# google/supersonic

Measured on AMD Instinct MI355X. Metric: rows/sec filter->project->aggregate, 100M x 8 INT64/DOUBLE, higher is better.
Workload: dtype int64/f64; 1 GPU; Q-FPA-wide: SUM(a+b),COUNT(*),SUM(c),MIN(d),MAX(d0),SUM(d1),SUM(d2*d3) WHERE a>499 over a device-resident 100000000-row x 8-col block per GPU; rows_per_gpu=100000000, parallelism=single GPU, tile_rows=512, grid=768, lds_bytes=35568, specialized_stages=1

## Files before the change

supersonic_amd/csrc/launch.h:

```cpp
#ifndef SSGPU_LAUNCH_H_
#define SSGPU_LAUNCH_H_

#ifndef __HIPCC_RTC__
#include <hip/hip_runtime_api.h>
#include <stdint.h>
#endif
#include "vm.h"

enum SlotKind {
  SLOT_SUM_INT = 0, SLOT_SUM_DD = 1, SLOT_MIN_U64 = 2, SLOT_MAX_U64 = 3, SLOT_MIN_F64 = 4,
  SLOT_MAX_F64 = 5, SLOT_FIRST = 6, SLOT_LAST = 7, SLOT_COUNT = 8
};
enum EmitKind {
  EMIT_U64 = 0, EMIT_I64KEY = 1, EMIT_U32 = 2, EMIT_I32KEY = 3, EMIT_F64 = 4, EMIT_F32 = 5,
  EMIT_DD_F64 = 6, EMIT_DD_F32 = 7, EMIT_U8 = 8,
  EMIT_DDRES_F64 = 9,
  EMIT_CNT_U64 = 20, EMIT_CNT_U32 = 21,
  EMIT_FKEY_F64 = 100, EMIT_FKEY_F32 = 101
};
#define SSGPU_STATE_ARRAYS 8

struct EmitDesc { void* data; uint8_t* is_null; int slot; int out_kind; };

struct GroupKeyOut { void* data; uint8_t* is_null; uint32_t shift, bits, nullbit, width; };
// ... 27 lines not shown
#define SSGPU_PART_MAX_WORDS 20
struct PartAggParams {
  const unsigned long long* recs;
  const unsigned int* counts;
  unsigned int n_segs, seg_cap, rec_words, n_parts;
  unsigned int local_capacity;
  unsigned int n_gaggs;
  unsigned int n_aggs, any_cnt;
  unsigned int slab_segs;
  VmGroupTable T;
  unsigned long long desc[VM_MAX_AGG_SLOTS];
  unsigned int* nan_flag;
  unsigned int hot_only, hot_base;
  DenseKeyMap dense;
};
hipError_t ssgpu_launch_part_agg(const PartAggParams& P, unsigned int lds_bytes, hipStream_t stream);
#if defined(__HIPCC__) || defined(__HIPCC_RTC__)
__device__ __forceinline__ bool ssgpu_dense_index(const DenseKeyMap& D, unsigned long long key, unsigned int* idx) {
  unsigned int i = 0; bool in = true;
  for (unsigned int k = 0; k < D.n_keys; ++k) {
    const DenseKeyMap::Key K = D.keys[k];
    const unsigned long long mask = K.bits >= 64u ? ~0ull : ((1ull << K.bits) - 1ull);
    unsigned long long off = ((key >> K.shift) - K.lo) & mask;
    const bool nullable = K.nullbit != 0xFFu;
    const bool is_null = nullable && ((key >> K.nullbit) & 1ull);
    const unsigned int values = nullable ? K.span - 1u : K.span;
    if (is_null) off = K.span - 1u;
    else if (off >= values) { in = false; off = 0; }
    i += (unsigned int)off * K.stride;
  }
  *idx = i;
  return in;
}
__device__ __forceinline__ unsigned long long ssgpu_dense_key_of(const DenseKeyMap& D, unsigned int idx) {
  unsigned long long key = 0ull;
  for (unsigned int k = 0; k < D.n_keys; ++k) {
    const DenseKeyMap::Key K = D.keys[k];
    const unsigned long long mask = K.bits >= 64u ? ~0ull : ((1ull << K.bits) - 1ull);
    const unsigned int off = (idx / K.stride) % K.span;
    if (K.nullbit != 0xFFu && off == K.span - 1u) key |= 1ull << K.nullbit;
    else key |= ((K.lo + off) & mask) << K.shift;
  }
  return key;
}
__device__ __forceinline__ unsigned int ssgpu_dense_entry(const DenseKeyMap& D, unsigned int idx, unsigned int* part) {
  if (D.n_parts == 1u) { *part = 0u; return idx; }
  unsigned int q = __umulhi(idx, D.parts_inv);
  if (q * D.n_parts > idx) --q;
  *part = idx - q * D.n_parts;
  return q;
}
#endif

#define SSGPU_PSCAT_THREADS 1024
#define SSGPU_PSCAT_XCDS 8
#define SSGPU_PSCAT_MAX_KEYS 8
#define SSGPU_PSCAT_MAX_FIELDS 24
#define SSGPU_PSCAT_MAX_PREDS 4
#define SSGPU_HOT_MAX 32
#define SSGPU_HOT_SLOTS 64
struct PlainScatterParams {
  unsigned long long n_rows;
  unsigned int n_parts, seg_cap, rec_words, rec_inv;
  unsigned int n_keys, n_fields, n_preds;
  struct Key { const void* data; const unsigned char* nulls; unsigned int width, shift, bits, nullbit; } keys[SSGPU_PSCAT_MAX_KEYS];
  struct Field { const void* src; unsigned int width, off; } fields[SSGPU_PSCAT_MAX_FIELDS];
  struct Pred { const void* data; const unsigned char* nulls; unsigned int kind, cmp, col_on_left, pad; unsigned long long bits; } preds[SSGPU_PSCAT_MAX_PREDS];
  unsigned long long* recs;
  unsigned int* counts;
  unsigned int* overflow;
  unsigned int n_hot, hot_pad;
  unsigned long long hot_keys[SSGPU_HOT_MAX];
  DenseKeyMap dense;
};
hipError_t ssgpu_launch_key_domain(const PlainScatterParams& S, const unsigned int* is_signed, unsigned long long* out, int grid, hipStream_t stream);
#define SSGPU_DENSE_HEADER 64
struct DenseFoldParams {
  const void* chunks; unsigned int n_chunks, n_gaggs, any_cnt, slots;
  unsigned long long chunk_bytes;
  unsigned long long* keys; unsigned long long* acc; unsigned int* cnt;
  const unsigned int* merge_op;
  unsigned int* flags_out;
  unsigned int* clear[2]; unsigned int n_clear[2];
};
hipError_t ssgpu_launch_dense_fold(const DenseFoldParams& P, hipStream_t stream);
hipError_t ssgpu_launch_dense_headers(void* chunks, unsigned int n_chunks, unsigned long long chunk_bytes, const unsigned int* overflow4, const unsigned int* error_flag, hipStream_t stream,
                                      unsigned int forced_flags = 0);
hipError_t ssgpu_launch_hot_keys(const PlainScatterParams& S, unsigned long long n_sample, unsigned int min_count, unsigned long long* out, hipStream_t stream);
struct PscatGeom { unsigned int threads, rows, wgs_per_cu, lds, pipe; };
PscatGeom ssgpu_part_scatter_plain_geom(unsigned int n_parts, unsigned int rec_words, int threads, int rows, int wgs_per_cu);
hipError_t ssgpu_launch_part_scatter_plain(const PlainScatterParams& P, const PscatGeom& g, int grid, hipStream_t stream);
struct FoldTailColumn {
  const void* src; const unsigned char* src_nulls; void* dst; unsigned char* dst_nulls; unsigned int op, kind;
  const unsigned long long* by; const unsigned char* by_nulls;
};
hipError_t ssgpu_launch_fold_tail(const FoldTailColumn* cols_dev, unsigned int n_cols, unsigned long long n_in, unsigned long long limit, hipStream_t stream);
unsigned int ssgpu_part_scatter_plain_lds(unsigned int n_parts, unsigned int rec_words, int rows_per_thread, int threads = SSGPU_PSCAT_THREADS);
hipError_t ssgpu_part_agg_set_max_lds(int bytes);
hipError_t ssgpu_launch_group_resident(const PartAggParams& A, const PlainScatterParams& S, unsigned int lds_bytes, int grid, hipStream_t stream);

struct JoinBuildParams {
  const void* key_data[8];
  const unsigned char* key_nulls[8];
  unsigned int width[8], shift[8], bits[8];
  unsigned int n_keys;
  unsigned int capacity_mask;
  unsigned long long n_rows;
  unsigned long long* keys;
  unsigned int* rows;
  unsigned int* special;
  unsigned int* flags;
  unsigned int* counts;
  unsigned int* slot_of_row;
  unsigned int word[8];
  unsigned long long* keys_hi;
};
hipError_t ssgpu_launch_join_expand(const unsigned int* offsets, const unsigned int* run_start, const unsigned int* rows_sorted,
                                    unsigned long long n_lhs, unsigned long long n_out, unsigned int* lhs_idx, unsigned int* rhs_row, hipStream_t stream);
hipError_t ssgpu_launch_join_build(const JoinBuildParams& P, hipStream_t stream);
hipError_t ssgpu_launch_fill_u32(unsigned int* p, unsigned int v, size_t n, hipStream_t stream);
struct GroupInitParams {
  unsigned long long* keys; unsigned long long n_keys;
  unsigned long long* acc; const unsigned long long* pattern; unsigned int ng; unsigned long long n_acc;
  unsigned int* cnt; unsigned long long n_cnt;
  unsigned int* z[4]; unsigned long long nz[4];
  unsigned int n_rep, pad; unsigned long long rep_stride;
};
hipError_t ssgpu_launch_group_init(const GroupInitParams& P, hipStream_t stream);

hipError_t ssgpu_launch_pipeline(const VmParams& P, int K, int grid, hipStream_t stream);
#ifndef __HIPCC_RTC__
#include <string>
void* ssgpu_rtc_specialize(int device, const VmInstr* prog, int n_instr, int K, bool math, const uint32_t* staged_width, const uint32_t* staged_lds_off,
                           int n_staged, uint32_t static_lds, std::string* why);
hipError_t ssgpu_launch_pipeline_rtc(void* handle, const VmParams& P, int grid, bool static_lds, hipStream_t stream);
void* ssgpu_rtc_specialize_part_agg(int device, const unsigned long long* desc, int n_aggs, unsigned int rec_words, unsigned int n_gaggs, bool any_cnt,
                                    unsigned int lds_bytes, std::string* why, const PlainScatterParams* source = nullptr,
                                    bool dense = false,
                                    bool prefetch = false);
hipError_t ssgpu_launch_group_resident_rtc(void* handle, const PartAggParams& A, const PlainScatterParams& S, int grid, hipStream_t stream);
hipError_t ssgpu_launch_part_agg_rtc(void* handle, const PartAggParams& P, hipStream_t stream);
void* ssgpu_rtc_specialize_pscat(int device, const PlainScatterParams& S, const PscatGeom& g, std::string* why);
hipError_t ssgpu_launch_part_scatter_plain_rtc(void* handle, const PlainScatterParams& P, const PscatGeom& g, int grid, hipStream_t stream);
void* ssgpu_rtc_function(void* handle);
void ssgpu_rtc_release(void* handle);
void ssgpu_rtc_cached_only(bool on);
void ssgpu_rtc_mode(int mode);
int ssgpu_rtc_current_mode();
bool ssgpu_rtc_pending();
void ssgpu_rtc_trim(int keep);
void ssgpu_rtc_stats(long long* modules, long long* code_bytes, long long* compilations, long long* disk_hits);
#endif
hipError_t ssgpu_pipeline_set_max_lds(int bytes);
hipError_t ssgpu_launch_finish_slots(const VmAccRec* partials, int n_slots, int n_parts, const int* slot_kind,
                                     VmAccRec* out, uint64_t* state , hipStream_t stream,
                                     const EmitDesc* descs = nullptr, int n_out = 0 );
hipError_t ssgpu_launch_slots_to_state(const VmAccRec* recs, int n_slots, const int* slot_kind, uint64_t* state,
                                       hipStream_t stream);
hipError_t ssgpu_launch_fold_state(const uint64_t* images, int n_images, uint64_t* state, int n_slots, const int* slot_kind, hipStream_t stream);
hipError_t ssgpu_launch_fold_emit(const uint64_t* images, int n_images, uint64_t* state, int n_slots, const int* slot_kind, VmAccRec* recs,
                                  const EmitDesc* descs, int n_out, hipStream_t stream);
hipError_t ssgpu_launch_state_to_slots(const uint64_t* state, int n_slots, const int* slot_kind, VmAccRec* recs,
                                       hipStream_t stream);
hipError_t ssgpu_launch_emit_scalar(const VmAccRec* recs, const EmitDesc* descs, int n_out, hipStream_t stream);
hipError_t ssgpu_launch_scan_counts(const uint32_t* in, uint32_t* out, int n, uint64_t* total, hipStream_t stream);
hipError_t ssgpu_launch_group_count(const GroupExtractParams& P, uint32_t* tile_counts, hipStream_t stream);
hipError_t ssgpu_launch_group_extract_lb(const GroupExtractParams& P, unsigned long long* status, uint64_t epoch, unsigned int* ctrl, unsigned int* error_flag, hipStream_t stream);
hipError_t ssgpu_launch_group_extract(const GroupExtractParams& P, hipStream_t stream);
hipError_t ssgpu_launch_fill_u64(uint64_t* p, uint64_t v, size_t n, hipStream_t stream);
hipError_t ssgpu_launch_fill_pattern_u64(uint64_t* p, const uint64_t* pattern, uint32_t plen, size_t n,
                                         hipStream_t stream);

hipError_t ssgpu_launch_sort_iota(uint32_t* idx, uint64_t n, hipStream_t s);
hipError_t ssgpu_launch_sort_load_keys(uint64_t* keys, const uint32_t* idx, const void* col, const uint8_t* nulls, uint32_t width,
                                       int kind, int descending, int null_pass, uint64_t n, unsigned long long* bits, hipStream_t s);
uint32_t ssgpu_sort_tiles(uint64_t n);
hipError_t ssgpu_launch_sort_hist(const uint64_t* keys, uint32_t shift, uint64_t n, uint32_t* hist, hipStream_t s);
hipError_t ssgpu_launch_sort_scatter(const uint64_t* keys_in, const uint32_t* idx_in, uint64_t* keys_out, uint32_t* idx_out,
                                     uint32_t shift, uint64_t n, const uint32_t* offsets, hipStream_t s);
hipError_t ssgpu_launch_sort_load_keys_hist(uint64_t* keys, const uint32_t* idx, const void* col, const uint8_t* nulls, uint32_t width, int kind,
                                            int descending, int null_pass, uint64_t n, unsigned long long* bits, uint32_t* hist8, uint32_t* base8, hipStream_t s,
                                            uint64_t* compact_out = nullptr);
hipError_t ssgpu_launch_sort_onesweep(const uint64_t* keys_in, const uint32_t* idx_in, uint64_t* keys_out, uint32_t* idx_out, uint32_t shift, uint64_t n,
                                      const uint32_t* digit_base, unsigned long long* status, uint32_t* ticket, uint64_t epoch, uint32_t* stuck, hipStream_t s);
hipError_t ssgpu_launch_sort_fix_ties(uint64_t* keys, uint32_t* idx, uint64_t n, uint32_t hi_shift, uint32_t* too_long, hipStream_t s);
struct SortRecField { const void* src; void* dst; unsigned int off, width; };
#define SSGPU_SORT_MAX_FIELDS 96
struct SortRecParams { void* recs; unsigned long long n; unsigned int stride, n_fields; SortRecField fields[SSGPU_SORT_MAX_FIELDS]; };
hipError_t ssgpu_launch_sort_pack(const SortRecParams& P, hipStream_t s);
hipError_t ssgpu_launch_sort_gather_rec(const SortRecParams& P, const uint32_t* idx, uint32_t idx_stride, hipStream_t s);
hipError_t ssgpu_launch_sort_fix_ties_compact(uint64_t* kc, const uint64_t* keys, uint64_t n, uint32_t* too_long, hipStream_t s);
hipError_t ssgpu_launch_sort_extract_idx(uint32_t* idx, const uint64_t* kc, uint64_t n, hipStream_t s);
struct UnpackPiece { unsigned long long src_off; void* dst; unsigned long long bytes; };
hipError_t ssgpu_launch_unpack(const char* slab, const UnpackPiece* pieces, unsigned int n_pieces, hipStream_t s);
uint64_t ssgpu_str_scan_partials(uint64_t n);
hipError_t ssgpu_launch_str_scan(uint64_t* data, uint64_t n, uint64_t* partials, hipStream_t s);
hipError_t ssgpu_launch_str_hash(const uint8_t* bytes, const uint64_t* offs, const uint8_t* nulls, uint64_t n, uint64_t* hashes, hipStream_t s);
hipError_t ssgpu_launch_str_insert(const uint8_t* bytes, const uint64_t* offs, const uint8_t* nulls, const uint64_t* hashes, uint64_t n,
                                   uint64_t* table, uint64_t cap, uint32_t* row_slot, uint32_t* error, hipStream_t s);
hipError_t ssgpu_launch_str_compact(const uint64_t* table, uint64_t cap, const uint8_t* bytes, const uint64_t* offs, uint32_t* count,
                                    uint32_t* d_slot, uint64_t* d_off, uint64_t* d_len, uint64_t* d_key, uint32_t* d_idx, hipStream_t s);
hipError_t ssgpu_launch_str_sort(uint64_t* d_key, uint32_t* d_idx, uint64_t d, uint64_t p, const uint8_t* bytes, const uint64_t* d_off,
                                 const uint64_t* d_len, hipStream_t s);
hipError_t ssgpu_launch_str_rank(const uint32_t* d_idx, const uint32_t* d_slot, const uint64_t* d_len, uint64_t d, int32_t* slot_rank,
                                 uint64_t* out_len, hipStream_t s);
hipError_t ssgpu_launch_str_codes(const uint32_t* row_slot, const uint8_t* nulls, const int32_t* slot_rank, uint64_t n, int32_t* codes, hipStream_t s);
hipError_t ssgpu_launch_str_gather(const uint8_t* bytes, const uint64_t* d_off, const uint32_t* d_idx, const uint64_t* out_off, uint64_t d,
                                   uint8_t* out, hipStream_t s);
hipError_t ssgpu_launch_str_recode(const int32_t* src, const uint8_t* nulls, const int32_t* remap, int32_t n_remap, uint64_t n, int32_t* dst,
                                   hipStream_t s);
hipError_t ssgpu_launch_sort_unkey(void* out, const uint64_t* keys, uint32_t width, int kind, int descending, uint64_t n, hipStream_t s);
hipError_t ssgpu_launch_sort_gather(void* out, uint8_t* out_nulls, const void* col, const uint8_t* nulls, uint32_t width,
                                    const uint32_t* idx, uint64_t n, hipStream_t s);
hipError_t ssgpu_launch_cluster_count(const void* const* data, const uint8_t* const* nulls, const uint32_t* width, uint32_t nkeys,
                                      uint64_t n, uint32_t* tile_counts, hipStream_t s);
hipError_t ssgpu_launch_cluster_flags(const void* const* data, const uint8_t* const* nulls, const uint32_t* width, uint32_t nkeys,
                                      uint64_t n, uint8_t* flag, hipStream_t s);
hipError_t ssgpu_launch_cluster_assign(const void* const* data, const uint8_t* const* nulls, const uint32_t* width, uint32_t nkeys,
                                       void* const* out_data, uint8_t* const* out_nulls, uint64_t n, const uint32_t* tile_offsets,
                                       uint32_t* seg_id, hipStream_t s);
hipError_t ssgpu_launch_gather_rowid(void* dst, const uint8_t* dst_null, const void* src, uint32_t width, int src_kind, int dst_kind, const uint64_t* rowids,
                                     uint64_t rowid_mask , int64_t row_id_base, const uint64_t* n_rows_dev, uint64_t n_rows_max, hipStream_t stream);
hipError_t ssgpu_launch_seq_sum(const void* src, const uint8_t* src_nulls, int src_kind, const uint32_t* seg_id, uint64_t n,
                                void* dst, uint8_t* dst_nulls, int dst_kind, hipStream_t s, uint64_t first = 0, uint64_t* state = nullptr, int resume = 0);
hipError_t ssgpu_launch_seg_first(const uint32_t* seg_id, const uint64_t* rowid, uint64_t n, uint32_t* first, hipStream_t s);
hipError_t ssgpu_launch_rank_scatter(const uint32_t* sorted, uint64_t n_seg, uint32_t* rank, hipStream_t s);
hipError_t ssgpu_launch_rank_rows(const uint32_t* seg_id, const uint32_t* rank, uint64_t n, uint32_t limit, uint32_t* out_rank, uint8_t* out_own, hipStream_t s);
hipError_t ssgpu_launch_dense_extract(const uint64_t* acc, const uint32_t* cnt, uint32_t n_gaggs, uint64_t n_rows,
                                      const GroupAggOut* outs, uint32_t n_out, hipStream_t s);

struct ImagePiece { const void* src; unsigned long long image_off; unsigned long long unpacked_off; unsigned int width; unsigned int pad; };
#define SSGPU_IMAGE_MAX_PIECES 92
#define SSGPU_IMAGE_HEADER 64
struct ImagePackParams {
  void* image;
  const unsigned long long* rows_dev;
  unsigned long long rows_host, capacity;
  unsigned int n_pieces, n_flags;
  const unsigned int* error_flags[8];
  const unsigned int* retry_flags[4];
  unsigned int n_retry, pad2;
  ImagePiece pieces[SSGPU_IMAGE_MAX_PIECES];
};
struct ImageUnpackParams {
  const void* images; void* unpacked;
  unsigned long long image_bytes, capacity, valid_off, trailer_off;
  unsigned int n_pieces, n_images;
  ImagePiece pieces[SSGPU_IMAGE_MAX_PIECES];
};
hipError_t ssgpu_launch_pack_image(const ImagePackParams& P, hipStream_t s);
struct ImageRoutePieces { unsigned int n_keys, n_dest; unsigned long long image_bytes; unsigned int* counters; unsigned int key_piece[16]; int key_null_piece[16]; };
hipError_t ssgpu_launch_route_images(const ImagePackParams& P, const ImageRoutePieces& R, hipStream_t s);
hipError_t ssgpu_launch_unpack_images(const ImageUnpackParams& P, hipStream_t s);

#endif
```

supersonic_amd/csrc/pipeline_kernels.hip:

```cpp
#ifndef __HIPCC_RTC__
#include <hip/hip_runtime.h>
#include <stdint.h>
#endif
#include "vm.h"
#include "launch.h"
#ifdef SSGPU_RTC_NINSTR
#include "rtc_prog.h"
#endif

typedef unsigned long long u64;
typedef long long i64;
typedef unsigned int u32;
typedef int i32;
typedef unsigned char u8;

#ifdef SSGPU_PC_PROFILE
#define PC_PROF(...) __VA_ARGS__
#else
#define PC_PROF(...)
#endif
struct LdsBase {
  __device__ __forceinline__ char* operator+(u32 off) const {
    return (char*)(__attribute__((address_space(3))) char*)off;
  }
// ... 344 lines not shown
        int src = __ffsll((long long)owner) - 1;                               \
        u64 tval = readlane64(bval, src);                                      \
        if (lane == 0) {                                                       \
          VmAccRec* A = acc_rec(P, I.dst, wave);                               \
          u64 x = A->cnt ? A->v1 : (u64)(IDENT), y = trow;                     \
          if (BETTER) { A->v1 = trow; A->v0 = tval; }                          \
          A->cnt += cnt;                                                       \
        }                                                                      \
      }                                                                        \
    }                                                                          \
  } break;

#define AGG_FUSED_I64(OPNAME, EXPR)                                            \
  case VM_##OPNAME: { CASE_FENCE;                                              \
    if (I.dst < VM_FAST_SLOTS) {                                               \
      u64 acc = F0[I.dst]; u32 ac = FC[I.dst];                                 \
      _Pragma("unroll") FOR_PAIRS {                                            \
        auto va = fetch2<u64>(I.a, I.a_mask, p);                               \
        auto vd = fetch2<u64>(I.d, I.b_mask, p);                               \
        Valid2 m = valid_pair_(p, tile_valid, I.b, I.c);                       \
        { u64 a = va.x, b = vd.x; acc += m.x ? (EXPR) : 0ull; }                \
        { u64 a = va.y, b = vd.y; acc += m.y ? (EXPR) : 0ull; }                \
        ac += (u32)m.x + (u32)m.y;                                             \
      }                                                                        \
      F0[I.dst] = acc; FC[I.dst] = ac;                                         \
    }                                                                          \
  } break;
#define AGG_FUSED_F64(OPNAME, EXPR)                                            \
  case VM_##OPNAME: { CASE_FENCE;                                              \
    if (I.dst < VM_FAST_SLOTS) {                                               \
      DD local; local.hi = u2d(F0[I.dst]); local.lo = u2d(F1[I.dst]); u32 ac = FC[I.dst]; \
      _Pragma("unroll") FOR_PAIRS {                                            \
        auto va = fetch2<double>(I.a, I.a_mask, p);                            \
        auto vd = fetch2<double>(I.d, I.b_mask, p);                            \
        Valid2 m = valid_pair_(p, tile_valid, I.b, I.c);                       \
        { double a = va.x, b = vd.x; if (m.x) local = dd_add_d(local, (EXPR)); } \
        { double a = va.y, b = vd.y; if (m.y) local = dd_add_d(local, (EXPR)); } \
        ac += (u32)m.x + (u32)m.y;                                             \
      }                                                                        \
      F0[I.dst] = d2u(local.hi); F1[I.dst] = d2u(local.lo); FC[I.dst] = ac;    \
    }                                                                          \
  } break;

#define STORE_OP(OPNAME, T)                                                    \
  case VM_##OPNAME: { CASE_FENCE;                                              \
    T* out = reinterpret_cast<T*>(P.outputs[I.dst].dst);                       \
    _Pragma("unroll") FOR_PAIRS {                                              \
      i64 r0 = tile_base + 2 * (i64)p;                                         \
      auto vv = fetch2<T>(I.a, I.a_mask, p);                             \
      if (r0 + 1 < vm_n_rows) {                                                \
        *reinterpret_cast<typename Vec2<T>::type*>(out + r0) = vv;             \
      } else if (r0 < vm_n_rows) {                                             \
        out[r0] = vv.x;                                                        \
      }                                                                        \
    }                                                                          \
  } break;

#define STOREC_OP(OPNAME, T)                                                   \
  case VM_##OPNAME: { CASE_FENCE;                                              \
    T* out = reinterpret_cast<T*>(P.outputs[I.dst].dst);                       \
    _Pragma("unroll") FOR_PAIRS {                                              \
      Valid2 m = valid_pair_(p, tile_valid, VM_NONE, I.c);          \
      auto vv = fetch2<T>(I.a, I.a_mask, p);                             \
      auto rk = lds_load2<u32>(I.b, p);                                        \
      if (m.x) out[rk.x] = vv.x;                                               \
      if (m.y) out[rk.y] = vv.y;                                               \
    }                                                                          \
  } break;

#define KEY_APPEND_OP(OPNAME, T, UT)                                           \
  case VM_##OPNAME: { CASE_FENCE;                                              \
    const u32 shift = (u32)(I.imm & 0xFF), bits = (u32)((I.imm >> 8) & 0xFF);  \
    const u32 nullbit = (u32)((I.imm >> 16) & 0xFF);                           \
    const u64 vmask = bits >= 64 ? ~0ull : ((1ull << bits) - 1ull);            \
    _Pragma("unroll") FOR_PAIRS {                                              \
      auto kk = lds_load2<u64>(I.dst, p);                                      \
      auto vv = lds_load2<T>(I.a, p);                                          \
      u64 a0 = ((u64)(UT)vv.x) & vmask, a1 = ((u64)(UT)vv.y) & vmask;          \
      if (I.b != VM_NONE) {                                                    \
        auto z = lds_load2<u8>(I.b, p);                                        \
        if (z.x) a0 = 1ull << (nullbit - shift);                               \
        if (z.y) a1 = 1ull << (nullbit - shift);                               \
      }                                                                        \
      lds_store2<u64>(I.dst, p, kk.x | (a0 << shift), kk.y | (a1 << shift));   \
    }                                                                          \
  } break;

#define GAGG_PROLOGUE(LOADT)                                                   \
      Valid2 m = valid_pair_(p, tile_valid, I.b, VM_NONE);          \
      auto sl = lds_load2<u32>(I.c, p);                                        \
      m.x = m.x && sl.x != 0xFFFFFFFFu; m.y = m.y && sl.y != 0xFFFFFFFFu;      \
      auto vv = lds_load2<LOADT>(I.a, p);

#define GAGG_APPLY(LOADT, SL, E, ATOM)                                         \
      if ((SL) & VM_SLOT_LOCAL) {                                              \
        const u32 li = ((SL) & ~VM_SLOT_LOCAL) * P.group.local_stride + s;     \
        u64* A = reinterpret_cast<u64*>(smem + P.group.local_acc_off) + li; LOADT e = (E); ATOM; \
        if (has_cnt) atomicAdd(reinterpret_cast<u32*>(smem + P.group.local_cnt_off) + li, 1u); \
      } else {                                                                 \
        u64* A = &P.group.acc[(u64)(SL) * ng + s]; LOADT e = (E); ATOM;        \
        if (has_cnt) atomicAdd(&P.group.cnt[(u64)(SL) * ng + s], 1u);          \
      }

#define GAGG_ATOMIC(OPNAME, LOADT, ATOM)                                       \
  case VM_##OPNAME: { CASE_FENCE;                                              \
    const u32 ng = (u32)(I.imm >> 32) & 0x7FFFFFFFu, s = (u32)I.imm;           \
    const bool has_cnt = (I.imm >> 63) != 0;                                   \
    _Pragma("unroll") FOR_PAIRS {                                              \
      GAGG_PROLOGUE(LOADT)                                                     \
      if (m.x) { GAGG_APPLY(LOADT, sl.x, vv.x, ATOM) }                         \
      if (m.y) { GAGG_APPLY(LOADT, sl.y, vv.y, ATOM) }                         \
    }                                                                          \
  } break;

__device__ __noinline__ u32 lookback_rows_before(unsigned long long* status, int tile, u32 run, u64 tag, unsigned int* ctrl, unsigned int* error_flag, int lane) {
  unsigned long long* const mine = status + tile;
  if (lane == 0) __hip_atomic_store(mine, (1ull << 62) | tag | (u64)run, __ATOMIC_RELAXED, __HIP_MEMORY_SCOPE_AGENT);
  u32 excl = 0, spins = 0;
  for (int j0 = tile - 1; j0 >= 0;) {
    const int j = j0 - lane;
    u64 v = (2ull << 62) | tag;
    if (j >= 0) v = __hip_atomic_load(status + j, __ATOMIC_RELAXED, __HIP_MEMORY_SCOPE_AGENT);
    const bool ready = (v >> 62) != 0 && (v & (0x3FFFFFFFull << 32)) == tag;
    const u64 pending = __ballot(!ready), prefixes = __ballot(ready && (v >> 62) == 2);
    const u32 stop = prefixes ? (u32)__builtin_ctzll(prefixes) : 63u;
    const u64 need = stop >= 63u ? ~0ull : ((2ull << stop) - 1ull);
    if (pending & need) {
      __builtin_amdgcn_s_sleep(2);
      if (++spins > (1u << 22)) { if (lane == 0) { atomicExch(ctrl + 3, 1u); atomicExch(error_flag, 3u); } break; }
      continue;
    }
    u32 part = (u32)lane <= stop ? (u32)v : 0u;
    for (int o = 32; o > 0; o >>= 1) part += (u32)__shfl_xor((int)part, o);
    excl += part;
    if (prefixes) break;
    j0 -= 64;
  }
  if (lane == 0) __hip_atomic_store(mine, (2ull << 62) | tag | (u64)(excl + run), __ATOMIC_RELAXED, __HIP_MEMORY_SCOPE_AGENT);
  return excl;
}

__device__ __forceinline__ double vm_math1(u32 fn, double a) {
  switch (fn) {
    case VM_MATH_EXP: return exp(a);     case VM_MATH_LN: return log(a);       case VM_MATH_LOG10: return log10(a);
    case VM_MATH_LOG2: return log2(a);   case VM_MATH_SIN: return sin(a);      case VM_MATH_COS: return cos(a);
    case VM_MATH_TAN: return tan(a);     case VM_MATH_ASIN: return asin(a);    case VM_MATH_ACOS: return acos(a);
    case VM_MATH_ATAN: return atan(a);   case VM_MATH_SINH: return sinh(a);    case VM_MATH_COSH: return cosh(a);
    case VM_MATH_TANH: return tanh(a);   case VM_MATH_ASINH: return asinh(a);  case VM_MATH_ACOSH: return acosh(a);
    default: return atanh(a);
  }
}

#ifndef SSGPU_RTC_PART
template <int K, bool MATH>
__global__ __launch_bounds__(VM_WG_THREADS, VM_WAVES_PER_EU) void ssgpu_pipeline_kernel(const VmParams P) {
#ifdef SSGPU_RTC_STATIC_LDS
  __shared__ __attribute__((aligned(16))) char rtc_static_lds[SSGPU_RTC_STATIC_LDS];
  asm volatile("" ::"v"((u32)(size_t)(__attribute__((address_space(3))) char*)rtc_static_lds));
#endif
  const int t = threadIdx.x;
  const int lane = t & 63;
  const int wave = t >> 6;
  const int tile_rows = VM_TILE_UNIT * K;
  i64 vm_n_rows = P.n_rows; int vm_n_tiles = P.n_tiles;
  if (P.n_rows_dev) {
    const u64 have = *P.n_rows_dev;
    vm_n_rows = have < (u64)P.n_rows ? (i64)have : P.n_rows;
    vm_n_tiles = (int)((vm_n_rows + tile_rows - 1) / tile_rows);
  }
  const int vm_first_tile = ((P.flags & VM_FLAG_XCD_CHUNKS) && (gridDim.x & 7u) == 0u) ? (int)((blockIdx.x & 7u) * (gridDim.x >> 3) + (blockIdx.x >> 3)) : (int)blockIdx.x;
  const int n_my_tiles = vm_n_tiles > vm_first_tile ? (vm_n_tiles - vm_first_tile + (int)gridDim.x - 1) / (int)gridDim.x : 0;
  const int n_units = STAGED_COUNT(P) * K;

  for (u32 o = (u32)t * 8u; o < (u32)P.n_slots * VM_ACC_STRIDE; o += VM_COMPUTE_THREADS * 8u)
    *reinterpret_cast<u64*>(smem + P.acc_lds_off + o) = 0ull;
  typedef u64 u64xS __attribute__((ext_vector_type(VM_FAST_SLOTS)));
  typedef u32 u32xS __attribute__((ext_vector_type(VM_FAST_SLOTS)));
  u64xS F0, F1; u32xS FC;
#pragma unroll
  for (int s = 0; s < VM_FAST_SLOTS; ++s) { F0[s] = P.slot_init0[s]; F1[s] = P.slot_init1[s]; FC[s] = 0; }
  bool vm_nan_seen = false;
  for (u32 o = (u32)t * 8u; o < 2u * (u32)tile_rows; o += VM_COMPUTE_THREADS * 8u)
    *reinterpret_cast<u64*>(smem + P.const_lds_off + o) = o < (u32)tile_rows ? 0x0101010101010101ull : 0ull;

  typedef u32 u32x8 __attribute__((ext_vector_type(8)));
  typedef const __attribute__((address_space(4))) u32x8* ProgPtr;
  const ProgPtr prog0 = (ProgPtr)(P.prog);

  for (int pc = t; pc < P.n_instr; pc += VM_COMPUTE_THREADS) {
    const VmInstr J = P.prog[pc];
    const u32 w = J.imm_width;
    if (w) {
      u64 lo = J.imm;
      if (w == 4) lo = (lo & 0xFFFFFFFFull) * 0x100000001ull;
      else if (w == 1) lo = (lo & 0xFFull) * 0x0101010101010101ull;
      u64* e = reinterpret_cast<u64*>(smem + P.imm_pool_lds_off + (u32)pc * 16u);
      e[0] = lo; e[1] = lo;
    }
  }

  if (P.group.local_capacity) {
    const VmGroupTable& G = P.group;
    for (u32 e = (u32)t; e < G.local_capacity; e += VM_COMPUTE_THREADS)
      reinterpret_cast<u64*>(smem + G.local_keys_off)[e] = VM_KEY_EMPTY;
    for (u32 i = (u32)t; i < G.local_capacity * G.local_stride; i += VM_COMPUTE_THREADS) {
      reinterpret_cast<u64*>(smem + G.local_acc_off)[i] = G.acc_init[(i % G.local_stride) % G.n_gaggs];
      if (G.local_cnt_off != VM_NONE) reinterpret_cast<u32*>(smem + G.local_cnt_off)[i] = 0u;
    }
    if (t < 2) reinterpret_cast<u32*>(smem + P.scratch_lds_off + 128u)[t] = 0u;
  }
  if (P.part_n) {
    u32* h = reinterpret_cast<u32*>(smem + P.part_lds_off);
    for (u32 i = (u32)t; i < P.part_n; i += VM_COMPUTE_THREADS) h[i] = 0u;
  }
  PC_PROF(if (P.debug_pc) for (int i = t; i <= P.n_instr; i += VM_COMPUTE_THREADS) reinterpret_cast<u64*>(smem + P.debug_pc_lds_off)[i] = 0ull;)
  __syncthreads();

  u32x4 pf[VM_PF_UNITS];
#pragma unroll
  for (int u = 0; u < VM_PF_UNITS; ++u) pf[u] = u32x4{0u, 0u, 0u, 0u};
  const int n_pf = n_units < VM_PF_UNITS ? n_units : VM_PF_UNITS;
  {
    const i64 tb = (i64)vm_first_tile * tile_rows;
    if (n_my_tiles > 0 && tb + tile_rows <= vm_n_rows) {
#pragma unroll
      for (int u = 0; u < VM_PF_UNITS; ++u)
        if (u < n_pf) load_unit<K>(P, u, tb, t, pf[u]);
    }
  }

  u64 dbg_wait = 0;
  const u64 dbg_t0 = P.debug ? __builtin_amdgcn_s_memtime() : 0;
  const ProgPtr prog = prog0;
  for (int it = 0; it < n_my_tiles; ++it) {
    const int tile = vm_first_tile + it * (int)gridDim.x;
    const i64 tile_base = (i64)tile * tile_rows;
    const u32 tile_valid = (u32)((vm_n_rows - tile_base) < (i64)tile_rows ? (vm_n_rows - tile_base) : (i64)tile_rows);
    const u64 tw0 = (P.debug || P.debug_pc) ? __builtin_amdgcn_s_memtime() : 0;
    __builtin_amdgcn_s_setprio(VM_STAGE_PRIO);
    if (tile_valid == (u32)tile_rows) {
      int tc = t;
      asm volatile("" : "+v"(tc));
#pragma unroll
      for (int u = 0; u < VM_PF_UNITS; ++u)
        if (u < n_pf) commit_unit<K>(P, u, pf[u], tc);
      if (P.debug) dbg_wait += __builtin_amdgcn_s_memtime() - tw0;
      if (n_units > VM_PF_UNITS) stage_units_direct<K>(P, VM_PF_UNITS, n_units, tile_base, tile_valid, t);
    } else {
      stage_units_direct<K>(P, 0, n_units, tile_base, tile_valid, t);
    }
    {
      const i64 tb = tile_base + (i64)gridDim.x * tile_rows;
      if (it + 1 < n_my_tiles && tb + tile_rows <= vm_n_rows) {
        int tl = t;
        asm volatile("" : "+v"(tl));
#pragma unroll
        for (int u = 0; u < VM_PF_UNITS; ++u)
          if (u < n_pf) load_unit<K>(P, u, tb, tl, pf[u]);
      }
    }

    __builtin_amdgcn_s_setprio(0);
#ifdef SSGPU_RTC_NINSTR
#define VM_PC_LOOP _Pragma("unroll") for (int pc = 0; pc < SSGPU_RTC_NINSTR; ++pc)
#define VM_FETCH_NEXT(pc) u32x8{kRtcProg[pc][0], kRtcProg[pc][1], kRtcProg[pc][2], kRtcProg[pc][3], kRtcProg[pc][4], kRtcProg[pc][5], kRtcProg[pc][6], kRtcProg[pc][7]}
    (void)prog;
    u32x8 raw_next = VM_FETCH_NEXT(0);
#else
#define VM_PC_LOOP for (int pc = 0; pc < P.n_instr; ++pc)
#define VM_FETCH_NEXT(pc) prog[pc]
    u32x8 raw_next = prog[0];
#endif
    PC_PROF(u64 dbg_pc_last = 0;
    if (P.debug_pc) { dbg_pc_last = __builtin_amdgcn_s_memtime(); if (t == 0) reinterpret_cast<u64*>(smem + P.debug_pc_lds_off)[P.n_instr] += dbg_pc_last - tw0; })
#ifdef SSGPU_RTC_NINSTR
#include "rtc_steps.h"
#else
    VM_PC_LOOP {
#include "vm_body.inc"
    }
#endif
    PC_PROF(if (P.debug_pc && P.n_instr > 0 && t == 0) reinterpret_cast<u64*>(smem + P.debug_pc_lds_off)[P.n_instr - 1] += __builtin_amdgcn_s_memtime() - dbg_pc_last;)
  }

  if (vm_nan_seen && P.error_flag) atomicOr(P.error_flag, SSGPU_FLAG_NAN_IN_MINMAX);
  if (P.part_n && P.tile_counts) {
    __syncthreads();
    const u32* h = reinterpret_cast<const u32*>(smem + P.part_lds_off);
    for (u32 i = (u32)t; i < P.part_n; i += VM_COMPUTE_THREADS) P.tile_counts[(u64)i * gridDim.x + blockIdx.x] = h[i] < P.part_seg_cap ? h[i] : P.part_seg_cap;
  }
  if (P.group.local_capacity) {
    const VmGroupTable& G = P.group;
    __syncthreads();
    const u32 ng = G.n_gaggs;
    u32 occupied = 0;
    for (u32 e = (u32)t; e < G.local_capacity; e += VM_COMPUTE_THREADS) {
      const u64 key = reinterpret_cast<const u64*>(smem + G.local_keys_off)[e];
      if (key == VM_KEY_EMPTY) continue;
      ++occupied;
      const u32 gs = group_insert(G, key);
      if (gs == 0xFFFFFFFFu) continue;
      for (u32 s = 0; s < ng; ++s) {
        const u64 v = reinterpret_cast<const u64*>(smem + G.local_acc_off)[e * G.local_stride + s];
        u64* A = &G.acc[(u64)gs * ng + s];
        const u32 op = G.merge_op[s];
        if (op == VM_MERGE_ADD_U64) { if (v) atomicAdd(A, v); }
        else if (op == VM_MERGE_MIN_U64) atomicMin(A, v);
        else if (op == VM_MERGE_MAX_U64) atomicMax(A, v);
        else if (op == VM_MERGE_ADD_F64_HI) dd_atomic_add(reinterpret_cast<double*>(A), u2d(v));
        else unsafeAtomicAdd(reinterpret_cast<double*>(A), u2d(v));
        if (G.local_cnt_off != VM_NONE) {
          const u32 c = reinterpret_cast<const u32*>(smem + G.local_cnt_off)[e * G.local_stride + s];
          if (c) atomicAdd(&G.cnt[(u64)gs * ng + s], c);
        }
      }
    }
    u32* st = reinterpret_cast<u32*>(smem + P.scratch_lds_off + 128u);
    if (occupied) atomicAdd(&st[1], occupied);
    __syncthreads();
    if (t == 0) { if (st[0]) atomicAdd(&G.stats[0], st[0]); atomicMax(&G.stats[1], st[1]); }
  }

  PC_PROF(if (P.debug_pc && t == 0) for (int i = 0; i <= P.n_instr; ++i) atomicAdd(&P.debug_pc[i], reinterpret_cast<const u64*>(smem + P.debug_pc_lds_off)[i]);)
  if (P.debug && t == 0) {
    P.debug[blockIdx.x * 4 + 0] = __builtin_amdgcn_s_memtime() - dbg_t0;
    P.debug[blockIdx.x * 4 + 1] = dbg_wait;
    P.debug[blockIdx.x * 4 + 2] = (u64)n_my_tiles;
  }
#pragma unroll
  for (int s = 0; s < VM_FAST_SLOTS; ++s) {
    if (s < P.n_slots) {
      const int kind = P.slot_kind[s];
      const u64 cnt = wave_reduce_u64((u64)FC[s], [](u64 x, u64 y) { return x + y; });
      u64 v0 = 0, v1 = 0;
      switch (kind) {
        case SLOT_COUNT: v0 = cnt; break;
        case SLOT_SUM_INT: v0 = wave_reduce_u64(F0[s], [](u64 x, u64 y) { return x + y; }); break;
        case SLOT_MIN_U64: v0 = wave_reduce_u64(F0[s], [](u64 x, u64 y) { return x < y ? x : y; }); break;
        case SLOT_MAX_U64: v0 = wave_reduce_u64(F0[s], [](u64 x, u64 y) { return x > y ? x : y; }); break;
        case SLOT_MIN_F64: v0 = wave_reduce_u64(F0[s], [](u64 x, u64 y) { return u2d(y) < u2d(x) ? y : x; }); break;
        case SLOT_MAX_F64: v0 = wave_reduce_u64(F0[s], [](u64 x, u64 y) { return u2d(x) < u2d(y) ? y : x; }); break;
        case SLOT_SUM_DD: {
          DD d; d.hi = u2d(F0[s]); d.lo = u2d(F1[s]);
          d = wave_reduce_dd(d); v0 = d2u(d.hi); v1 = d2u(d.lo);
        } break;
        case SLOT_FIRST: case SLOT_LAST: {
          const bool first = kind == SLOT_FIRST;
          const u64 trow = first ? wave_reduce_u64(F1[s], [](u64 x, u64 y) { return x < y ? x : y; })
                                 : wave_reduce_u64(FC[s] ? F1[s] : 0ull, [](u64 x, u64 y) { return x > y ? x : y; });
          const u64 owner = __ballot(FC[s] != 0 && F1[s] == trow);
          const int src = owner ? __ffsll((long long)owner) - 1 : 0;
          v0 = readlane64(F0[s], src); v1 = trow;
        } break;
        default: break;
      }
      if (lane == 0) { VmAccRec* A = acc_rec(P, (u32)s, wave); A->v0 = v0; A->v1 = v1; A->cnt = cnt; A->pad = 0; }
    }
  }

  __syncthreads();
  for (int s = t; s < P.n_slots; s += VM_COMPUTE_THREADS)
    for (int w = 0; w < VM_WAVES; ++w)
      P.wg_partials[((size_t)blockIdx.x * P.n_slots + s) * VM_WAVES + w] = *acc_rec(P, (u32)s, w);
}
#endif

#ifndef __HIPCC_RTC__

__device__ __forceinline__ void combine_rec(int kind, VmAccRec& acc, const VmAccRec& r) {
  if (r.cnt == 0) return;
  switch (kind) {
    case SLOT_COUNT:
    case SLOT_SUM_INT: acc.v0 += r.v0; break;
    case SLOT_SUM_DD: {
      DD a; a.hi = u2d(acc.v0); a.lo = u2d(acc.v1);
      DD b; b.hi = u2d(r.v0); b.lo = u2d(r.v1);
      a = dd_add(a, b); acc.v0 = d2u(a.hi); acc.v1 = d2u(a.lo);
    } break;
    case SLOT_MIN_U64: acc.v0 = acc.cnt ? (r.v0 < acc.v0 ? r.v0 : acc.v0) : r.v0; break;
    case SLOT_MAX_U64: acc.v0 = acc.cnt ? (r.v0 > acc.v0 ? r.v0 : acc.v0) : r.v0; break;
    case SLOT_MIN_F64: acc.v0 = acc.cnt ? (u2d(r.v0) < u2d(acc.v0) ? r.v0 : acc.v0) : r.v0; break;
    case SLOT_MAX_F64: acc.v0 = acc.cnt ? (u2d(acc.v0) < u2d(r.v0) ? r.v0 : acc.v0) : r.v0; break;
    case SLOT_FIRST: if (!acc.cnt || r.v1 < acc.v1) { acc.v0 = r.v0; acc.v1 = r.v1; } break;
    case SLOT_LAST: if (!acc.cnt || r.v1 >= acc.v1) { acc.v0 = r.v0; acc.v1 = r.v1; } break;
  }
  acc.cnt += r.cnt;
}

__device__ __forceinline__ void slot_to_state(const VmAccRec r, int kind, int s, int n_slots, u64* __restrict__ state) {
  u64* sum_i = state; u64* cnt = state + n_slots; u64* hi = state + 2 * n_slots; u64* lo = state + 3 * n_slots;
  u64* mn = state + 4 * n_slots; u64* mx = state + 5 * n_slots;
  u64* mnf = state + 6 * n_slots; u64* mxf = state + 7 * n_slots;
  const bool fl = kind == SLOT_FIRST || kind == SLOT_LAST;
  sum_i[s] = (kind == SLOT_SUM_INT || kind == SLOT_COUNT || fl) ? r.v0 : 0;
  cnt[s] = r.cnt;
  hi[s] = kind == SLOT_SUM_DD ? r.v0 : d2u(0.0);
  lo[s] = kind == SLOT_SUM_DD ? r.v1 : d2u(0.0);
  mn[s] = (kind == SLOT_MIN_U64 && r.cnt) ? (r.v0 ^ 0x8000000000000000ull) : (kind == SLOT_FIRST && r.cnt) ? (r.v1 ^ 0x8000000000000000ull) : 0x7FFFFFFFFFFFFFFFull;
  mx[s] = (kind == SLOT_MAX_U64 && r.cnt) ? (r.v0 ^ 0x8000000000000000ull) : (kind == SLOT_LAST && r.cnt) ? (r.v1 ^ 0x8000000000000000ull) : 0x8000000000000000ull;
  mnf[s] = (kind == SLOT_MIN_F64 && r.cnt) ? r.v0 : d2u(__builtin_inf());
  mxf[s] = (kind == SLOT_MAX_F64 && r.cnt) ? r.v0 : d2u(-__builtin_inf());
}
__device__ __forceinline__ VmAccRec state_to_slot(const u64* __restrict__ state, int kind, int s, int n_slots) {
  VmAccRec r; r.v0 = 0; r.v1 = 0; r.pad = 0;
  r.cnt = state[n_slots + s];
  switch (kind) {
    case SLOT_COUNT: case SLOT_SUM_INT: r.v0 = state[s]; break;
    case SLOT_SUM_DD: {
      DD a; a.hi = u2d(state[2 * n_slots + s]); a.lo = 0.0;
      a = dd_add_d(a, u2d(state[3 * n_slots + s]));
      r.v0 = d2u(a.hi); r.v1 = d2u(a.lo);
    } break;
    case SLOT_MIN_U64: r.v0 = state[4 * n_slots + s] ^ 0x8000000000000000ull; break;
    case SLOT_MAX_U64: r.v0 = state[5 * n_slots + s] ^ 0x8000000000000000ull; break;
    case SLOT_MIN_F64: r.v0 = state[6 * n_slots + s]; break;
    case SLOT_MAX_F64: r.v0 = state[7 * n_slots + s]; break;
    case SLOT_FIRST: r.v0 = state[s]; r.v1 = state[4 * n_slots + s] ^ 0x8000000000000000ull; break;
    case SLOT_LAST: r.v0 = state[s]; r.v1 = state[5 * n_slots + s] ^ 0x8000000000000000ull; break;
    default: break;
  }
  return r;
}

__device__ __forceinline__ void emit_scalar_one(const EmitDesc d, const VmAccRec r);
__global__ __launch_bounds__(256) void ssgpu_finish_slots_kernel(const VmAccRec* __restrict__ partials, int n_slots,
                                                                 int n_parts, const int* __restrict__ slot_kind,
                                                                 VmAccRec* __restrict__ out, u64* __restrict__ state,
                                                                 const EmitDesc* __restrict__ descs, int n_out) {
  __shared__ VmAccRec tree[256];
  const int s = blockIdx.x, t = threadIdx.x;
  const int kind = slot_kind[s];
  VmAccRec acc; acc.v0 = 0; acc.v1 = 0; acc.cnt = 0; acc.pad = 0;
  if (kind == SLOT_SUM_DD) { acc.v0 = d2u(-0.0); acc.v1 = d2u(0.0); }
  for (int i = t; i < n_parts; i += 256) {
    const VmAccRec r = partials[((size_t)(i / VM_WAVES) * n_slots + s) * VM_WAVES + (i % VM_WAVES)];
    combine_rec(kind, acc, r);
  }
  tree[t] = acc;
  __syncthreads();
  for (int stride = 128; stride > 0; stride >>= 1) {
    if (t < stride) { VmAccRec a = tree[t]; combine_rec(kind, a, tree[t + stride]); tree[t] = a; }
    __syncthreads();
  }
  if (t == 0) { out[s] = tree[0]; if (state) slot_to_state(tree[0], kind, s, n_slots, state); }
  if (descs)
    for (int i = t; i < n_out; i += 256) { const EmitDesc d = descs[i]; if (d.slot == s) emit_scalar_one(d, tree[0]); }
}

__global__ void ssgpu_slots_to_state_kernel(const VmAccRec* __restrict__ recs, int n_slots,
                                            const int* __restrict__ slot_kind, u64* __restrict__ state) {
  int s = blockIdx.x * blockDim.x + threadIdx.x;
  if (s >= n_slots) return;
  slot_to_state(recs[s], slot_kind[s], s, n_slots, state);
}
__global__ void ssgpu_state_to_slots_kernel(const u64* __restrict__ state, int n_slots,
                                            const int* __restrict__ slot_kind, VmAccRec* __restrict__ recs) {
  int s = blockIdx.x * blockDim.x + threadIdx.x;
  if (s >= n_slots) return;
  recs[s] = state_to_slot(state, slot_kind[s], s, n_slots);
}


__device__ __forceinline__ void emit_value(void* dst, size_t idx, int out_kind, u64 v0, u64 v1) {
  switch (out_kind) {
    case EMIT_U64: reinterpret_cast<u64*>(dst)[idx] = v0; break;
    case EMIT_I64KEY: reinterpret_cast<i64*>(dst)[idx] = unkey_i64(v0); break;
    case EMIT_U32: reinterpret_cast<u32*>(dst)[idx] = (u32)v0; break;
    case EMIT_I32KEY: reinterpret_cast<i32*>(dst)[idx] = (i32)unkey_i64(v0); break;
    case EMIT_F64: reinterpret_cast<double*>(dst)[idx] = u2d(v0); break;
    case EMIT_F32: reinterpret_cast<float*>(dst)[idx] = (float)u2d(v0); break;
    case EMIT_DD_F64: { double hi = u2d(v0), lo = u2d(v1);
      reinterpret_cast<double*>(dst)[idx] = (lo == 0.0) ? hi : hi + lo; } break;
    case EMIT_DDRES_F64: { const double hi = u2d(v0), lo = u2d(v1), sm = hi + lo, bp = sm - hi;
      reinterpret_cast<double*>(dst)[idx] = (lo == 0.0) ? 0.0 : (hi - (sm - bp)) + (lo - bp); } break;
    case EMIT_DD_F32: { double hi = u2d(v0), lo = u2d(v1);
      reinterpret_cast<float*>(dst)[idx] = (float)((lo == 0.0) ? hi : hi + lo); } break;
    case EMIT_U8: reinterpret_cast<u8*>(dst)[idx] = (u8)(v0 != 0); break;
    default: break;
  }
}


__device__ __forceinline__ void emit_scalar_one(const EmitDesc d, const VmAccRec r) {
  if (d.out_kind == EMIT_CNT_U64 || d.out_kind == EMIT_CNT_U32)
    emit_value(d.data, 0, d.out_kind == EMIT_CNT_U64 ? EMIT_U64 : EMIT_U32, r.cnt, 0);
  else
    emit_value(d.data, 0, d.out_kind, r.v0, r.v1);
  if (d.is_null) d.is_null[0] = r.cnt == 0;
}
__global__ void ssgpu_emit_scalar_kernel(const VmAccRec* __restrict__ recs, const EmitDesc* __restrict__ descs,
                                         int n_out) {
  int i = blockIdx.x * blockDim.x + threadIdx.x;
  if (i >= n_out) return;
  const EmitDesc d = descs[i];
  emit_scalar_one(d, recs[d.slot]);
}

__global__ __launch_bounds__(1024) void ssgpu_scan_counts_kernel(const u32* __restrict__ in, u32* __restrict__ out,
                                                                  int n, u64* __restrict__ total) {
  __shared__ u64 wave_sums[16];
  __shared__ u64 carry_s;
  const int t = threadIdx.x, lane = t & 63, wave = t >> 6;
  if (t == 0) carry_s = 0;
  __syncthreads();
  for (int base = 0; base < n; base += 1024 * 8) {
    u32 v[8]; u64 sum = 0;
    int i0 = base + t * 8;
#pragma unroll
    for (int j = 0; j < 8; ++j) { v[j] = (i0 + j < n) ? in[i0 + j] : 0u; sum += v[j]; }
    u64 inc = sum;
#pragma unroll
    for (int d = 1; d < 64; d <<= 1) { u64 o = __shfl_up(inc, d); if (lane >= d) inc += o; }
    if (lane == 63) wave_sums[wave] = inc;
    __syncthreads();
    u64 wpre = 0;
    for (int w = 0; w < wave; ++w) wpre += wave_sums[w];
    u64 run = carry_s + wpre + (inc - sum);
#pragma unroll
    for (int j = 0; j < 8; ++j) { if (i0 + j < n) out[i0 + j] = (u32)run; run += v[j]; }
    __syncthreads();
    if (t == 1023) carry_s = run;
    __syncthreads();
  }
  if (t == 0) *total = carry_s;
}

__device__ __forceinline__ bool group_slot_occupied(const GroupExtractParams& P, u32 slot) {
  if (slot > P.capacity + P.extra_slots) return false;
  return P.keys[slot] != VM_KEY_EMPTY;
}

__global__ __launch_bounds__(256) void ssgpu_group_count_kernel(const GroupExtractParams P, u32* __restrict__ tile_counts) {
  __shared__ u32 wsum[4];
  const int t = threadIdx.x, lane = t & 63, wave = t >> 6;
  u32 s0 = blockIdx.x * 512u + t * 2u;
  bool o0 = group_slot_occupied(P, s0);
  bool o1 = group_slot_occupied(P, s0 + 1);
  u32 c = (u32)__popcll(__ballot(o0)) + (u32)__popcll(__ballot(o1));
  if (lane == 0) wsum[wave] = c;
  __syncthreads();
  if (t == 0) tile_counts[blockIdx.x] = wsum[0] + wsum[1] + wsum[2] + wsum[3];
}

__device__ __forceinline__ void group_extract_slot(const GroupExtractParams& P, u32 slot, u32 row);
__global__ __launch_bounds__(256) void ssgpu_group_extract_lb_kernel(const GroupExtractParams P, unsigned long long* __restrict__ status, u64 tag,
                                                                     unsigned int* __restrict__ ctrl, unsigned int* __restrict__ error_flag) {
  __shared__ u32 wsum[4];
  __shared__ u32 s_tile, s_base;
  const int t = threadIdx.x, lane = t & 63, wave = t >> 6;
  if (t == 0) s_tile = atomicAdd(ctrl + 2, 1u);
  __syncthreads();
  const u32 tile = s_tile;
  const u32 s0 = tile * 512u + (u32)t * 2u;
  const bool o0 = group_slot_occupied(P, s0), o1 = group_slot_occupied(P, s0 + 1);
  const u64 b0 = __ballot(o0), b1 = __ballot(o1);
  if (lane == 0) wsum[wave] = (u32)__popcll(b0) + (u32)__popcll(b1);
  __syncthreads();
  if (wave == 0) {
    const u32 run = wsum[0] + wsum[1] + wsum[2] + wsum[3];
    const u32 excl = lookback_rows_before(status, (int)tile, run, tag, ctrl, error_flag, lane);
    if (lane == 0) {
      s_base = excl;
      if (tile == gridDim.x - 1u) *reinterpret_cast<u64*>(ctrl) = (u64)excl + run;
    }
  }
  __syncthreads();
  u32 base = s_base;
  for (int w = 0; w < wave; ++w) base += wsum[w];
  const u64 lt = (1ull << lane) - 1ull;
  const u32 r0 = base + (u32)__popcll(b0 & lt) + (u32)__popcll(b1 & lt);
  if (o0) group_extract_slot(P, s0, r0);
  if (o1) group_extract_slot(P, s0 + 1, r0 + (o0 ? 1u : 0u));
}

__global__ __launch_bounds__(256) void ssgpu_group_extract_kernel(const GroupExtractParams P) {
  __shared__ u32 wsum[4];
  const int t = threadIdx.x, lane = t & 63, wave = t >> 6;
  u32 s0 = blockIdx.x * 512u + t * 2u;
  bool o0 = group_slot_occupied(P, s0);
  bool o1 = group_slot_occupied(P, s0 + 1);
  u64 b0 = __ballot(o0), b1 = __ballot(o1);
  if (lane == 0) wsum[wave] = (u32)__popcll(b0) + (u32)__popcll(b1);
  __syncthreads();
  u32 base = P.tile_offsets[blockIdx.x];
  for (int w = 0; w < wave; ++w) base += wsum[w];
  const u64 lt = (1ull << lane) - 1ull;
  u32 r0 = base + (u32)__popcll(b0 & lt) + (u32)__popcll(b1 & lt);
  if (o0) group_extract_slot(P, s0, r0);
  if (o1) group_extract_slot(P, s0 + 1, r0 + (o0 ? 1u : 0u));
}
__device__ __forceinline__ void group_extract_slot(const GroupExtractParams& P, u32 slot, u32 row) {
  {
    const u64 key = slot == P.capacity ? VM_KEY_EMPTY : P.keys[slot];
    for (u32 q = 0; q < P.n_keys; ++q) {
      const GroupKeyOut ko = P.keys_out[q];
      u64 field = key >> ko.shift;
      bool isnull = ko.nullbit != 0xFF && ((key >> ko.nullbit) & 1ull);
      u64 vmask = ko.bits >= 64 ? ~0ull : ((1ull << ko.bits) - 1ull);
      u64 v = isnull ? 0ull : (field & vmask);
      if (ko.width == 8) reinterpret_cast<u64*>(ko.data)[row] = v;
      else if (ko.width == 4) reinterpret_cast<u32*>(ko.data)[row] = (u32)v;
      else reinterpret_cast<u8*>(ko.data)[row] = (u8)v;
      if (ko.is_null) ko.is_null[row] = isnull;
    }
    for (u32 q = 0; q < P.n_aggs_out; ++q) {
      const GroupAggOut ao = P.aggs_out[q];
      u64 v0 = P.acc[(u64)slot * P.n_gaggs + ao.s];
      u32 c = ao.has_cnt ? P.cnt[(u64)slot * P.n_gaggs + ao.s] : 1u;
      if (ao.out_kind == EMIT_FKEY_F64) {
        v0 = (v0 & 0x8000000000000000ull) ? (v0 & 0x7FFFFFFFFFFFFFFFull) : ~v0;
        emit_value(ao.data, row, EMIT_F64, v0, 0);
      } else if (ao.out_kind == EMIT_FKEY_F32) {
        v0 = (v0 & 0x8000000000000000ull) ? (v0 & 0x7FFFFFFFFFFFFFFFull) : ~v0;
        emit_value(ao.data, row, EMIT_F32, v0, 0);
      } else {
        emit_value(ao.data, row, ao.out_kind, v0, (ao.out_kind == EMIT_DD_F64 || ao.out_kind == EMIT_DDRES_F64) ? P.acc[(u64)slot * P.n_gaggs + ao.s + 1] : 0ull);
      }
      if (ao.is_null) ao.is_null[row] = c == 0;
    }
  }
}

#endif

#if !defined(__HIPCC_RTC__) || defined(SSGPU_RTC_PART)
#ifdef SSGPU_RTC_PART
#include "rtc_part.h"
#define PART_NG(P) kPartNg
#define PART_W(P) kPartW
#define PART_ANY_CNT(P) (kPartAnyCnt != 0u)
#define PART_NAGGS(P) kPartNAggs
#define PART_AGG_LOOP _Pragma("unroll") for (u32 s = 0; s < kPartNAggs; ++s)
#define PART_DESC(s) kPartDesc[s]
#define PART_DENSE(P) (kPartDense != 0u)
#else
#define PART_NG(P) (P).n_gaggs
#define PART_W(P) (P).rec_words
#define PART_ANY_CNT(P) ((P).any_cnt != 0u)
#define PART_NAGGS(P) (P).n_aggs
#define PART_AGG_LOOP for (u32 s = 0; s < n_aggs; ++s)
#define PART_DESC(s) readlane64(mydesc, (int)(s))
#define PART_DENSE(P) ((P).dense.on != 0u)
// ... 635 lines not shown
  size_t stride = (size_t)gridDim.x * blockDim.x;
  for (; i < n; i += stride) p[i] = v;
}

__global__ void ssgpu_fill_u64_kernel(u64* __restrict__ p, u64 v, size_t n) {
  size_t i = (size_t)blockIdx.x * blockDim.x + threadIdx.x;
  size_t stride = (size_t)gridDim.x * blockDim.x;
  for (; i < n; i += stride) p[i] = v;
}
__global__ __launch_bounds__(256) void ssgpu_group_init_kernel(const GroupInitParams P) {
  const u64 first = (u64)blockIdx.x * 256 + threadIdx.x, stride = (u64)gridDim.x * 256;
  for (u32 r = 0; r <= P.n_rep; ++r) {
    u64* const keys = reinterpret_cast<u64*>(reinterpret_cast<char*>(P.keys) + (u64)r * P.rep_stride);
    u64* const acc = reinterpret_cast<u64*>(reinterpret_cast<char*>(P.acc) + (u64)r * P.rep_stride);
    u32* const cnt = reinterpret_cast<u32*>(reinterpret_cast<char*>(P.cnt) + (u64)r * P.rep_stride);
    for (u64 i = first; i < P.n_keys; i += stride) keys[i] = VM_KEY_EMPTY;
    for (u64 i = first; i < P.n_acc; i += stride) acc[i] = P.pattern[i % P.ng];
    for (u64 i = first; i < P.n_cnt; i += stride) cnt[i] = 0u;
  }
  for (int q = 0; q < 4; ++q) for (u64 i = first; i < P.nz[q]; i += stride) P.z[q][i] = 0u;
}
__global__ void ssgpu_fill_pattern_u64_kernel(u64* __restrict__ p, const u64* __restrict__ pattern, u32 plen, size_t n) {
  size_t i = (size_t)blockIdx.x * blockDim.x + threadIdx.x;
  size_t stride = (size_t)gridDim.x * blockDim.x;
  for (; i < n; i += stride) p[i] = pattern[i % plen];
}

hipError_t ssgpu_launch_pipeline(const VmParams& P, int K, int grid, hipStream_t stream) {
  dim3 g(grid), b(VM_WG_THREADS);
  size_t lds = P.lds_bytes;
  if (P.uses_math) {
    switch (K) {
      case 1: hipLaunchKernelGGL((ssgpu_pipeline_kernel<1, true>), g, b, lds, stream, P); break;
      case 2: hipLaunchKernelGGL((ssgpu_pipeline_kernel<2, true>), g, b, lds, stream, P); break;
      case 4: hipLaunchKernelGGL((ssgpu_pipeline_kernel<4, true>), g, b, lds, stream, P); break;
      default: return hipErrorInvalidValue;
    }
    return hipGetLastError();
  }
  switch (K) {
    case 1: hipLaunchKernelGGL((ssgpu_pipeline_kernel<1, false>), g, b, lds, stream, P); break;
    case 2: hipLaunchKernelGGL((ssgpu_pipeline_kernel<2, false>), g, b, lds, stream, P); break;
    case 4: hipLaunchKernelGGL((ssgpu_pipeline_kernel<4, false>), g, b, lds, stream, P); break;
    default: return hipErrorInvalidValue;
  }
  return hipGetLastError();
}
__global__ __launch_bounds__(256) void ssgpu_join_expand_kernel(const u32* __restrict__ offsets, const u32* __restrict__ run_start,
                                                                const u32* __restrict__ rows_sorted, u64 n_lhs, u64 n_out,
                                                                u32* __restrict__ lhs_idx, u32* __restrict__ rhs_row) {
  const u64 o = (u64)blockIdx.x * 256 + threadIdx.x;
  if (o >= n_out) return;
  u64 lo = 0, hi = n_lhs - 1;
  while (lo < hi) {
    const u64 mid = (lo + hi + 1) >> 1;
    if ((u64)offsets[mid] <= o) lo = mid; else hi = mid - 1;
  }
  const u32 s = run_start[lo];
  lhs_idx[o] = (u32)lo;
  rhs_row[o] = s == VM_NONE ? VM_NONE : rows_sorted[(u64)s + (o - (u64)offsets[lo])];
}
hipError_t ssgpu_launch_join_expand(const unsigned int* offsets, const unsigned int* run_start, const unsigned int* rows_sorted,
                                    unsigned long long n_lhs, unsigned long long n_out, unsigned int* lhs_idx, unsigned int* rhs_row, hipStream_t stream) {
  if (n_out) hipLaunchKernelGGL(ssgpu_join_expand_kernel, dim3((unsigned)((n_out + 255) / 256)), dim3(256), 0, stream,
                                offsets, run_start, rows_sorted, (u64)n_lhs, (u64)n_out, lhs_idx, rhs_row);
  return hipGetLastError();
}
hipError_t ssgpu_launch_join_build(const JoinBuildParams& P, hipStream_t stream) {
  if (P.n_rows) hipLaunchKernelGGL(ssgpu_join_build_kernel, dim3((unsigned)((P.n_rows + 255) / 256)), dim3(256), 0, stream, P);
  return hipGetLastError();
}
__global__ __launch_bounds__(256) void ssgpu_gather_rowid_kernel(void* __restrict__ dst, const u8* __restrict__ dst_null, const void* __restrict__ src,
                                                                 u32 width, int src_kind, int dst_kind, const u64* __restrict__ rowids, u64 rowid_mask, i64 row_id_base,
                                                                 const u64* __restrict__ n_rows_dev, u64 n_rows_max) {
  const u64 i = (u64)blockIdx.x * 256 + threadIdx.x;
  const u64 n = n_rows_dev ? *n_rows_dev : n_rows_max;
  if (i >= n || i >= n_rows_max) return;
  const bool isnull = dst_null && dst_null[i];
  const u64 r = isnull ? 0ull : (u64)((i64)(rowids[i] & rowid_mask) - row_id_base);
  if (src_kind == dst_kind) {
    if (width == 8) reinterpret_cast<u64*>(dst)[i] = isnull ? 0ull : reinterpret_cast<const u64*>(src)[r];
    else if (width == 4) reinterpret_cast<u32*>(dst)[i] = isnull ? 0u : reinterpret_cast<const u32*>(src)[r];
    else reinterpret_cast<u8*>(dst)[i] = isnull ? (u8)0 : reinterpret_cast<const u8*>(src)[r];
    return;
  }
  i64 vi = 0; u64 vu = 0; double vf = 0.0; int fam = 0;
  if (!isnull) switch (src_kind) {
    case 0: vi = reinterpret_cast<const i32*>(src)[r]; fam = 0; break;
    case 1: vu = reinterpret_cast<const u32*>(src)[r]; fam = 1; break;
    case 2: vi = reinterpret_cast<const i64*>(src)[r]; fam = 0; break;
    case 3: vu = reinterpret_cast<const u64*>(src)[r]; fam = 1; break;
    case 4: vf = (double)reinterpret_cast<const float*>(src)[r]; fam = 2; break;
    case 5: vf = reinterpret_cast<const double*>(src)[r]; fam = 2; break;
    default: vu = reinterpret_cast<const u8*>(src)[r]; fam = 1; break;
  }
  if (dst_kind == 4 || dst_kind == 5) {
    const double d = fam == 2 ? vf : (fam == 1 ? (double)vu : (double)vi);
    if (dst_kind == 5) reinterpret_cast<double*>(dst)[i] = d;
    else reinterpret_cast<float*>(dst)[i] = fam == 2 ? (float)vf : (fam == 1 ? (float)vu : (float)vi);
    return;
  }
  u64 bits;
  if (fam == 2) {
    const double tr = trunc(vf);
    bits = (tr >= -9223372036854775808.0 && tr < 9223372036854775808.0) ? (u64)(i64)tr : 0x8000000000000000ull;
  } else bits = fam == 1 ? vu : (u64)vi;
  if (dst_kind == 2 || dst_kind == 3) reinterpret_cast<u64*>(dst)[i] = bits;
  else if (dst_kind == 0 || dst_kind == 1) reinterpret_cast<u32*>(dst)[i] = (u32)bits;
  else reinterpret_cast<u8*>(dst)[i] = (u8)bits;
}
hipError_t ssgpu_launch_gather_rowid(void* dst, const uint8_t* dst_null, const void* src, uint32_t width, int src_kind, int dst_kind, const uint64_t* rowids, uint64_t rowid_mask,
                                     int64_t row_id_base, const uint64_t* n_rows_dev, uint64_t n_rows_max, hipStream_t stream) {
  if (n_rows_max) hipLaunchKernelGGL(ssgpu_gather_rowid_kernel, dim3((unsigned)((n_rows_max + 255) / 256)), dim3(256), 0, stream,
                                     dst, dst_null, src, width, src_kind, dst_kind, (const u64*)rowids, (u64)rowid_mask, (i64)row_id_base, (const u64*)n_rows_dev, (u64)n_rows_max);
  return hipGetLastError();
}
hipError_t ssgpu_launch_fill_u32(unsigned int* p, unsigned int v, size_t n, hipStream_t stream) {
  if (n) hipLaunchKernelGGL(ssgpu_fill_u32_kernel, dim3((unsigned)std::min<size_t>((n + 255) / 256, 4096)), dim3(256), 0, stream, p, v, n);
  return hipGetLastError();
}
hipError_t ssgpu_launch_part_agg(const PartAggParams& P, unsigned int lds_bytes, hipStream_t stream) {
  if (P.rec_words <= 8) hipLaunchKernelGGL(ssgpu_part_agg_kernel<8>, dim3(P.n_parts), dim3(SSGPU_PART_THREADS), lds_bytes, stream, P);
  else if (P.rec_words <= 16) hipLaunchKernelGGL(ssgpu_part_agg_kernel<16>, dim3(P.n_parts), dim3(SSGPU_PART_THREADS), lds_bytes, stream, P);
  else if (P.rec_words <= SSGPU_PART_MAX_WORDS) hipLaunchKernelGGL(ssgpu_part_agg_kernel<SSGPU_PART_MAX_WORDS>, dim3(P.n_parts), dim3(SSGPU_PART_THREADS), lds_bytes, stream, P);
  else return hipErrorInvalidValue;
  return hipGetLastError();
}
hipError_t ssgpu_launch_group_resident(const PartAggParams& P, const PlainScatterParams& S, unsigned int lds_bytes, int grid, hipStream_t stream) {
  if (P.rec_words <= 8) hipLaunchKernelGGL(ssgpu_group_resident_kernel<8>, dim3(grid), dim3(SSGPU_PART_THREADS), lds_bytes, stream, P, S);
  else hipLaunchKernelGGL(ssgpu_group_resident_kernel<16>, dim3(grid), dim3(SSGPU_PART_THREADS), lds_bytes, stream, P, S);
  return hipGetLastError();
}
hipError_t ssgpu_part_agg_set_max_lds(int bytes) {
  hipError_t e = hipFuncSetAttribute(reinterpret_cast<const void*>(ssgpu_part_agg_kernel<8>), hipFuncAttributeMaxDynamicSharedMemorySize, bytes);
  if (e != hipSuccess) return e;
  e = hipFuncSetAttribute(reinterpret_cast<const void*>(ssgpu_group_resident_kernel<8>), hipFuncAttributeMaxDynamicSharedMemorySize, bytes);
  if (e != hipSuccess) return e;
  e = hipFuncSetAttribute(reinterpret_cast<const void*>(ssgpu_group_resident_kernel<16>), hipFuncAttributeMaxDynamicSharedMemorySize, bytes);
  if (e != hipSuccess) return e;
  e = hipFuncSetAttribute(reinterpret_cast<const void*>(ssgpu_part_agg_kernel<SSGPU_PART_MAX_WORDS>), hipFuncAttributeMaxDynamicSharedMemorySize, bytes);
  if (e != hipSuccess) return e;
  return hipFuncSetAttribute(reinterpret_cast<const void*>(ssgpu_part_agg_kernel<16>), hipFuncAttributeMaxDynamicSharedMemorySize, bytes);
}
hipError_t ssgpu_pipeline_set_max_lds(int bytes) {
  hipError_t e;
  e = hipFuncSetAttribute(reinterpret_cast<const void*>(ssgpu_pipeline_kernel<1, false>), hipFuncAttributeMaxDynamicSharedMemorySize, bytes); if (e != hipSuccess) return e;
  e = hipFuncSetAttribute(reinterpret_cast<const void*>(ssgpu_pipeline_kernel<2, false>), hipFuncAttributeMaxDynamicSharedMemorySize, bytes); if (e != hipSuccess) return e;
  e = hipFuncSetAttribute(reinterpret_cast<const void*>(ssgpu_pipeline_kernel<4, false>), hipFuncAttributeMaxDynamicSharedMemorySize, bytes); if (e != hipSuccess) return e;
  e = hipFuncSetAttribute(reinterpret_cast<const void*>(ssgpu_pipeline_kernel<1, true>), hipFuncAttributeMaxDynamicSharedMemorySize, bytes); if (e != hipSuccess) return e;
  e = hipFuncSetAttribute(reinterpret_cast<const void*>(ssgpu_pipeline_kernel<2, true>), hipFuncAttributeMaxDynamicSharedMemorySize, bytes); if (e != hipSuccess) return e;
  e = hipFuncSetAttribute(reinterpret_cast<const void*>(ssgpu_pipeline_kernel<4, true>), hipFuncAttributeMaxDynamicSharedMemorySize, bytes);
  return e;
}
hipError_t ssgpu_launch_finish_slots(const VmAccRec* partials, int n_slots, int n_parts, const int* slot_kind,
                                     VmAccRec* out, uint64_t* state, hipStream_t stream, const EmitDesc* descs, int n_out) {
  hipLaunchKernelGGL(ssgpu_finish_slots_kernel, dim3(n_slots), dim3(256), 0, stream, partials, n_slots, n_parts, slot_kind, out, (u64*)state, descs, n_out);
  return hipGetLastError();
}
hipError_t ssgpu_launch_slots_to_state(const VmAccRec* recs, int n_slots, const int* slot_kind, uint64_t* state, hipStream_t stream) {
  int blocks = (n_slots + 63) / 64;
  hipLaunchKernelGGL(ssgpu_slots_to_state_kernel, dim3(blocks), dim3(64), 0, stream, recs, n_slots, slot_kind, (u64*)state);
  return hipGetLastError();
}
__device__ __forceinline__ void fold_state_slot(const u64* __restrict__ images, int n_images, u64* __restrict__ state, int n_slots, int kind, int s);
__global__ __launch_bounds__(64) void ssgpu_fold_state_kernel(const u64* __restrict__ images, int n_images, u64* __restrict__ state,
                                                              int n_slots, const int* __restrict__ slot_kind) {
  const int s = blockIdx.x * 64 + threadIdx.x;
  if (s >= n_slots) return;
  fold_state_slot(images, n_images, state, n_slots, slot_kind[s], s);
}
__device__ __forceinline__ void fold_state_slot(const u64* __restrict__ images, int n_images, u64* __restrict__ state, int n_slots, int kind, int s) {
  const size_t total = (size_t)SSGPU_STATE_ARRAYS * n_slots;
  u64 a[SSGPU_STATE_ARRAYS];
  for (int k = 0; k < SSGPU_STATE_ARRAYS; ++k) a[k] = images[(size_t)k * n_slots + s];
  for (int r = 1; r < n_images; ++r) {
    u64 v[SSGPU_STATE_ARRAYS];
    for (int k = 0; k < SSGPU_STATE_ARRAYS; ++k) v[k] = images[(size_t)r * total + (size_t)k * n_slots + s];
    if (kind == SLOT_FIRST) { if ((i64)v[4] < (i64)a[4]) a[0] = v[0]; }
    else if (kind == SLOT_LAST) { if ((i64)v[5] > (i64)a[5]) a[0] = v[0]; }
    else a[0] += v[0];
    a[1] += v[1];
    a[2] = d2u(u2d(a[2]) + u2d(v[2]));
    a[3] = d2u(u2d(a[3]) + u2d(v[3]));
    a[4] = (i64)v[4] < (i64)a[4] ? v[4] : a[4];
    a[5] = (i64)v[5] > (i64)a[5] ? v[5] : a[5];
    a[6] = u2d(v[6]) < u2d(a[6]) ? v[6] : a[6];
    a[7] = u2d(v[7]) > u2d(a[7]) ? v[7] : a[7];
  }
  for (int k = 0; k < SSGPU_STATE_ARRAYS; ++k) state[(size_t)k * n_slots + s] = a[k];
}
__global__ __launch_bounds__(256) void ssgpu_fold_emit_kernel(const u64* __restrict__ images, int n_images, u64* __restrict__ state, int n_slots,
                                                              const int* __restrict__ slot_kind, VmAccRec* __restrict__ recs,
                                                              const EmitDesc* __restrict__ descs, int n_out) {
  for (int s = threadIdx.x; s < n_slots; s += 256) {
    fold_state_slot(images, n_images, state, n_slots, slot_kind[s], s);
    recs[s] = state_to_slot(state, slot_kind[s], s, n_slots);
  }
  __threadfence_block();
  __syncthreads();
  for (int i = threadIdx.x; i < n_out; i += 256) { const EmitDesc d = descs[i]; emit_scalar_one(d, recs[d.slot]); }
}
hipError_t ssgpu_launch_fold_emit(const uint64_t* images, int n_images, uint64_t* state, int n_slots, const int* slot_kind, VmAccRec* recs,
                                  const EmitDesc* descs, int n_out, hipStream_t stream) {
  hipLaunchKernelGGL(ssgpu_fold_emit_kernel, dim3(1), dim3(256), 0, stream, (const u64*)images, n_images, (u64*)state, n_slots, slot_kind, recs, descs, n_out);
  return hipGetLastError();
}
hipError_t ssgpu_launch_fold_state(const uint64_t* images, int n_images, uint64_t* state, int n_slots, const int* slot_kind, hipStream_t stream) {
  if (n_slots > 0) hipLaunchKernelGGL(ssgpu_fold_state_kernel, dim3((n_slots + 63) / 64), dim3(64), 0, stream, (const u64*)images, n_images, (u64*)state, n_slots, slot_kind);
  return hipGetLastError();
}
hipError_t ssgpu_launch_state_to_slots(const uint64_t* state, int n_slots, const int* slot_kind, VmAccRec* recs, hipStream_t stream) {
  int blocks = (n_slots + 63) / 64;
  hipLaunchKernelGGL(ssgpu_state_to_slots_kernel, dim3(blocks), dim3(64), 0, stream, (const u64*)state, n_slots, slot_kind, recs);
  return hipGetLastError();
}
hipError_t ssgpu_launch_emit_scalar(const VmAccRec* recs, const EmitDesc* descs, int n_out, hipStream_t stream) {
  int blocks = (n_out + 63) / 64;
  hipLaunchKernelGGL(ssgpu_emit_scalar_kernel, dim3(blocks), dim3(64), 0, stream, recs, descs, n_out);
  return hipGetLastError();
}
__global__ __launch_bounds__(1024) void ssgpu_scan_chunk_totals_kernel(const u32* __restrict__ in, int n, u32* __restrict__ totals) {
  __shared__ u64 wave_sums[16];
  const int t = threadIdx.x, lane = t & 63, wave = t >> 6;
  const int i0 = blockIdx.x * 8192 + t * 8;
  u64 sum = 0;
#pragma unroll
  for (int j = 0; j < 8; ++j) sum += (i0 + j < n) ? in[i0 + j] : 0u;
#pragma unroll
  for (int d = 32; d > 0; d >>= 1) sum += __shfl_xor(sum, d);
  if (lane == 0) wave_sums[wave] = sum;
  __syncthreads();
  if (t == 0) { u64 s = 0; for (int w = 0; w < 16; ++w) s += wave_sums[w]; totals[blockIdx.x] = (u32)s; }
}
__global__ __launch_bounds__(1024) void ssgpu_scan_chunks_kernel(const u32* __restrict__ in, u32* __restrict__ out, int n,
                                                                  const u32* __restrict__ chunk_base) {
  __shared__ u64 wave_sums[16];
  const int t = threadIdx.x, lane = t & 63, wave = t >> 6;
  const int i0 = blockIdx.x * 8192 + t * 8;
  u32 v[8]; u64 sum = 0;
#pragma unroll
  for (int j = 0; j < 8; ++j) { v[j] = (i0 + j < n) ? in[i0 + j] : 0u; sum += v[j]; }
  u64 inc = sum;
#pragma unroll
  for (int d = 1; d < 64; d <<= 1) { u64 o = __shfl_up(inc, d); if (lane >= d) inc += o; }
  if (lane == 63) wave_sums[wave] = inc;
  __syncthreads();
  u64 run = chunk_base[blockIdx.x] + (inc - sum);
  for (int w = 0; w < wave; ++w) run += wave_sums[w];
#pragma unroll
  for (int j = 0; j < 8; ++j) { if (i0 + j < n) out[i0 + j] = (u32)run; run += v[j]; }
}

hipError_t ssgpu_launch_scan_counts(const uint32_t* in, uint32_t* out, int n, uint64_t* total, hipStream_t stream) {
  if (n <= 65536) {
    hipLaunchKernelGGL(ssgpu_scan_counts_kernel, dim3(1), dim3(1024), 0, stream, in, out, n, (u64*)total);
    return hipGetLastError();
  }
  static thread_local u32* d_totals = nullptr; static thread_local u32* d_bases = nullptr; static thread_local int cap = 0;
  const int chunks = (n + 8191) / 8192;
  if (chunks > cap) {
    if (d_totals) { (void)hipFree(d_totals); (void)hipFree(d_bases); }
    hipError_t e = hipMalloc((void**)&d_totals, (size_t)chunks * 4); if (e != hipSuccess) return e;
    e = hipMalloc((void**)&d_bases, (size_t)chunks * 4); if (e != hipSuccess) return e;
    cap = chunks;
  }
  hipLaunchKernelGGL(ssgpu_scan_chunk_totals_kernel, dim3(chunks), dim3(1024), 0, stream, in, n, d_totals);
  hipLaunchKernelGGL(ssgpu_scan_counts_kernel, dim3(1), dim3(1024), 0, stream, d_totals, d_bases, chunks, (u64*)total);
  hipLaunchKernelGGL(ssgpu_scan_chunks_kernel, dim3(chunks), dim3(1024), 0, stream, in, out, n, d_bases);
  return hipGetLastError();
}
hipError_t ssgpu_launch_group_count(const GroupExtractParams& P, uint32_t* tile_counts, hipStream_t stream) {
  int blocks = (int)(((size_t)P.capacity + 1 + 511) / 512);
  hipLaunchKernelGGL(ssgpu_group_count_kernel, dim3(blocks), dim3(256), 0, stream, P, tile_counts);
  return hipGetLastError();
}
hipError_t ssgpu_launch_group_extract_lb(const GroupExtractParams& P, unsigned long long* status, uint64_t epoch, unsigned int* ctrl, unsigned int* error_flag, hipStream_t stream) {
  int blocks = (int)(((size_t)P.capacity + 1 + P.extra_slots + 511) / 512);
  hipLaunchKernelGGL(ssgpu_group_extract_lb_kernel, dim3(blocks), dim3(256), 0, stream, P, status, (u64)((epoch & 0x3FFFFFFFull) << 32), ctrl, error_flag);
  return hipGetLastError();
}
hipError_t ssgpu_launch_group_extract(const GroupExtractParams& P, hipStream_t stream) {
  int blocks = (int)(((size_t)P.capacity + 1 + 511) / 512);
  hipLaunchKernelGGL(ssgpu_group_extract_kernel, dim3(blocks), dim3(256), 0, stream, P);
  return hipGetLastError();
}
hipError_t ssgpu_launch_fill_u64(uint64_t* p, uint64_t v, size_t n, hipStream_t stream) {
  int blocks = (int)((n + 255) / 256); if (blocks > 4096) blocks = 4096; if (blocks < 1) blocks = 1;
  hipLaunchKernelGGL(ssgpu_fill_u64_kernel, dim3(blocks), dim3(256), 0, stream, (u64*)p, (u64)v, n);
  return hipGetLastError();
}
hipError_t ssgpu_launch_group_init(const GroupInitParams& P, hipStream_t stream) {
  const uint64_t n = std::max<uint64_t>(std::max<uint64_t>(P.n_keys, P.n_acc), std::max<uint64_t>(P.n_cnt, std::max<uint64_t>(std::max<uint64_t>(P.nz[0], P.nz[3]), std::max<uint64_t>(P.nz[1], P.nz[2]))));
  int blocks = (int)std::min<uint64_t>((n + 255) / 256, 4096); if (blocks < 1) blocks = 1;
  hipLaunchKernelGGL(ssgpu_group_init_kernel, dim3(blocks), dim3(256), 0, stream, P);
  return hipGetLastError();
}
hipError_t ssgpu_launch_fill_pattern_u64(uint64_t* p, const uint64_t* pattern, uint32_t plen, size_t n, hipStream_t stream) {
  int blocks = (int)((n + 255) / 256); if (blocks > 4096) blocks = 4096; if (blocks < 1) blocks = 1;
  hipLaunchKernelGGL(ssgpu_fill_pattern_u64_kernel, dim3(blocks), dim3(256), 0, stream, (u64*)p, (const u64*)pattern, plen, n);
  return hipGetLastError();
}
#endif
```

supersonic_amd/csrc/runtime.cpp:

```cpp
#include <hip/hip_runtime_api.h>

#include <atomic>
#include <map>
#include <mutex>
#include <stdio.h>
#include <string.h>
#include <algorithm>
#include <cmath>
#include <string>
#include <unistd.h>
#include <thread>
#include <unordered_set>
#include <vector>
#include <deque>
#include <functional>

#include "engine.h"

using namespace ssgpu;

#define HIP_TRY(ctx, expr)                                                          \
  do {                                                                               \
    hipError_t _e = (expr);                                                          \
    if (_e != hipSuccess) {                                                          \
      (ctx)->err = _e == hipErrorOutOfMemory ? std::string("Memory exceeded: ") + #expr : std::string(#expr) + ": " + hipGetErrorString(_e); \
      return _e == hipErrorOutOfMemory ? SSGPU_ERROR_MEMORY_EXCEEDED : SSGPU_ERROR_HIP; \
    }                                                                                \
  } while (0)

static bool trace_on() { static const bool on = getenv("SSGPU_TRACE") != nullptr; return on; }
struct ssgpu_ctx {
  std::atomic<int> refs{1};
  int device = -1;
  hipStream_t stream = nullptr, copy_stream = nullptr;
  std::atomic<bool> copy_pending{false};
  hipEvent_t copy_ev = nullptr;
  bool own_stream = false;
  int cu_count = 0;
  std::string err;
  LowerOptions opt;
  int64_t grid_limit = 0;
  int64_t out_arena = 1;
  int64_t tile_map = 1;
  int64_t wgs_per_cu = 3;
  int64_t group_capacity = 1 << 18;
  int64_t group_local = 1;
  int64_t group_partition = 1;
  int64_t part_n = 0;
  int64_t part_wgs_per_cu = 0;
  int64_t part_lds_target = 0;
  int64_t sort_records = 1;
  int64_t sort_hybrid = 1;
  int64_t group_slab = 1;
  int64_t group_scout = 1;
  int64_t group_scout_rows = 8 << 20;
  int64_t group_resident = 1;
  int64_t group_dense = 1;
  int64_t dense_parts = 0;
  int64_t dense_min_rows = 1 << 16;
  int64_t async_handoff = 1;
  int64_t lazy_feedback = 0;
  int64_t part_prefetch = 1;
  int64_t fuse_emit = 1;
  int64_t pscat_pipe = 1;
  int64_t pscat_threads = 0, pscat_rows = 0, pscat_wgs = 0;
  int64_t part_plain = 1;
  int64_t sort_compact = 1;
  int64_t sort_hi_digits = 4;
  int64_t part_agg_lds = 0;
  int64_t profile = 1;
  int64_t profile_total = 1;
  int64_t debug_timing = 0;
  int64_t specialize = 3;
  int64_t specialize_min_rows = 1 << 22;
};

struct MemQuota { int64_t limit = -1; int64_t used = 0; };
static thread_local MemQuota* g_quota = nullptr;
struct QuotaScope { MemQuota* saved; explicit QuotaScope(MemQuota* q) : saved(g_quota) { g_quota = q; } ~QuotaScope() { g_quota = saved; } };

static std::atomic<long long> g_dev_bytes{0}, g_pinned_bytes{0}, g_live_plans{0}, g_live_blocks{0}, g_events{0};

struct DevPool {
  std::mutex m;
  std::multimap<size_t, std::pair<void*, int>> blocks;
  size_t bytes = 0;
  size_t limit() { static const size_t v = [] { const char* e = getenv("SSGPU_POOL_MB"); return (size_t)(e ? atoll(e) : 4096) << 20; }(); return v; }
  bool park(void* p, size_t cap) {
    if (limit() == 0) return false;
    hipPointerAttribute_t attr;
    if (hipPointerGetAttributes(&attr, p) != hipSuccess) { (void)hipGetLastError(); return false; }
    const int dev = attr.device;
    std::lock_guard<std::mutex> lock(m);
    if (bytes + cap > limit() || blocks.size() >= 4096) return false;
    blocks.emplace(cap, std::make_pair(p, dev)); bytes += cap;
    return true;
  }
  void* take(size_t want, size_t* cap) {
    int dev = 0;
    if (limit() == 0 || hipGetDevice(&dev) != hipSuccess) return nullptr;
    const size_t most = want <= 4096 ? 4096 : want * 2;
    std::lock_guard<std::mutex> lock(m);
    for (auto it = blocks.lower_bound(want); it != blocks.end() && it->first <= most; ++it)
      if (it->second.second == dev) { void* p = it->second.first; *cap = it->first; bytes -= it->first; blocks.erase(it); return p; }
    return nullptr;
  }
  size_t trim(int dev);
  size_t parked(int dev) {
    std::lock_guard<std::mutex> lock(m);
    size_t n = 0;
    for (auto& b : blocks) if (dev < 0 || b.second.second == dev) n += b.first;
    return n;
  }
};
static DevPool g_pool;
size_t DevPool::trim(int dev) {
  std::vector<std::pair<void*, size_t>> out;
  {
    std::lock_guard<std::mutex> lock(m);
    for (auto it = blocks.begin(); it != blocks.end();)
      if (dev < 0 || it->second.second == dev) { out.emplace_back(it->second.first, it->first); bytes -= it->first; it = blocks.erase(it); } else ++it;
  }
  size_t freed = 0;
  for (auto& b : out) { (void)hipFree(b.first); g_dev_bytes.fetch_sub((long long)b.second); freed += b.second; }
  return freed;
}
static std::atomic<int> g_device_contexts{0};
static thread_local bool tls_park_released = false;

struct DevBuf {
  void* p = nullptr;
  size_t cap = 0;
  bool view = false;
  MemQuota* q = nullptr;
  ~DevBuf() { release(); }
  void release() {
    if (p && !view) {
      if (q) q->used -= (int64_t)cap;
      if (!(tls_park_released && g_pool.park(p, cap))) { (void)hipFree(p); g_dev_bytes.fetch_sub((long long)cap); }
    }
    p = nullptr; cap = 0; q = nullptr; view = false;
  }
  void set_view(void* ptr, size_t bytes) { release(); p = ptr; cap = bytes; view = true; }
  hipError_t ensure(size_t bytes) {
    if (bytes <= cap && p) return hipSuccess;
    if (view) return hipErrorInvalidValue;
    size_t want = std::max<size_t>(bytes, 256);
    MemQuota* Q = g_quota;
    if (Q && Q->limit >= 0 && Q->used - (q == Q ? (int64_t)cap : 0) + (int64_t)want > Q->limit) return hipErrorOutOfMemory;
    static const bool trace = getenv("SSGPU_TRACE") != nullptr;
    if (trace && want >= (64u << 20)) fprintf(stderr, "[ssgpu trace] device buffer %zu -> %zu MiB\n", cap >> 20, want >> 20);
    release();
    size_t pooled_cap = 0;
    if (void* pooled = (Q && Q->limit >= 0) ? nullptr : g_pool.take(want, &pooled_cap)) { p = pooled; cap = pooled_cap; q = Q; if (q) q->used += (int64_t)cap; return hipSuccess; }
    hipError_t e = hipMalloc(&p, want);
    if (e == hipErrorOutOfMemory) {
      (void)hipGetLastError();
      int dev = -1;
      if (hipGetDevice(&dev) == hipSuccess && g_pool.trim(dev) > 0) e = hipMalloc(&p, want);
    }
    if (e == hipSuccess) { cap = want; q = Q; g_dev_bytes.fetch_add((long long)want); if (q) q->used += (int64_t)want; } else p = nullptr;
    return e;
  }
  template <typename T> T* as() const { return reinterpret_cast<T*>(p); }
};

struct PinnedBuf {
  void* p = nullptr;
  size_t cap = 0;
  ~PinnedBuf() { drop(); }
  void drop() { if (p) { (void)hipHostFree(p); g_pinned_bytes.fetch_sub((long long)cap); } p = nullptr; cap = 0; }
  hipError_t ensure(size_t bytes) {
    if (bytes <= cap && p) return hipSuccess;
    drop();
    size_t want = std::max<size_t>(bytes, 256);
    hipError_t e = hipHostMalloc(&p, want, hipHostMallocDefault);
    if (e == hipSuccess) { cap = want; g_pinned_bytes.fetch_add((long long)want); } else p = nullptr;
    return e;
  }
};

struct OutCol { DevBuf data, nulls; bool nullable = false; uint32_t width = 8; };

struct StageExec {
  DevBuf prog_main, prog_count;
  struct RtcSlot {
    void* h = nullptr; bool tried = false; uint32_t static_lds = 0, tag = 0;
    int missed_mode = -1;
    bool stronger_mode_now() const { if (h || missed_mode < 0) return false; const int m = ssgpu_rtc_current_mode(); return missed_mode == 1 && m != 1; }
    bool pending = false; std::chrono::steady_clock::time_point next_poll{};
    void drop() { if (h) ssgpu_rtc_release(h); h = nullptr; tried = false; static_lds = 0; tag = 0; pending = false; missed_mode = -1; }
    bool ask_again() {
      if (!pending) return false;
      const auto now = std::chrono::steady_clock::now();
      if (now < next_poll) return false;
      next_poll = now + std::chrono::milliseconds(20);
      return true;
    }
    void asked() { pending = !h && ssgpu_rtc_pending(); missed_mode = h ? -1 : ssgpu_rtc_current_mode(); if (pending) next_poll = std::chrono::steady_clock::now() + std::chrono::milliseconds(20); }
  };
  RtcSlot rtc_main;
  std::vector<VmInstr> host_prog_main;
  std::string rtc_why;
  ProgramLayout lay{};
  ProgramLayout lay_count{};
  int n_instr_main = 0, n_instr_count = 0;
  int grid = 0;
  DevBuf wg_partials, slot_recs, slot_kind, emit_descs, state;
  DevBuf tile_counts, tile_offsets, total;
  DevBuf xstatus; uint64_t x_epoch = 0;
  DevBuf gkeys, gacc, gcnt, goverflow, gpattern, gmergeop;
  int group_wgs = 3;
  bool group_local = true;
  int group_sub = 1;
  bool group_partitioned = false;
  uint32_t part_n = 256;
  bool part_n_chosen = false;
  bool part_slab_failed = false;
  bool scouted = false;
  int64_t scout_full_rows = 0;
  bool part_slab = false;
  double part_groups_est = 0;
  uint32_t part_seg_growth = 1;
  bool part_failed = false;
  DevBuf prog_pscatter, part_hist, part_recs;
  ProgramLayout lay_pscatter{};
  int n_instr_pscatter = 0;
  RtcSlot rtc_pscatter; std::vector<VmInstr> host_prog_pscatter;
  RtcSlot rtc_plain;
  RtcSlot rtc_part;
  RtcSlot rtc_resident;
  RtcSlot rtc_hot;
  uint32_t hot_n = 0; uint64_t hot_keys[SSGPU_HOT_MAX] = {0};
  int64_t hot_sampled_run = -1;
  DevBuf hot_out;
  struct DenseState {
    bool on = false, failed = false, checked = false, fixed = false, resident = false;
    uint32_t n_keys = 0, n_chunks = 1;
    uint64_t lo[8] = {0}, hi[8] = {0};
    uint32_t span[8] = {0}, stride[8] = {0};
    uint64_t slots = 0;
    uint32_t np = 0, cap = 0;
    uint64_t chunk_bytes = 0;
    int64_t widened = 0;
  } dense;
  DevBuf dense_dom, dense_flags;
  void* dense_table = nullptr;
  std::vector<DevBuf> rowid_tmp;
  std::vector<DevBuf> jkeys, jkeys_hi, jrows, jmisc;
  std::vector<DevBuf> jcounts, jstarts, jslot_of_row, jrows_sorted;
  DevBuf jx_offsets, jx_lhs_idx, jx_rhs_row;
  std::vector<VmJoin> vm_joins;
  uint32_t capacity = 0;
  DevBuf error_flag;
  DevBuf debug, debug_pc, total2;
  DevBuf skeys_a, skeys_b, skeys_c, sidx_a, sidx_b, shist, soffs, seg_id, sstatus, sticket, srecs, dflag;
  DevBuf rank_first, rank_of_seg, rank_row, rank_own;
  DevBuf seg_counts, seg_offsets, seg_total;
  DevBuf route_scratch;
  uint64_t sort_epoch = 0;
  bool emit_ready = false;
  bool emitted_with_finish = false;
  bool pattern_ready = false;
  DevBuf out_arena;
  std::vector<OutCol> out;
  int64_t out_rows = -1;
  const void* out_rows_dev = nullptr;
  int64_t out_capacity = 0;
  int last_group_shape = 0;
  int last_reruns = 0;
  int last_sort_passes = 0, last_sort_mode = 0;
  bool last_plain_scatter = false;
  PinnedBuf fb_host;
  int fb_pending = 0;
  hipEvent_t fb_event = nullptr;
  int steady = 0;
  uint32_t steady_bypass = 0;
};

struct ssgpu_result {
  ssgpu_plan* plan = nullptr;
  std::vector<PinnedBuf> host_data, host_nulls;
  std::vector<bool> fetched;
  std::vector<ssgpu_dict*> concat_dicts;
  ~ssgpu_result() { for (ssgpu_dict* d : concat_dicts) if (d) ssgpu_dict_destroy(d); }
};

struct ssgpu_plan {
  ssgpu_ctx* ctx = nullptr;
  MemQuota quota;
  int64_t expr_row_capacity = INT64_MAX;
  PlanDesc desc;
  std::vector<Stage> stages;
  std::vector<StageExec> exec;
  Schema result_schema;
  std::vector<std::string> attr_names;
  std::vector<ssgpu_column> aux_cols;
  int64_t aux_rows = -1;
  std::string describe, describe_full;
  std::atomic<int> interrupted{0};
  int64_t n_runs = 0;
  bool specialize = false;
  bool cached_only = false;
  bool best_effort = false; int64_t be_cut = -1, be_capacity = 0, be_window = 0, be_base = 0, be_window_fail = 0;
  uint32_t group_capacity_hint = 0;
  bool lazy_feedback = false;
  bool background = false;
  int64_t background_min_rows = 0;
  hipEvent_t ev_begin = nullptr, ev_end = nullptr, ev_dom0 = nullptr, ev_dom1 = nullptr;
  static const int kEventRing = 256;
  hipEvent_t ring0[kEventRing] = {nullptr}, ring1[kEventRing] = {nullptr};
  uint64_t profiled_runs = 0;
  bool events_valid = false;
  ssgpu_counters counters{};
  std::vector<VmInstr> host_prog_scratch;
  bool partial_pending = false;
  int64_t last_rows = 0;
  bool deferred = false;
  bool nan_seen = false;
  const ssgpu_dict* dict = nullptr;
  std::vector<ssgpu_column> last_cols; int64_t last_base = 0; bool last_partial = false;
  std::vector<DevBuf> host_stage_data[2], host_stage_nulls[2];
  DevBuf host_states;
  struct HostStream {
    bool open = false; int rc = SSGPU_OK;
    int64_t chunk_rows = 0, fill = 0, pushed = 0, chunks = 0; int cur = 0;
    int kind = 1;
    std::vector<PinnedBuf> pin_data[2], pin_nulls[2];
    hipEvent_t uploaded[2] = {nullptr, nullptr}, consumed[2] = {nullptr, nullptr};
    bool in_flight[2] = {false, false};
    void drop_events() {
      for (int b = 0; b < 2; ++b) {
        if (uploaded[b]) (void)hipEventDestroy(uploaded[b]);
        if (consumed[b]) (void)hipEventDestroy(consumed[b]);
        uploaded[b] = consumed[b] = nullptr; in_flight[b] = false;
      }
    }
  } host_stream;
  struct StreamJob {
    int kind = 0;
    ssgpu_plan* head = nullptr; ssgpu_plan* tail = nullptr;
    std::vector<DevBuf> acc_data, acc_nulls;
    int64_t acc_rows = 0, acc_cap = 0;
    int64_t rows_hint = 0;
  };
  StreamJob* stream_job = nullptr;
  ssgpu_plan* skip_plan = nullptr;
  int64_t run_row_end = 0;
  bool keep_error_flags = false;
  ssgpu_result result;
};

struct ssgpu_block {
  ssgpu_ctx* ctx = nullptr;
  Schema schema;
  int64_t capacity = 0, rows = 0;
  DevBuf arena;
  std::vector<DevBuf> data, nulls;
  ssgpu_dict* dict = nullptr;
};
static const size_t kBlockColumnSkew = 512, kBlockArenaMin = 32u << 20;

static int fail(ssgpu_ctx* ctx, const Status& s) { if (ctx) ctx->err = s.msg; return s.code; }
static const Stage::ConcatCol* concat_of(const ssgpu_plan* p, int32_t col) {
  if (p->stages.empty()) return nullptr;
  for (auto& cc : p->stages.back().concat) if (cc.out_col == col) return &cc;
  return nullptr;
}

extern "C" {

int ssgpu_abi_version(void) { return SSGPU_ABI_VERSION; }

int ssgpu_ctx_create(int device_id, ssgpu_ctx** out) {
  if (!out) return SSGPU_ERROR_INVALID_ARGUMENT_VALUE;
  ssgpu_ctx* c = new ssgpu_ctx;
  c->device = device_id;
  if (device_id >= 0) {
    int n = 0;
    hipError_t e = hipGetDeviceCount(&n);
    if (e != hipSuccess || device_id >= n) { delete c; return SSGPU_ERROR_NO_DEVICE; }
    if (hipSetDevice(device_id) != hipSuccess) { delete c; return SSGPU_ERROR_NO_DEVICE; }
    hipDeviceProp_t prop;
    if (hipGetDeviceProperties(&prop, device_id) != hipSuccess) { delete c; return SSGPU_ERROR_NO_DEVICE; }
    c->cu_count = prop.multiProcessorCount;
    if (hipStreamCreateWithFlags(&c->stream, hipStreamNonBlocking) != hipSuccess ||
        hipStreamCreateWithFlags(&c->copy_stream, hipStreamNonBlocking) != hipSuccess) { delete c; return SSGPU_ERROR_HIP; }
    c->own_stream = true;
    g_device_contexts.fetch_add(1);
    (void)ssgpu_pipeline_set_max_lds(160 * 1024);
    (void)ssgpu_part_agg_set_max_lds(160 * 1024);
  }
  if (const char* e = getenv("SSGPU_SPECIALIZE")) c->specialize = atoi(e);
  if (const char* e = getenv("SSGPU_GROUP_DENSE")) c->group_dense = atoi(e);
  *out = c;
  return SSGPU_OK;
}

static void ctx_release(ssgpu_ctx* c) {
  if (c->refs.fetch_sub(1) != 1) return;
  if (c->device >= 0) {
    if (c->own_stream && c->stream) (void)hipStreamDestroy(c->stream);
    if (c->copy_stream) (void)hipStreamDestroy(c->copy_stream);
    if (c->copy_ev) { (void)hipEventDestroy(c->copy_ev); c->copy_ev = nullptr; }
    if (g_device_contexts.fetch_sub(1) == 1) (void)g_pool.trim(-1);
  }
  delete c;
}
int64_t ssgpu_pool_trim(int32_t device) { return (int64_t)g_pool.trim(device); }
void ssgpu_ctx_destroy(ssgpu_ctx* c) { if (c) ctx_release(c); }

int ssgpu_ctx_has_device(const ssgpu_ctx* c) { return c && c->device >= 0 ? 1 : 0; }
const char* ssgpu_last_error(const ssgpu_ctx* c) { return c ? c->err.c_str() : "null context"; }
void* ssgpu_ctx_stream(ssgpu_ctx* c) { return c ? (void*)c->stream : nullptr; }
void* ssgpu_ctx_copy_stream(ssgpu_ctx* c) { return c ? (void*)c->copy_stream : nullptr; }

int ssgpu_ctx_set_stream(ssgpu_ctx* c, void* s) {
  if (!c || c->device < 0) return SSGPU_ERROR_NO_DEVICE;
  if (c->own_stream && c->stream) (void)hipStreamDestroy(c->stream);
  c->stream = (hipStream_t)s; c->own_stream = false;
  return SSGPU_OK;
}

int ssgpu_ctx_synchronize(ssgpu_ctx* c) {
  if (!c || c->device < 0) return SSGPU_ERROR_NO_DEVICE;
  HIP_TRY(c, hipStreamSynchronize(c->stream));
  HIP_TRY(c, hipStreamSynchronize(c->copy_stream));
  return SSGPU_OK;
}

int ssgpu_ctx_set_option(ssgpu_ctx* c, const char* key, int64_t value) {
  if (!c || !key) return SSGPU_ERROR_INVALID_ARGUMENT_VALUE;
  std::string k(key);
  if (k == "tile_rows") {
    if (value != 0 && (value % VM_TILE_UNIT != 0 || value > 4 * VM_TILE_UNIT)) { c->err = "tile_rows must be 0 or 1, 2, 4 times the workgroup's row-pair count"; return SSGPU_ERROR_INVALID_ARGUMENT_VALUE; }
    c->opt.tile_rows = (int)value;
  } else if (k == "lds_target_bytes") c->opt.lds_target_bytes = (int)value;
  else if (k == "grid_limit") c->grid_limit = value;
  else if (k == "wgs_per_cu") c->wgs_per_cu = value > 0 ? value : 3;
  else if (k == "tile_map") c->tile_map = value;
  else if (k == "out_arena") c->out_arena = value;
  else if (k == "group_local") c->group_local = value;
  else if (k == "group_partition") c->group_partition = value;
  else if (k == "part_n") c->part_n = value;
  else if (k == "part_wgs_per_cu") c->part_wgs_per_cu = value;
  else if (k == "part_lds_target") c->part_lds_target = value;
  else if (k == "part_agg_lds") c->part_agg_lds = value;
  else if (k == "group_slab") c->group_slab = value;
  else if (k == "group_resident") c->group_resident = value;
  else if (k == "group_dense") c->group_dense = value;
  else if (k == "dense_parts") c->dense_parts = value;
  else if (k == "dense_min_rows") c->dense_min_rows = value;
  else if (k == "group_scout") c->group_scout = value;
  else if (k == "group_scout_rows") c->group_scout_rows = value;
  else if (k == "part_plain") c->part_plain = value;
  else if (k == "pscat_threads") c->pscat_threads = value;
  else if (k == "pscat_rows") c->pscat_rows = value;
  else if (k == "pscat_wgs") c->pscat_wgs = value;
  else if (k == "pscat_pipe") c->pscat_pipe = value;
  else if (k == "fuse_emit") c->fuse_emit = value;
  else if (k == "part_prefetch") c->part_prefetch = value;
  else if (k == "lazy_feedback") c->lazy_feedback = value;
  else if (k == "async_handoff") c->async_handoff = value;
  else if (k == "sort_records") c->sort_records = value;
  else if (k == "sort_hybrid") c->sort_hybrid = value;
  else if (k == "sort_hi_digits") c->sort_hi_digits = value;
  else if (k == "sort_compact") c->sort_compact = value;
  else if (k == "group_capacity") {
    int64_t cap = 1; while (cap < value) cap <<= 1;
    c->group_capacity = cap;
  } else if (k == "profile") c->profile = value;
  else if (k == "profile_total") c->profile_total = value;
  else if (k == "debug_timing") c->debug_timing = value;
  else if (k == "specialize") c->specialize = value;
  else if (k == "specialize_min_rows") c->specialize_min_rows = value < 0 ? 0 : value;
  else { c->err = "unknown option " + k; return SSGPU_ERROR_INVALID_ARGUMENT_VALUE; }
  return SSGPU_OK;
}

int ssgpu_host_alloc(ssgpu_ctx* c, size_t bytes, void** out) {
  if (!c || c->device < 0) return SSGPU_ERROR_NO_DEVICE;
  HIP_TRY(c, hipHostMalloc(out, std::max<size_t>(bytes, 1), hipHostMallocDefault));
  return SSGPU_OK;
}
void ssgpu_host_free(ssgpu_ctx* c, void* p) { (void)c; if (p) (void)hipHostFree(p); }

int ssgpu_block_create(ssgpu_ctx* c, const ssgpu_attr* schema, int32_t n, int64_t cap, ssgpu_block** out) {
  if (!c || c->device < 0) return SSGPU_ERROR_NO_DEVICE;
  ssgpu_block* b = new ssgpu_block;
  b->ctx = c; b->capacity = cap; b->rows = 0;
  b->data.resize(n); b->nulls.resize(n);
  size_t total = 0;
  for (int i = 0; i < n; ++i) {
    Attr a; a.name = schema[i].name ? schema[i].name : ""; a.dtype = schema[i].dtype; a.nullable = schema[i].nullable != 0;
    int w = dtype_width(a.dtype);
    if (w == 0) { delete b; c->err = "variable-length columns are outside the device hot path"; return SSGPU_ERROR_NOT_IMPLEMENTED; }
    b->schema.push_back(a);
    total += (size_t)cap * w + (a.nullable ? (size_t)cap : 0);
  }
  if (total >= kBlockArenaMin) {
    auto pitch = [](size_t bytes) { return ((bytes + (2u << 20) - 1) / (2u << 20)) * (2u << 20) + kBlockColumnSkew; };
    size_t need = 0;
    for (int i = 0; i < n; ++i) need += pitch((size_t)cap * dtype_width(b->schema[i].dtype)) + (b->schema[i].nullable ? pitch((size_t)cap) : 0);
    if (b->arena.ensure(need) != hipSuccess) { delete b; c->err = "device allocation failed"; return SSGPU_ERROR_MEMORY_EXCEEDED; }
    size_t off = 0;
    for (int i = 0; i < n; ++i) { const size_t bytes = (size_t)cap * dtype_width(b->schema[i].dtype); b->data[i].set_view(b->arena.as<char>() + off, bytes); off += pitch(bytes); }
    for (int i = 0; i < n; ++i) if (b->schema[i].nullable) { b->nulls[i].set_view(b->arena.as<char>() + off, (size_t)cap); off += pitch((size_t)cap); }
  } else {
    for (int i = 0; i < n; ++i) {
      if (b->data[i].ensure((size_t)cap * dtype_width(b->schema[i].dtype)) != hipSuccess) { delete b; c->err = "device allocation failed"; return SSGPU_ERROR_MEMORY_EXCEEDED; }
      if (b->schema[i].nullable && b->nulls[i].ensure((size_t)cap) != hipSuccess) { delete b; c->err = "device allocation failed"; return SSGPU_ERROR_MEMORY_EXCEEDED; }
    }
  }
  c->refs.fetch_add(1);
  g_live_blocks.fetch_add(1);
  *out = b;
  return SSGPU_OK;
}
void ssgpu_block_destroy(ssgpu_block* b) { if (!b) return; ssgpu_ctx* c = b->ctx; ssgpu_dict_destroy(b->dict); delete b; g_live_blocks.fetch_sub(1); if (c) ctx_release(c); }

static const int64_t kFileChunkRows = 8192;

static bool read_slab(FILE* f, char* dst, size_t bytes) {
  const long pos = ftell(f);
  const int fd = fileno(f);
  const int kReaders = bytes >= (8u << 20) ? 4 : 1;
  const size_t part = (bytes + kReaders - 1) / kReaders;
  std::atomic<bool> ok{true};
  auto read_part = [&](int i) {
    size_t lo = (size_t)i * part, hi = std::min(bytes, lo + part);
    while (lo < hi) {
      const ssize_t got = pread(fd, dst + lo, hi - lo, (off_t)(pos + (long)lo));
      if (got <= 0) { ok = false; return; }
      lo += (size_t)got;
    }
  };
  std::vector<std::thread> readers;
  for (int i = 1; i < kReaders; ++i) readers.emplace_back(read_part, i);
  read_part(0);
  for (auto& t : readers) t.join();
  return ok && fseek(f, pos + (long)bytes, SEEK_SET) == 0;
}

static const int64_t kMaxStringDomain = int64_t(1) << 30;
static int encode_string_domain(ssgpu_ctx* c, ssgpu_block* b, const std::vector<int>& scols, DevBuf& heap, DevBuf& lens, DevBuf& dnull) {
  hipStream_t s = c->copy_stream;
  const uint64_t rows = (uint64_t)b->rows, n = rows * scols.size();
  std::vector<uint64_t> off_h(1, 0);
  std::vector<char> heap_h;
  uint32_t D = 0;
  if (n) {
    uint64_t cap = 64, np2 = 1;
    while (cap < 2 * n) cap <<= 1;
    while (np2 < n) np2 <<= 1;
    DevBuf partials, hashes, table, row_slot, flags, d_slot, d_off, d_len, d_key, d_idx, slot_rank, out_off, out_heap;
    const bool alloc_ok =
        partials.ensure(ssgpu_str_scan_partials(n) * 8) == hipSuccess && hashes.ensure(n * 8) == hipSuccess && table.ensure(cap * 8) == hipSuccess &&
        row_slot.ensure(n * 4) == hipSuccess && flags.ensure(8) == hipSuccess && d_slot.ensure(n * 4) == hipSuccess && d_off.ensure(n * 8) == hipSuccess &&
        d_len.ensure(n * 8) == hipSuccess && d_key.ensure(np2 * 8) == hipSuccess && d_idx.ensure(np2 * 4) == hipSuccess &&
        slot_rank.ensure(cap * 4) == hipSuccess && out_off.ensure((n + 1) * 8) == hipSuccess;
    if (!alloc_ok) { c->err = "Memory exceeded: the STRING dictionary's device tables"; return SSGPU_ERROR_MEMORY_EXCEEDED; }
    const uint8_t* bytes = heap.as<uint8_t>();
    const uint64_t* offs = lens.as<uint64_t>();
    HIP_TRY(c, ssgpu_launch_str_scan(lens.as<uint64_t>(), n, partials.as<uint64_t>(), s));
    HIP_TRY(c, ssgpu_launch_str_hash(bytes, offs, dnull.as<uint8_t>(), n, hashes.as<uint64_t>(), s));
    HIP_TRY(c, hipMemsetAsync(table.p, 0, cap * 8, s));
    HIP_TRY(c, hipMemsetAsync(flags.p, 0, 8, s));
    HIP_TRY(c, ssgpu_launch_str_insert(bytes, offs, dnull.as<uint8_t>(), hashes.as<uint64_t>(), n, table.as<uint64_t>(), cap, row_slot.as<uint32_t>(),
                                       flags.as<uint32_t>() + 1, s));
    HIP_TRY(c, ssgpu_launch_str_compact(table.as<uint64_t>(), cap, bytes, offs, flags.as<uint32_t>(), d_slot.as<uint32_t>(), d_off.as<uint64_t>(),
                                        d_len.as<uint64_t>(), d_key.as<uint64_t>(), d_idx.as<uint32_t>(), s));
    uint32_t fl[2] = {0, 0};
    HIP_TRY(c, hipMemcpyAsync(fl, flags.p, 8, hipMemcpyDeviceToHost, s));
    HIP_TRY(c, hipStreamSynchronize(s));
    if (fl[1]) { c->err = "STRING dictionary: hash table overflow"; return SSGPU_ERROR_UNKNOWN; }
    D = fl[0];
    uint64_t p2 = 1;
    while (p2 < D) p2 <<= 1;
    HIP_TRY(c, ssgpu_launch_str_sort(d_key.as<uint64_t>(), d_idx.as<uint32_t>(), D, D ? p2 : 0, bytes, d_off.as<uint64_t>(), d_len.as<uint64_t>(), s));
    HIP_TRY(c, ssgpu_launch_str_rank(d_idx.as<uint32_t>(), d_slot.as<uint32_t>(), d_len.as<uint64_t>(), D, slot_rank.as<int32_t>(), out_off.as<uint64_t>(), s));
    HIP_TRY(c, ssgpu_launch_str_scan(out_off.as<uint64_t>(), D, partials.as<uint64_t>(), s));
    for (size_t k = 0; k < scols.size(); ++k)
      HIP_TRY(c, ssgpu_launch_str_codes(row_slot.as<uint32_t>() + k * rows, dnull.as<uint8_t>() + k * rows, slot_rank.as<int32_t>(), rows,
                                        b->data[scols[k]].as<int32_t>(), s));
    off_h.resize((size_t)D + 1);
    HIP_TRY(c, hipMemcpyAsync(off_h.data(), out_off.p, ((size_t)D + 1) * 8, hipMemcpyDeviceToHost, s));
    HIP_TRY(c, hipStreamSynchronize(s));
    if (out_heap.ensure(std::max<uint64_t>(off_h[D], 1)) != hipSuccess) { c->err = "Memory exceeded: the STRING dictionary's values"; return SSGPU_ERROR_MEMORY_EXCEEDED; }
    HIP_TRY(c, ssgpu_launch_str_gather(bytes, d_off.as<uint64_t>(), d_idx.as<uint32_t>(), out_off.as<uint64_t>(), D, out_heap.as<uint8_t>(), s));
    heap_h.resize((size_t)off_h[D]);
    if (off_h[D]) HIP_TRY(c, hipMemcpyAsync(heap_h.data(), out_heap.p, (size_t)off_h[D], hipMemcpyDeviceToHost, s));
    HIP_TRY(c, hipStreamSynchronize(s));
  }
  ssgpu_dict* d = nullptr;
  const int rc = ssgpu_dict_create_sorted(heap_h.data(), off_h.data(), (int64_t)D, &d);
  if (rc != SSGPU_OK) { c->err = "STRING dictionary: too many distinct values"; return rc; }
  ssgpu_dict_destroy(b->dict);
  b->dict = d;
  return SSGPU_OK;
}

int ssgpu_block_create_from_file(ssgpu_ctx* c, const ssgpu_attr* schema, int32_t n, const char* path, ssgpu_block** out) {
  if (!c || c->device < 0) return SSGPU_ERROR_NO_DEVICE;
  FILE* f = path ? fopen(path, "rb") : nullptr;
  if (!f) { c->err = std::string("cannot open ") + (path ? path : "(null)"); return SSGPU_ERROR_INVALID_ARGUMENT_VALUE; }
  std::vector<int> width(n); std::vector<bool> nullable(n), is_str(n);
  std::vector<int> scols;
  for (int i = 0; i < n; ++i) {
    width[i] = dtype_width(schema[i].dtype); nullable[i] = schema[i].nullable != 0; is_str[i] = schema[i].dtype == SSGPU_STRING;
    if (width[i] == 0) { fclose(f); c->err = "variable-length columns of the file format are outside the device hot path"; return SSGPU_ERROR_NOT_IMPLEMENTED; }
    if (is_str[i]) scols.push_back(i);
  }
  const size_t ns = scols.size();
// ... 523 lines not shown

int attach_pc_profile(ssgpu_ctx* c, StageExec& ex, VmParams* P) {
  if (c->debug_timing < 2) return SSGPU_OK;
  HIP_TRY(c, ex.debug_pc.ensure((size_t)(P->n_instr + 1) * 8));
  HIP_TRY(c, hipMemsetAsync(ex.debug_pc.p, 0, (size_t)(P->n_instr + 1) * 8, c->stream));
  P->debug_pc = ex.debug_pc.as<unsigned long long>();
  P->debug_pc_lds_off = (P->lds_bytes + 7u) & ~7u;
  P->lds_bytes = P->debug_pc_lds_off + (uint32_t)(P->n_instr + 1) * 8u;
  return SSGPU_OK;
}
int print_pc_profile(ssgpu_ctx* c, StageExec& ex, const Program& prog, int n_instr) {
  if (c->debug_timing < 2) return SSGPU_OK;
  std::vector<unsigned long long> cyc((size_t)n_instr + 1);
  HIP_TRY(c, hipStreamSynchronize(c->stream));
  HIP_TRY(c, hipMemcpy(cyc.data(), ex.debug_pc.p, cyc.size() * 8, hipMemcpyDeviceToHost));
  double tot = 0; for (auto v : cyc) tot += (double)v;
  fprintf(stderr, "[ssgpu pc-profile] staging+wait %5.1f%%\n", 100.0 * (double)cyc[n_instr] / tot);
  for (int pc = 0; pc < n_instr && pc < (int)prog.code.size(); ++pc)
    fprintf(stderr, "[ssgpu pc-profile] %3d %-22s %5.1f%%\n", pc, vm_op_name(prog.code[pc].op), 100.0 * (double)cyc[pc] / tot);
  return SSGPU_OK;
}

int grid_for(ssgpu_ctx* c, const ProgramLayout& L, int n_tiles) {
  int per_cu = (int)std::min<uint32_t>((uint32_t)c->wgs_per_cu, (160u * 1024u) / std::max<uint32_t>(L.lds_bytes, 1));
  if (per_cu < 1) per_cu = 1;
  int64_t g = (int64_t)c->cu_count * per_cu;
  if (c->grid_limit > 0) g = std::min<int64_t>(g, c->grid_limit);
  g = std::min<int64_t>(g, std::max(1, n_tiles));
  return (int)std::max<int64_t>(g, 1);
}

static hipError_t launch_main(ssgpu_plan* p, const Stage& st, StageExec& ex, const VmParams& P, int K, int grid) {
  ssgpu_ctx* c = p->ctx;
  if (p->specialize && !P.debug_pc) {
    void* h = rtc_for(p, ex, ex.rtc_main, st.main, ex.lay, ex.host_prog_main, ex.n_instr_main, P.lds_bytes, "");
    if (h) return ssgpu_launch_pipeline_rtc(h, P, grid, ex.rtc_main.static_lds != 0, c->stream);
  }
  return ssgpu_launch_pipeline(P, K, grid, c->stream);
}

void fill_params(VmParams* P, const Program& prog, const ProgramLayout& L, const DevBuf& dev_prog, int n_instr,
                 const InCols& in, int64_t row_id_base) {
  memset(P, 0, sizeof(*P));
  P->prog = dev_prog.as<const VmInstr>();
  P->n_instr = n_instr;
  P->n_staged = (int)prog.staged.size();
  P->n_outputs = prog.n_outputs;
  P->uses_math = prog.uses_math ? 1u : 0u;
  P->n_slots = prog.n_slots;
  P->n_rows = in.rows;
  P->n_rows_dev = in.rows_dev;
  P->row_id_base = row_id_base;
  P->tile_rows = VM_TILE_UNIT * L.K;
  P->n_tiles = (int)((in.rows + P->tile_rows - 1) / P->tile_rows);
  P->acc_lds_off = L.acc_off;
  P->scratch_lds_off = L.scratch_off;
  P->imm_pool_lds_off = L.imm_pool_off;
  P->const_lds_off = L.imm_pool_off + 16u * (uint32_t)prog.code.size();
  P->lds_bytes = L.lds_bytes;
  for (size_t i = 0; i < prog.staged.size(); ++i) {
    const StagedInput& s = prog.staged[i];
    P->staged[i].src = s.is_null_mask ? (const void*)in.cols[s.col].is_null : in.cols[s.col].data;
    P->staged[i].lds_off = prog.regs[s.reg].row_off * (uint32_t)P->tile_rows;
    P->staged[i].width = prog.regs[s.reg].width;
  }
}

int ensure_out_cols(ssgpu_ctx* c, const Stage& st, StageExec& ex, int64_t rows) {
  ex.out.resize(st.out_schema.size());
  size_t total = 0;
  for (size_t i = 0; i < st.out_schema.size(); ++i) {
    OutCol& oc = ex.out[i];
    oc.width = (uint32_t)dtype_width(st.out_schema[i].dtype);
    oc.nullable = st.out_schema[i].nullable;
    total += (size_t)std::max<int64_t>(rows, 1) * (oc.width + (oc.nullable ? 1u : 0u));
  }
  if (c->out_arena && total >= kBlockArenaMin && st.out_schema.size() > 1) {
    auto pitch = [](size_t bytes) { return ((bytes + (2u << 20) - 1) / (2u << 20)) * (2u << 20) + kBlockColumnSkew; };
    bool fits = ex.out_arena.p != nullptr;
    for (size_t i = 0; i < ex.out.size() && fits; ++i)
      fits = ex.out[i].data.view && ex.out[i].data.cap >= (size_t)std::max<int64_t>(rows, 1) * ex.out[i].width + 16 &&
             (!ex.out[i].nullable || (ex.out[i].nulls.view && ex.out[i].nulls.cap >= (size_t)std::max<int64_t>(rows, 1) + 16));
    if (!fits) {
      size_t need = 0;
      for (auto& oc : ex.out) need += pitch((size_t)rows * oc.width + 16) + (oc.nullable ? pitch((size_t)rows + 16) : 0);
      for (auto& oc : ex.out) { oc.data.release(); oc.nulls.release(); }
      ex.out_arena.release();
      HIP_TRY(c, ex.out_arena.ensure(need));
      size_t off = 0;
      for (auto& oc : ex.out) { const size_t bytes = (size_t)rows * oc.width + 16; oc.data.set_view(ex.out_arena.as<char>() + off, bytes); off += pitch(bytes); }
      for (auto& oc : ex.out) if (oc.nullable) { oc.nulls.set_view(ex.out_arena.as<char>() + off, (size_t)rows + 16); off += pitch((size_t)rows + 16); }
    }
    ex.out_capacity = rows;
    return SSGPU_OK;
  }
  for (size_t i = 0; i < st.out_schema.size(); ++i) {
    OutCol& oc = ex.out[i];
    if (oc.data.view) oc.data.release();
    if (oc.nulls.view) oc.nulls.release();
    HIP_TRY(c, oc.data.ensure((size_t)std::max<int64_t>(rows, 1) * oc.width + 16));
    if (oc.nullable) HIP_TRY(c, oc.nulls.ensure((size_t)std::max<int64_t>(rows, 1) + 16));
  }
  ex.out_capacity = rows;
  return SSGPU_OK;
}

void fill_fast_slots(VmParams* P, const Stage& st) {
  for (size_t i = 0; i < st.aggs.size() && i < VM_FAST_SLOTS; ++i) {
    const int kind = st.aggs[i].slot == (int)i ? st.aggs[i].slot_kind : SLOT_COUNT;
    uint64_t i0 = 0, i1 = 0;
    const double pinf = __builtin_inf(), ninf = -__builtin_inf(), nzero = -0.0;
    switch (kind) {
      case SLOT_SUM_DD: memcpy(&i0, &nzero, 8); break;
      case SLOT_MIN_U64: i0 = ~0ull; break;
      case SLOT_MIN_F64: memcpy(&i0, &pinf, 8); break;
      case SLOT_MAX_F64: memcpy(&i0, &ninf, 8); break;
      case SLOT_FIRST: i1 = ~0ull; break;
      default: break;
    }
    P->slot_init0[i] = i0; P->slot_init1[i] = i1; P->slot_kind[i] = kind;
  }
}

int distinct_flags(ssgpu_ctx* c, const Stage& st, StageExec& ex, const InCols& in, ssgpu_column* out) {
  const uint32_t nk = (uint32_t)st.distinct_cols.size();
  if (nk > 16) { c->err = "DISTINCT aggregate under more than 15 group keys"; return SSGPU_ERROR_NOT_IMPLEMENTED; }
  const void* kdata[16] = {nullptr}; const uint8_t* knulls[16] = {nullptr}; uint32_t kwidth[16] = {0};
  for (uint32_t k = 0; k < nk; ++k) {
    const int col = st.distinct_cols[k];
    kdata[k] = in.cols[col].data; knulls[k] = in.cols[col].is_null; kwidth[k] = (uint32_t)dtype_width(st.in_schema[col].dtype);
  }
  HIP_TRY(c, ex.dflag.ensure((size_t)std::max<int64_t>(in.rows, 1)));
  HIP_TRY(c, ssgpu_launch_cluster_flags(kdata, knulls, kwidth, nk, (uint64_t)in.rows, ex.dflag.as<uint8_t>(), c->stream));
  out->data = ex.dflag.p; out->is_null = nullptr;
  return SSGPU_OK;
}

int prepare_scalar_emit(ssgpu_plan* p, size_t si, int* n_out);
int run_scalar_agg(ssgpu_plan* p, size_t si, const InCols& in0, int64_t row_id_base, bool stop_at_partial) {
  ssgpu_ctx* c = p->ctx; Stage& st = p->stages[si]; StageExec& ex = p->exec[si];
  InCols in = in0;
  if (!st.distinct_cols.empty()) {
    ssgpu_column f; const int rc = distinct_flags(c, st, ex, in0, &f); if (rc != SSGPU_OK) return rc;
    in.cols.push_back(f);
  }
  VmParams P;
  fill_params(&P, st.main, ex.lay, ex.prog_main, ex.n_instr_main, in, row_id_base);
  apply_joins(p, ex, st.main, &P);
  if (c->tile_map >= 2) P.flags |= VM_FLAG_XCD_CHUNKS;
  fill_fast_slots(&P, st);
  const int grid = grid_for(c, ex.lay, P.n_tiles);
  ex.grid = grid;
  const int ns = st.main.n_slots;
  HIP_TRY(c, ex.wg_partials.ensure((size_t)grid * ns * VM_WAVES * sizeof(VmAccRec)));
  HIP_TRY(c, ex.slot_recs.ensure((size_t)ns * sizeof(VmAccRec)));
  HIP_TRY(c, ex.state.ensure((size_t)ns * SSGPU_STATE_ARRAYS * sizeof(uint64_t)));
  if (!ex.slot_kind.p) {
    std::vector<int> kinds((size_t)ns, SLOT_COUNT);
    for (size_t i = 0; i < st.aggs.size(); ++i)
      if (st.aggs[i].slot == (int)i) kinds[i] = st.aggs[i].slot_kind;
    HIP_TRY(c, ex.slot_kind.ensure(kinds.size() * sizeof(int)));
    HIP_TRY(c, hipMemcpy(ex.slot_kind.p, kinds.data(), kinds.size() * sizeof(int), hipMemcpyHostToDevice));
  }
  P.wg_partials = ex.wg_partials.as<VmAccRec>();
  P.error_flag = ex.error_flag.as<unsigned int>();
  if (c->debug_timing) {
    HIP_TRY(c, ex.debug.ensure((size_t)grid * 4 * 8));
    P.debug = ex.debug.as<unsigned long long>();
  }
  { int rc = attach_pc_profile(c, ex, &P); if (rc != SSGPU_OK) return rc; }
  if (c->profile) HIP_TRY(c, hipEventRecord(p->ev_dom0, c->stream));
  HIP_TRY(c, launch_main(p, st, ex, P, ex.lay.K, grid));
  if (c->profile) HIP_TRY(c, hipEventRecord(p->ev_dom1, c->stream));
  { int rc = print_pc_profile(c, ex, st.main, P.n_instr); if (rc != SSGPU_OK) return rc; }
  int n_emit = 0;
  ex.emitted_with_finish = false;
  if (!stop_at_partial && c->fuse_emit) { const int rc = prepare_scalar_emit(p, si, &n_emit); if (rc != SSGPU_OK) return rc; ex.emitted_with_finish = true; }
  HIP_TRY(c, ssgpu_launch_finish_slots(ex.wg_partials.as<VmAccRec>(), ns, grid * VM_WAVES, ex.slot_kind.as<int>(),
                                       ex.slot_recs.as<VmAccRec>(), stop_at_partial ? ex.state.as<uint64_t>() : nullptr, c->stream,
                                       ex.emitted_with_finish ? ex.emit_descs.as<EmitDesc>() : nullptr, n_emit));
  p->counters.n_launches += 2;
  p->counters.tile_rows = P.tile_rows; p->counters.grid = grid; p->counters.lds_bytes = (int32_t)ex.lay.lds_bytes;
  if (c->debug_timing) {
    std::vector<unsigned long long> dbg((size_t)grid * 4);
    HIP_TRY(c, hipMemcpy(dbg.data(), ex.debug.p, dbg.size() * 8, hipMemcpyDeviceToHost));
    double tot = 0, wait = 0, tiles = 0;
    for (int g = 0; g < grid; ++g) { tot += (double)dbg[g * 4]; wait += (double)dbg[g * 4 + 1]; tiles += (double)dbg[g * 4 + 2]; }
    fprintf(stderr, "[ssgpu debug] grid=%d tiles/wg=%.1f cycles/wg=%.0f wait=%.1f%% cycles/tile=%.0f (wait %.0f)\n", grid, tiles / grid,
            tot / grid, 100.0 * wait / tot, tot / tiles, wait / tiles);
  }
  return SSGPU_OK;
}

static const int64_t kSeqSumPiece = 1 << 21;
static int run_seq_sums(ssgpu_plan* p, Stage& st, StageExec& ex, const InCols& in, const uint32_t* seg_id) {
  ssgpu_ctx* c = p->ctx;
  auto kind_of = [](int dtype) {
    switch (dtype) {
      case SSGPU_INT32: return 0; case SSGPU_UINT32: return 1; case SSGPU_INT64: return 2; case SSGPU_UINT64: return 3;
      case SSGPU_FLOAT: return 4; default: return 5;
    }
  };
  for (auto& q : st.seq_sums) {
    const void* src = in.cols[q.in_col].data;
    const uint8_t* src_nulls = st.in_schema[q.in_col].nullable ? in.cols[q.in_col].is_null : nullptr;
    uint8_t* dst_nulls = ex.out[q.out_col].nullable ? ex.out[q.out_col].nulls.as<uint8_t>() : nullptr;
    const int sk = kind_of(st.in_schema[q.in_col].dtype), dk = kind_of(st.out_schema[q.out_col].dtype);
    if (seg_id || in.rows <= kSeqSumPiece) {
      HIP_TRY(c, ssgpu_launch_seq_sum(src, src_nulls, sk, seg_id, (uint64_t)in.rows, ex.out[q.out_col].data.p, dst_nulls, dk, c->stream));
      p->counters.n_launches += 1;
      continue;
    }
    HIP_TRY(c, ex.total2.ensure(16));
    for (int64_t first = 0; first < in.rows; first += kSeqSumPiece) {
      const int64_t end = std::min<int64_t>(in.rows, first + kSeqSumPiece);
      HIP_TRY(c, ssgpu_launch_seq_sum(src, src_nulls, sk, nullptr, (uint64_t)end, ex.out[q.out_col].data.p, dst_nulls, dk, c->stream,
                                      (uint64_t)first, ex.total2.as<uint64_t>(), first > 0 ? 1 : 0));
      p->counters.n_launches += 1;
      if (end < in.rows) {
        HIP_TRY(c, hipStreamSynchronize(c->stream));
        if (p->interrupted.exchange(0)) { c->err = "interrupted"; return SSGPU_INTERRUPTED; }
      }
    }
  }
  return SSGPU_OK;
}

int prepare_scalar_emit(ssgpu_plan* p, size_t si, int* n_out) {
  ssgpu_ctx* c = p->ctx; Stage& st = p->stages[si]; StageExec& ex = p->exec[si];
  int rc = ensure_out_cols(c, st, ex, 1);
  if (rc != SSGPU_OK) return rc;
  *n_out = (int)st.aggs.size();
  if (!ex.emit_ready) {
    std::vector<EmitDesc> descs;
    for (size_t i = 0; i < st.aggs.size(); ++i) {
      EmitDesc d; d.data = ex.out[i].data.p; d.is_null = ex.out[i].nullable ? ex.out[i].nulls.as<uint8_t>() : nullptr;
      d.slot = st.aggs[i].slot; d.out_kind = st.aggs[i].emit_kind;
      descs.push_back(d);
    }
    HIP_TRY(c, ex.emit_descs.ensure(std::max<size_t>(descs.size(), 1) * sizeof(EmitDesc)));
    HIP_TRY(c, hipMemcpy(ex.emit_descs.p, descs.data(), descs.size() * sizeof(EmitDesc), hipMemcpyHostToDevice));
    ex.emit_ready = true;
  }
  return SSGPU_OK;
}

int emit_scalar_agg(ssgpu_plan* p, size_t si) {
  ssgpu_ctx* c = p->ctx; StageExec& ex = p->exec[si];
  int n_out = 0;
  const int rc = prepare_scalar_emit(p, si, &n_out);
  if (rc != SSGPU_OK) return rc;
  if (ex.emitted_with_finish) { ex.emitted_with_finish = false; ex.out_rows = 1; return SSGPU_OK; }
  HIP_TRY(c, ssgpu_launch_emit_scalar(ex.slot_recs.as<VmAccRec>(), ex.emit_descs.as<EmitDesc>(), n_out, c->stream));
  p->counters.n_launches += 1;
  ex.out_rows = 1;
  return SSGPU_OK;
}

int segment_ids(ssgpu_ctx* c, const Stage& st, StageExec& ex, const InCols& in, ssgpu_column* out) {
  const uint32_t nk = (uint32_t)st.segment_cols.size();
  if (nk > 16) { c->err = "AggregateClusters with more than 16 keys"; return SSGPU_ERROR_NOT_IMPLEMENTED; }
  const void* kdata[16] = {nullptr}; const uint8_t* knulls[16] = {nullptr}; uint32_t kwidth[16] = {0};
  void* okdata[16] = {nullptr}; uint8_t* oknulls[16] = {nullptr};
  for (uint32_t k = 0; k < nk; ++k) {
    const int col = st.segment_cols[k];
    kdata[k] = in.cols[col].data; knulls[k] = st.in_schema[col].nullable ? in.cols[col].is_null : nullptr; kwidth[k] = (uint32_t)dtype_width(st.in_schema[col].dtype);
  }
  const uint64_t n = (uint64_t)in.rows;
  const int ntile = (int)((n + 511) / 512);
  HIP_TRY(c, ex.seg_counts.ensure((size_t)std::max(ntile, 1) * 4)); HIP_TRY(c, ex.seg_offsets.ensure((size_t)std::max(ntile, 1) * 4));
  HIP_TRY(c, ex.seg_total.ensure(8)); HIP_TRY(c, ex.seg_id.ensure(std::max<uint64_t>(n, 1) * 4));
  HIP_TRY(c, hipMemsetAsync(ex.seg_total.p, 0, 8, c->stream));
  HIP_TRY(c, ssgpu_launch_cluster_count(kdata, knulls, kwidth, nk, n, ex.seg_counts.as<uint32_t>(), c->stream));
  HIP_TRY(c, ssgpu_launch_scan_counts(ex.seg_counts.as<uint32_t>(), ex.seg_offsets.as<uint32_t>(), ntile, ex.seg_total.as<uint64_t>(), c->stream));
  HIP_TRY(c, ssgpu_launch_cluster_assign(kdata, knulls, kwidth, nk, okdata, oknulls, n, ex.seg_offsets.as<uint32_t>(), ex.seg_id.as<uint32_t>(), c->stream));
  out->data = ex.seg_id.p; out->is_null = nullptr;
  return SSGPU_OK;
}

int rank_columns(ssgpu_plan* p, const Stage& st, StageExec& ex, const InCols& in, ssgpu_column* rank_out, ssgpu_column* own_out) {
  ssgpu_ctx* c = p->ctx;
  if (p->run_row_end >= (1ll << 32) - 1) { c->err = "DISTINCT / CONCAT aggregates under max_unique_keys_in_result: row ids beyond 2^32"; return SSGPU_ERROR_NOT_IMPLEMENTED; }
  ssgpu_column seg;
  int rc = segment_ids(c, st, ex, in, &seg);
  if (rc != SSGPU_OK) return rc;
  const uint64_t n = (uint64_t)in.rows;
  uint64_t n_seg = 0;
  HIP_TRY(c, hipMemcpyAsync(&n_seg, ex.seg_total.p, 8, hipMemcpyDeviceToHost, c->stream));
  HIP_TRY(c, hipStreamSynchronize(c->stream));
  HIP_TRY(c, ex.rank_first.ensure(std::max<uint64_t>(n_seg, 1) * 4)); HIP_TRY(c, ex.rank_of_seg.ensure(std::max<uint64_t>(n_seg, 1) * 4));
  HIP_TRY(c, ex.rank_row.ensure(std::max<uint64_t>(n, 1) * 4)); HIP_TRY(c, ex.rank_own.ensure(std::max<uint64_t>(n, 1)));
  HIP_TRY(c, ssgpu_launch_seg_first(ex.seg_id.as<uint32_t>(), (const uint64_t*)in.cols[st.rank_rowid_col].data, n, ex.rank_first.as<uint32_t>(), c->stream));
  uint32_t* sorted = nullptr;
  rc = sort_rows_by_u32(p, ex, ex.rank_first.as<uint32_t>(), n_seg, &sorted);
  if (rc != SSGPU_OK) return rc;
  HIP_TRY(c, ssgpu_launch_rank_scatter(sorted, n_seg, ex.rank_of_seg.as<uint32_t>(), c->stream));
  HIP_TRY(c, ssgpu_launch_rank_rows(ex.seg_id.as<uint32_t>(), ex.rank_of_seg.as<uint32_t>(), n, (uint32_t)std::min<int64_t>(st.rank_limit, 0xFFFFFFFFll), ex.rank_row.as<uint32_t>(),
                                    ex.rank_own.as<uint8_t>(), c->stream));
  p->counters.n_launches += 3;
  rank_out->data = ex.rank_row.p; rank_out->is_null = nullptr;
  own_out->data = ex.rank_own.p; own_out->is_null = nullptr;
  return SSGPU_OK;
}

int run_materialize(ssgpu_plan* p, size_t si, const InCols& in0, int64_t row_id_base) {
  ssgpu_ctx* c = p->ctx; Stage& st = p->stages[si]; StageExec& ex = p->exec[si];
  int rc = ensure_out_cols(c, st, ex, in0.rows);
  if (rc != SSGPU_OK) return rc;
  ex.out_rows_dev = nullptr;
  InCols in = in0;
  if (!st.distinct_cols.empty()) {
    ssgpu_column f; rc = distinct_flags(c, st, ex, in0, &f); if (rc != SSGPU_OK) return rc;
    in.cols.push_back(f);
  }
  if (st.has_segment) {
    ssgpu_column f; rc = segment_ids(c, st, ex, in0, &f); if (rc != SSGPU_OK) return rc;
    in.cols.push_back(f);
  }
  if (st.has_rank) {
    ssgpu_column r, o; rc = rank_columns(p, st, ex, in0, &r, &o); if (rc != SSGPU_OK) return rc;
    in.cols.push_back(r); in.cols.push_back(o);
  }
  VmParams P;
  fill_params(&P, st.main, ex.lay, ex.prog_main, ex.n_instr_main, in, row_id_base);
  apply_joins(p, ex, st.main, &P);
  P.error_flag = ex.error_flag.as<unsigned int>();
  if (c->tile_map >= 1) P.flags |= VM_FLAG_XCD_CHUNKS;
  int oi = 0;
  for (size_t i = 0; i < ex.out.size(); ++i) {
    P.outputs[oi].dst = ex.out[i].data.p; P.outputs[oi].width = ex.out[i].width; ++oi;
    if (ex.out[i].nullable) { P.outputs[oi].dst = ex.out[i].nulls.p; P.outputs[oi].width = 1; ++oi; }
  }
  rc = attach_pc_profile(c, ex, &P);
  if (rc != SSGPU_OK) return rc;
  const int grid = grid_for(c, ex.lay, P.n_tiles);
  ex.grid = grid;
  p->counters.tile_rows = P.tile_rows; p->counters.grid = grid; p->counters.lds_bytes = (int32_t)ex.lay.lds_bytes;
  bool dom0_recorded = false;
  if (st.has_filter) {
    const int nt = std::max(P.n_tiles, 1);
    HIP_TRY(c, ex.tile_counts.ensure((size_t)nt * sizeof(uint32_t)));
    HIP_TRY(c, ex.tile_offsets.ensure((size_t)nt * sizeof(uint32_t)));
    HIP_TRY(c, ex.total.ensure(16));
    if (c->profile) { HIP_TRY(c, hipEventRecord(p->ev_dom0, c->stream)); dom0_recorded = true; }
    VmParams C;
    fill_params(&C, st.count_pass, ex.lay_count, ex.prog_count, ex.n_instr_count, in, row_id_base);
    apply_joins(p, ex, st.count_pass, &C);
    C.tile_counts = ex.tile_counts.as<unsigned int>();
    C.count_sub_k = ex.lay.K;
    if (c->tile_map >= 2) C.flags |= VM_FLAG_XCD_CHUNKS;
    C.error_flag = P.error_flag;
    const int cgrid = grid_for(c, ex.lay_count, C.n_tiles);
    HIP_TRY(c, ssgpu_launch_pipeline(C, ex.lay_count.K, cgrid, c->stream));
    HIP_TRY(c, ssgpu_launch_scan_counts(ex.tile_counts.as<uint32_t>(), ex.tile_offsets.as<uint32_t>(), P.n_tiles,
                                        ex.total.as<uint64_t>(), c->stream));
    P.tile_offsets = ex.tile_offsets.as<unsigned int>();
    p->counters.n_launches += 2;
    ex.out_rows = -1;
  } else if (in.rows_dev) {
    ex.out_rows = -1; ex.out_rows_dev = in.rows_dev;
  } else {
    ex.out_rows = in.rows;
  }
  if (c->profile && !dom0_recorded) HIP_TRY(c, hipEventRecord(p->ev_dom0, c->stream));
  HIP_TRY(c, launch_main(p, st, ex, P, ex.lay.K, grid));
  if (c->profile) HIP_TRY(c, hipEventRecord(p->ev_dom1, c->stream));
  p->counters.n_launches += 1;
  return print_pc_profile(c, ex, st.main, ex.n_instr_main);
}

static int gather_first_last(ssgpu_plan* p, Stage& st, StageExec& ex, size_t nk, const InCols& in, int64_t row_id_base,
                             const uint64_t* n_rows_dev, uint64_t n_rows_max) {
  ssgpu_ctx* c = p->ctx;
  for (size_t j = 0; j < st.aggs.size(); ++j) {
    const int col = st.aggs[j].gather_col;
    if (col < 0) continue;
    auto kind_of = [](int dtype) {
      switch (dtype) {
        case SSGPU_INT32: case SSGPU_DATE: case SSGPU_STRING: return 0; case SSGPU_UINT32: return 1;
        case SSGPU_INT64: case SSGPU_DATETIME: return 2; case SSGPU_UINT64: return 3;
        case SSGPU_FLOAT: return 4; case SSGPU_DOUBLE: return 5; default: return 6;
      }
    };
    HIP_TRY(c, ssgpu_launch_gather_rowid(ex.out[nk + j].data.p, ex.out[nk + j].nullable ? ex.out[nk + j].nulls.as<uint8_t>() : nullptr,
                                         in.cols[col].data, ex.out[nk + j].width, kind_of(st.in_schema[col].dtype), kind_of(st.out_schema[nk + j].dtype),
                                         ex.rowid_tmp[j].as<uint64_t>(), st.aggs[j].gather_low32 ? 0xFFFFFFFFull : ~0ull, row_id_base,
                                         n_rows_dev, n_rows_max, c->stream));
    p->counters.n_launches += 1;
  }
  return SSGPU_OK;
}
static int ensure_rowid_tmp(ssgpu_ctx* c, Stage& st, StageExec& ex, uint64_t rows) {
  ex.rowid_tmp.resize(st.aggs.size());
  for (size_t j = 0; j < st.aggs.size(); ++j)
    if (st.aggs[j].gather_col >= 0) HIP_TRY(c, ex.rowid_tmp[j].ensure(std::max<uint64_t>(rows, 1) * 8));
  return SSGPU_OK;
}

int extract_groups(ssgpu_plan* p, Stage& st, StageExec& ex, uint32_t capacity, uint32_t ng, const InCols& in, int64_t row_id_base, uint32_t extra_slots = 0) {
  ssgpu_ctx* c = p->ctx;
  const size_t slots = (size_t)capacity + 1 + extra_slots;
  const int ntile = (int)((slots + 511) / 512);
  int rc = ensure_out_cols(c, st, ex, (int64_t)slots);
  if (rc != SSGPU_OK) return rc;
  HIP_TRY(c, ex.total.ensure(16));
// ... 962 lines not shown
    std::vector<uint64_t> pattern(ng, 0);
    for (size_t i = 0; i < st.group_acc_init.size(); ++i) pattern[i] = st.group_acc_init[i];
    HIP_TRY(c, hipMemcpy(ex.gpattern.p, pattern.data(), ng * 8, hipMemcpyHostToDevice));
    ex.pattern_ready = true;
  }
  HIP_TRY(c, ssgpu_launch_fill_pattern_u64(ex.gacc.as<uint64_t>(), ex.gpattern.as<uint64_t>(), ng, slots * ng, c->stream));
  HIP_TRY(c, hipMemsetAsync(ex.gcnt.p, 0, slots * ng * 4, c->stream));
  HIP_TRY(c, hipMemsetAsync(ex.error_flag.p, 0, 4, c->stream));
  InCols ext = in;
  ssgpu_column segcol; segcol.data = ex.seg_id.p; segcol.is_null = nullptr;
  ext.cols.push_back(segcol);
  if (!st.distinct_cols.empty()) {
    ssgpu_column f; const int frc = distinct_flags(c, st, ex, in, &f); if (frc != SSGPU_OK) return frc;
    ext.cols.push_back(f);
  }
  VmParams P;
  fill_params(&P, st.main, ex.lay, ex.prog_main, ex.n_instr_main, ext, row_id_base);
  apply_joins(p, ex, st.main, &P);
  P.error_flag = ex.error_flag.as<unsigned int>();
  P.group.acc = ex.gacc.as<unsigned long long>();
  P.group.cnt = ex.gcnt.as<unsigned int>();
  const int grid = grid_for(c, ex.lay, P.n_tiles);
  if (c->profile) HIP_TRY(c, hipEventRecord(p->ev_dom0, c->stream));
  HIP_TRY(c, launch_main(p, st, ex, P, ex.lay.K, grid));
  if (c->profile) HIP_TRY(c, hipEventRecord(p->ev_dom1, c->stream));
  rc = ensure_rowid_tmp(c, st, ex, nseg);
  if (rc != SSGPU_OK) return rc;
  std::vector<GroupAggOut> outs(st.aggs.size());
  for (size_t j = 0; j < st.aggs.size(); ++j) {
    outs[j].data = st.aggs[j].gather_col >= 0 ? ex.rowid_tmp[j].p : ex.out[nk + j].data.p;
    outs[j].is_null = ex.out[nk + j].nullable ? ex.out[nk + j].nulls.as<uint8_t>() : nullptr;
    outs[j].s = st.aggs[j].slot; outs[j].out_kind = st.aggs[j].emit_kind; outs[j].has_cnt = st.aggs[j].has_cnt ? 1 : 0;
  }
  HIP_TRY(c, ssgpu_launch_dense_extract(ex.gacc.as<uint64_t>(), ex.gcnt.as<uint32_t>(), ng, nseg, outs.data(), (uint32_t)outs.size(), c->stream));
  rc = gather_first_last(p, st, ex, nk, in, row_id_base, nullptr, nseg);
  if (rc == SSGPU_OK && !st.seq_sums.empty()) rc = run_seq_sums(p, st, ex, in, ex.seg_id.as<uint32_t>());
  if (rc != SSGPU_OK) return rc;
  p->counters.n_launches += 6;
  ex.out_rows = (int64_t)nseg;
  return SSGPU_OK;
}

int run_join_expand(ssgpu_plan* p, size_t si, const InCols& in) {
  ssgpu_ctx* c = p->ctx; Stage& st = p->stages[si]; StageExec& ex = p->exec[si];
  if (si == 0 || p->exec[si - 1].jrows_sorted.empty()) { c->err = "join expansion without its index"; return SSGPU_ERROR_UNKNOWN; }
  StageExec& bx = p->exec[si - 1];
  const size_t join_id = bx.jrows_sorted.size() - 1;
  const uint64_t n = (uint64_t)in.rows;
  const size_t n_in = in.cols.size();
  const uint32_t* run_start = static_cast<const uint32_t*>(in.cols[n_in - 2].data);
  const uint32_t* run_count = static_cast<const uint32_t*>(in.cols[n_in - 1].data);
  HIP_TRY(c, ex.jx_offsets.ensure(std::max<uint64_t>(n, 1) * 4)); HIP_TRY(c, ex.total.ensure(8));
  HIP_TRY(c, hipMemsetAsync(ex.total.p, 0, 8, c->stream));
  uint64_t n_out = 0;
  if (n > 0) {
    if (n >= (1ull << 31)) { c->err = "hash join: more than 2^31 lhs rows per GPU is not supported yet"; return SSGPU_ERROR_NOT_IMPLEMENTED; }
    HIP_TRY(c, ssgpu_launch_scan_counts(run_count, ex.jx_offsets.as<uint32_t>(), (int)n, ex.total.as<uint64_t>(), c->stream));
    HIP_TRY(c, hipMemcpyAsync(&n_out, ex.total.p, 8, hipMemcpyDeviceToHost, c->stream));
    HIP_TRY(c, hipStreamSynchronize(c->stream));
  }
  if (n_out >= (uint64_t)VM_NONE) { c->err = "hash join: the result has more than 2^32 rows"; return SSGPU_ERROR_MEMORY_EXCEEDED; }
  int rc = ensure_out_cols(c, st, ex, (int64_t)n_out);
  if (rc != SSGPU_OK) return rc;
  HIP_TRY(c, ex.jx_lhs_idx.ensure(std::max<uint64_t>(n_out, 1) * 4)); HIP_TRY(c, ex.jx_rhs_row.ensure(std::max<uint64_t>(n_out, 1) * 4));
  if (c->profile) HIP_TRY(c, hipEventRecord(p->ev_dom0, c->stream));
  HIP_TRY(c, ssgpu_launch_join_expand(ex.jx_offsets.as<uint32_t>(), run_start, bx.jrows_sorted[join_id].as<uint32_t>(), n, n_out,
                                      ex.jx_lhs_idx.as<uint32_t>(), ex.jx_rhs_row.as<uint32_t>(), c->stream));
  for (size_t q = 0; q < st.join_out.size(); ++q) {
    const Stage::JoinOut& f = st.join_out[q];
    const void* src; const uint8_t* src_null; const uint32_t* idx;
    if (f.from_rhs) {
      src = p->aux_cols[f.col].data; src_null = p->desc.aux_schema[f.col].nullable ? p->aux_cols[f.col].is_null : nullptr;
      idx = ex.jx_rhs_row.as<uint32_t>();
    } else {
      src = in.cols[f.col].data; src_null = in.cols[f.col].is_null; idx = ex.jx_lhs_idx.as<uint32_t>();
    }
    HIP_TRY(c, ssgpu_launch_sort_gather(ex.out[q].data.p, ex.out[q].nullable ? ex.out[q].nulls.as<uint8_t>() : nullptr, src, src_null,
                                        ex.out[q].width, idx, n_out, c->stream));
  }
  if (c->profile) HIP_TRY(c, hipEventRecord(p->ev_dom1, c->stream));
  p->counters.n_launches += 2 + (int)st.join_out.size();
  ex.out_rows = (int64_t)n_out;
  return SSGPU_OK;
}

int run_fold_tail(ssgpu_plan* p, size_t si, const InCols& in) {
  ssgpu_ctx* c = p->ctx; Stage& st = p->stages[si]; StageExec& ex = p->exec[si];
  if (st.fold_cut) {
    const int64_t keep = std::min<int64_t>(in.rows, p->be_capacity);
    int rc = ensure_out_cols(c, st, ex, keep);
    if (rc != SSGPU_OK) return rc;
    if (c->profile) HIP_TRY(c, hipEventRecord(p->ev_dom0, c->stream));
    for (size_t i = 0; i < st.out_schema.size() && keep > 0; ++i) {
      HIP_TRY(c, hipMemcpyAsync(ex.out[i].data.p, in.cols[i].data, (size_t)keep * ex.out[i].width, hipMemcpyDeviceToDevice, c->stream));
      if (ex.out[i].nullable) {
        if (st.in_schema[i].nullable && in.cols[i].is_null) HIP_TRY(c, hipMemcpyAsync(ex.out[i].nulls.p, in.cols[i].is_null, (size_t)keep, hipMemcpyDeviceToDevice, c->stream));
        else HIP_TRY(c, hipMemsetAsync(ex.out[i].nulls.p, 0, (size_t)keep, c->stream));
      }
    }
    if (c->profile) HIP_TRY(c, hipEventRecord(p->ev_dom1, c->stream));
    p->be_cut = -1;
    if (in.rows > keep) {
      unsigned long long next = 0;
      HIP_TRY(c, hipMemcpyAsync(&next, static_cast<const unsigned long long*>(in.cols[st.in_schema.size() - 1].data) + keep, 8, hipMemcpyDeviceToHost, c->stream));
      HIP_TRY(c, hipStreamSynchronize(c->stream));
      p->be_cut = (int64_t)next + p->be_base;
    }
    ex.out_rows = keep;
    return SSGPU_OK;
  }
  const int64_t keep = std::min<int64_t>(in.rows, st.fold_limit + 1);
  int rc = ensure_out_cols(c, st, ex, keep);
  if (rc != SSGPU_OK) return rc;
  auto kind_of = [](int dtype) {
    switch (dtype) {
      case SSGPU_INT32: case SSGPU_DATE: case SSGPU_STRING: return 0u; case SSGPU_UINT32: return 1u;
      case SSGPU_INT64: case SSGPU_DATETIME: return 2u; case SSGPU_UINT64: return 3u;
      case SSGPU_FLOAT: return 4u; case SSGPU_DOUBLE: return 5u; default: return 6u;
    }
  };
  std::vector<FoldTailColumn> cols(st.out_schema.size());
  for (size_t i = 0; i < cols.size(); ++i) {
    cols[i].src = in.cols[i].data; cols[i].src_nulls = st.in_schema[i].nullable ? in.cols[i].is_null : nullptr;
    cols[i].dst = ex.out[i].data.p; cols[i].dst_nulls = ex.out[i].nullable ? ex.out[i].nulls.as<uint8_t>() : nullptr;
    cols[i].op = (unsigned)st.fold_op[i]; cols[i].kind = kind_of(st.out_schema[i].dtype);
    const int by = i < st.fold_by.size() ? st.fold_by[i] : -1;
    cols[i].by = by >= 0 ? (const unsigned long long*)in.cols[by].data : nullptr;
    cols[i].by_nulls = by >= 0 && st.in_schema[by].nullable ? in.cols[by].is_null : nullptr;
  }
  HIP_TRY(c, ex.emit_descs.ensure(std::max<size_t>(cols.size(), 1) * sizeof(FoldTailColumn)));
  HIP_TRY(c, hipMemcpyAsync(ex.emit_descs.p, cols.data(), cols.size() * sizeof(FoldTailColumn), hipMemcpyHostToDevice, c->stream));
  HIP_TRY(c, hipStreamSynchronize(c->stream));
  if (c->profile) HIP_TRY(c, hipEventRecord(p->ev_dom0, c->stream));
  HIP_TRY(c, ssgpu_launch_fold_tail(ex.emit_descs.as<FoldTailColumn>(), (unsigned)cols.size(), (unsigned long long)in.rows, (unsigned long long)st.fold_limit, c->stream));
  if (c->profile) HIP_TRY(c, hipEventRecord(p->ev_dom1, c->stream));
  p->counters.n_launches += 1;
  ex.out_rows = keep;
  return SSGPU_OK;
}

static const void* rows_word(const StageExec& ex) { return ex.out_rows_dev ? ex.out_rows_dev : ex.total.p; }
int stage_rows(ssgpu_plan* p, size_t si, int64_t* rows) {
  ssgpu_ctx* c = p->ctx; StageExec& ex = p->exec[si];
  if (ex.out_rows < 0) {
    uint64_t total = 0;
    HIP_TRY(c, hipMemcpyAsync(&total, rows_word(ex), 8, hipMemcpyDeviceToHost, c->stream));
    HIP_TRY(c, hipStreamSynchronize(c->stream));
    ex.out_rows = (int64_t)total;
  }
  *rows = ex.out_rows;
  return SSGPU_OK;
}

int check_error_flags(ssgpu_plan* p);

int check_error_flags(ssgpu_plan* p) {
  ssgpu_ctx* c = p->ctx;
  std::vector<uint32_t> flags(p->exec.size(), 0);
  for (size_t i = 0; i < p->exec.size(); ++i)
    if (p->exec[i].error_flag.p)
      HIP_TRY(c, hipMemcpyAsync(&flags[i], p->exec[i].error_flag.p, 4, hipMemcpyDeviceToHost, c->stream));
  HIP_TRY(c, hipStreamSynchronize(c->stream));
  for (uint32_t& f : flags) {
    if (f & SSGPU_FLAG_NAN_IN_MINMAX) p->nan_seen = true;
    f &= 0xFFu;
  }
  for (uint32_t f : flags) {
    if (f == 3) { c->err = "decoupled look-back: a tile waited for an earlier tile's row count for too long and gave up"; return SSGPU_ERROR_HIP; }
    if (f) {
      c->err = f == 2 ? "Evaluation error: invalid argument of a signaling math expression (negative input of SQRT)"
                      : "Evaluation error: division by zero in a signaling expression";
      return SSGPU_ERROR_EVALUATION_ERROR;
    }
  }
  return SSGPU_OK;
}

static int order_after_uploads(ssgpu_ctx* c) {
  if (!c->copy_pending.exchange(false, std::memory_order_acq_rel)) return SSGPU_OK;
  if (!c->copy_ev) HIP_TRY(c, hipEventCreateWithFlags(&c->copy_ev, hipEventDisableTiming));
  HIP_TRY(c, hipEventRecord(c->copy_ev, c->copy_stream));
  HIP_TRY(c, hipStreamWaitEvent(c->stream, c->copy_ev, 0));
  return SSGPU_OK;
}
int run_plan(ssgpu_plan* p, const ssgpu_column* cols, int32_t n_cols, int64_t rows, int64_t row_id_base, bool partial);

int settle_plan(ssgpu_plan* p) {
  if (!p->deferred) return SSGPU_OK;
  ssgpu_ctx* c = p->ctx;
  p->deferred = false;
  HIP_TRY(c, hipStreamSynchronize(c->stream));
  bool rerun = false;
  for (auto& ex : p->exec) {
    if (!ex.fb_pending) continue;
    const uint32_t* fb = static_cast<const uint32_t*>(ex.fb_host.p);
    const int kind = ex.fb_pending; ex.fb_pending = 0;
    if (fb[0] || (kind == 2 && (fb[1] || fb[3]))) { rerun = true; ex.steady = 0; }
    else if (kind == 1 && (uint64_t)fb[1] > 2ull * ex.steady_bypass + (uint64_t)(p->last_rows >> 6)) ex.steady = 0;
  }
  if (!rerun) return SSGPU_OK;
  std::vector<ssgpu_column> cols = p->last_cols;
  return run_plan(p, cols.data(), (int32_t)cols.size(), p->last_rows, p->last_base, p->last_partial);
}

int fix_nan_minmax(ssgpu_plan* p) {
  if (!p->nan_seen) return SSGPU_OK;
  p->nan_seen = false;
  if (p->desc.nan_exact || p->partial_pending) return SSGPU_OK;
  ssgpu_ctx* c = p->ctx;
  p->desc.nan_exact = true;
  std::vector<Stage> stages; Schema schema; std::string describe;
  Status s = lower_plan(p->desc, &stages, &schema, &describe);
  if (!s.ok()) { p->desc.nan_exact = false; return SSGPU_OK; }
  HIP_TRY(c, hipStreamSynchronize(c->stream));
  for (auto& ex : p->exec) { ex.rtc_main.drop(); ex.rtc_pscatter.drop(); ex.rtc_plain.drop(); ex.rtc_part.drop(); ex.rtc_resident.drop(); ex.rtc_hot.drop(); }
  for (auto& ex : p->exec) if (ex.fb_event) { (void)hipEventDestroy(ex.fb_event); ex.fb_event = nullptr; g_events.fetch_sub(1); }
  p->exec.clear();
  p->stages = stages; p->describe = describe;
  p->exec.resize(p->stages.size());
  std::vector<ssgpu_column> cols = p->last_cols;
  int rc = run_plan(p, cols.data(), (int32_t)cols.size(), p->last_rows, p->last_base, false);
  if (rc != SSGPU_OK) return rc;
  rc = settle_plan(p);
  if (rc != SSGPU_OK) return rc;
  rc = check_error_flags(p);
  p->nan_seen = false;
  return rc;
}

int run_plan(ssgpu_plan* p, const ssgpu_column* cols, int32_t n_cols, int64_t rows, int64_t row_id_base, bool partial) {
  ssgpu_ctx* c = p->ctx;
  if (!c || c->device < 0) { if (c) c->err = "no gfx950 device bound to this context (bind-only context)"; return SSGPU_ERROR_NO_DEVICE; }
  ssgpu_rtc_mode(!p->cached_only ? 0 : p->background && rows >= p->background_min_rows ? 2 : 1);
  p->run_row_end = row_id_base + rows;
  p->nan_seen = false;
  if (p->deferred) {
    p->deferred = false;
    for (auto& ex : p->exec) {
      if (!ex.fb_pending) continue;
      if (ex.fb_event) HIP_TRY(c, hipEventSynchronize(ex.fb_event)); else HIP_TRY(c, hipStreamSynchronize(c->stream));
      const uint32_t* fb = static_cast<const uint32_t*>(ex.fb_host.p);
      const int kind = ex.fb_pending; ex.fb_pending = 0;
      if (fb[0] || (kind == 2 && (fb[1] || fb[3]))) ex.steady = 0;
      else if (kind == 1 && (uint64_t)fb[1] > 2ull * ex.steady_bypass + (uint64_t)(p->last_rows >> 6)) ex.steady = 0;
    }
  }
  if (n_cols != (int)p->desc.input_schema.size()) { c->err = "column count does not match the plan's input schema"; return SSGPU_ERROR_ATTRIBUTE_COUNT_MISMATCH; }
  if (rows < 0) { c->err = "negative row count"; return SSGPU_ERROR_INVALID_ARGUMENT_VALUE; }
  if (p->interrupted.exchange(0)) { c->err = "interrupted"; return SSGPU_INTERRUPTED; }
  QuotaScope quota_scope(&p->quota);
  HIP_TRY(c, hipSetDevice(c->device));
  { const int orc = order_after_uploads(c); if (orc != SSGPU_OK) return orc; }
  memset(&p->counters, 0, sizeof(p->counters));
  p->counters.rows_in = rows;
  p->result.fetched.assign(p->result.fetched.size(), false);
  for (ssgpu_dict*& cd : p->result.concat_dicts) { if (cd) ssgpu_dict_destroy(cd); cd = nullptr; }
  InCols in; in.cols.assign(cols, cols + n_cols); in.rows = rows;
  if (partial && !(p->stages.size() == 1 && p->stages[0].kind == STAGE_SCALAR_AGG)) {
    c->err = "partial runs need a plan whose only stage is a ScalarAggregate"; return SSGPU_ERROR_NOT_IMPLEMENTED;
  }
  for (size_t si = 0; si < p->stages.size(); ++si) {
    if (si == 0) ++p->n_runs;
    int rc = prepare_stage(p, si);
    if (rc != SSGPU_OK) return rc;
  }
  if (c->profile) {
    const int slot = (int)(p->profiled_runs % ssgpu_plan::kEventRing);
    if (!p->ring0[slot]) { HIP_TRY(c, hipEventCreate(&p->ring0[slot])); HIP_TRY(c, hipEventCreate(&p->ring1[slot])); g_events.fetch_add(2); }
    p->ev_dom0 = p->ring0[slot]; p->ev_dom1 = p->ring1[slot];
    ++p->profiled_runs;
    p->events_valid = false;
    if (c->profile_total) HIP_TRY(c, hipEventRecord(p->ev_begin, c->stream));
  }
  for (size_t si = 0; si < p->exec.size(); ++si)
    if (p->exec[si].error_flag.p && !p->keep_error_flags && !(si == 0 && p->stages[si].kind == STAGE_GROUP_AGG)) HIP_TRY(c, hipMemsetAsync(p->exec[si].error_flag.p, 0, sizeof(uint32_t), c->stream));
  int64_t alg_bytes = 0;
  for (size_t si = 0; si < p->stages.size(); ++si) {
    if (p->interrupted.exchange(0)) { c->err = "interrupted"; return SSGPU_INTERRUPTED; }
    Stage& st = p->stages[si];
    int rc = SSGPU_OK;
    alg_bytes += st.algorithmic_bytes_per_row * in.rows;
    rc = build_joins(p, st, p->exec[si]);
    if (rc != SSGPU_OK) return rc;
    switch (st.kind) {
      case STAGE_SCALAR_AGG:
        rc = run_scalar_agg(p, si, in, row_id_base, partial);
        if (rc == SSGPU_OK && !partial) rc = emit_scalar_agg(p, si);
        if (rc == SSGPU_OK && !partial && !st.seq_sums.empty()) rc = run_seq_sums(p, st, p->exec[si], in, nullptr);
        break;
      case STAGE_MATERIALIZE: rc = run_materialize(p, si, in, row_id_base); break;
      case STAGE_GROUP_AGG: rc = run_group_agg(p, si, in, row_id_base); break;
      case STAGE_SORT: rc = run_sort(p, si, in); break;
      case STAGE_CLUSTERS: rc = run_clusters(p, si, in, row_id_base); break;
      case STAGE_JOIN_EXPAND: rc = run_join_expand(p, si, in); break;
      case STAGE_FOLD_TAIL: rc = run_fold_tail(p, si, in); break;
      default: c->err = "stage kind not executable yet"; rc = SSGPU_ERROR_NOT_IMPLEMENTED; break;
    }
    if (rc != SSGPU_OK) return rc;
    if (si + 1 < p->stages.size()) {
      StageExec& ex = p->exec[si];
      const Stage& nx = p->stages[si + 1];
      const bool device_rows = c->async_handoff != 0 && !c->debug_timing && ex.out_rows < 0 && ex.out_capacity > 0 && nx.kind == STAGE_MATERIALIZE &&
                               !nx.has_filter && nx.distinct_cols.empty() && !nx.has_segment && !nx.has_rank && nx.joins.empty();
      int64_t r = 0;
      in.rows_dev = nullptr;
      if (device_rows) {
        r = ex.out_capacity;
        in.rows_dev = static_cast<const unsigned long long*>(rows_word(ex));
      } else {
        rc = stage_rows(p, si, &r);
        if (rc != SSGPU_OK) return rc;
        rc = check_error_flags(p);
        if (rc != SSGPU_OK) return rc;
      }
      in.cols.clear();
      for (auto& oc : ex.out) { ssgpu_column col; col.data = oc.data.p; col.is_null = oc.nullable ? oc.nulls.as<uint8_t>() : nullptr; in.cols.push_back(col); }
      in.rows = r;
      row_id_base = 0;
    }
  }
  if (c->profile && c->profile_total) { HIP_TRY(c, hipEventRecord(p->ev_end, c->stream)); p->events_valid = true; }
  p->counters.algorithmic_bytes = alg_bytes;
  p->last_rows = rows;
  p->last_cols.assign(cols, cols + n_cols); p->last_base = row_id_base; p->last_partial = partial;
  p->partial_pending = partial;
  return SSGPU_OK;
}

}

extern "C" {

int ssgpu_plan_run(ssgpu_plan* p, const ssgpu_column* cols, int32_t n_cols, int64_t rows, ssgpu_result** out) {
  if (!p) return SSGPU_ERROR_INVALID_ARGUMENT_VALUE;
  int rc = run_plan(p, cols, n_cols, rows, 0, false);
  if (rc != SSGPU_OK) return rc;
  if (!p->lazy_feedback) {
    rc = settle_plan(p);
    if (rc != SSGPU_OK) return rc;
    (void)check_error_flags(p);
    rc = fix_nan_minmax(p);
    if (rc != SSGPU_OK) return rc;
  }
  if (out) *out = &p->result;
  return SSGPU_OK;
}

int ssgpu_plan_run_best_effort(ssgpu_plan* p, const ssgpu_column* cols, int32_t n_cols, int64_t rows, int64_t start_row, int64_t* next_row, ssgpu_result** out) {
  if (!p || !next_row) return SSGPU_ERROR_INVALID_ARGUMENT_VALUE;
  ssgpu_ctx* c = p->ctx;
  if (!p->best_effort) { if (c) c->err = "ssgpu_plan_run_best_effort needs a plan whose root is a BestEffortGroupAggregate"; return SSGPU_ERROR_INVALID_ARGUMENT_VALUE; }
  if (n_cols != (int)p->desc.input_schema.size()) { c->err = "column count does not match the plan's input schema"; return SSGPU_ERROR_ATTRIBUTE_COUNT_MISMATCH; }
  if (start_row < 0 || start_row > rows) { c->err = "start_row outside the input"; return SSGPU_ERROR_INVALID_ARGUMENT_VALUE; }
  std::vector<ssgpu_column> win((size_t)n_cols);
  auto window = [&](int64_t s) {
    for (int i = 0; i < n_cols; ++i) {
      const size_t w = (size_t)dtype_width(p->desc.input_schema[i].dtype);
      win[i].data = cols[i].data ? static_cast<const char*>(cols[i].data) + (size_t)s * w : nullptr;
      win[i].is_null = cols[i].is_null ? cols[i].is_null + s : nullptr;
    }
  };
  auto run_range = [&](int64_t s, int64_t n) -> int {
    window(s);
    p->be_base = s;
    int rc = run_plan(p, win.data(), n_cols, n, 0, false);
    if (rc != SSGPU_OK) return rc;
    rc = settle_plan(p);
    if (rc != SSGPU_OK) return rc;
    rc = check_error_flags(p);
    if (rc != SSGPU_OK) return rc;
    return fix_nan_minmax(p);
  };
  const int64_t left = rows - start_row;
  int64_t W = p->be_window > 0 ? p->be_window : std::max<int64_t>(1 << 16, p->be_capacity < (INT64_MAX >> 4) ? p->be_capacity * 8 : INT64_MAX);
  for (;;) {
    W = std::max<int64_t>(1, std::min(W, left));
    if (left == 0) W = 0;
    int rc = run_range(start_row, W);
    if (rc == SSGPU_ERROR_MEMORY_EXCEEDED && W > 1) {
      p->be_window_fail = W;
      W = std::max<int64_t>(1, W / 2); p->be_window = W; p->be_capacity = std::min(p->be_capacity, W);
      HIP_TRY(c, hipStreamSynchronize(c->stream));
      for (auto& ex : p->exec) { ex.rtc_main.drop(); ex.rtc_pscatter.drop(); ex.rtc_plain.drop(); ex.rtc_part.drop(); ex.rtc_resident.drop(); ex.rtc_hot.drop(); }
      for (auto& ex : p->exec) if (ex.fb_event) { (void)hipEventDestroy(ex.fb_event); ex.fb_event = nullptr; g_events.fetch_sub(1); }
      p->exec.clear(); p->exec.resize(p->stages.size());
      p->deferred = false;
      { uint32_t cap = 1024; while ((int64_t)cap < 4 * W && cap < (1u << 30)) cap *= 2; p->group_capacity_hint = cap; }
      continue;
    }
    if (rc != SSGPU_OK) return rc;
    if (p->be_cut >= 0) {
      const int64_t end = p->be_cut;
      if (end <= start_row || end > start_row + W) { c->err = "best-effort cut outside the window"; return SSGPU_ERROR_HIP; }
      rc = run_range(start_row, end - start_row);
      if (rc != SSGPU_OK) return rc;
      if (p->be_cut >= 0) { c->err = "best-effort run over its own cut still overflows"; return SSGPU_ERROR_HIP; }
      *next_row = end;
      break;
    }
    if (W >= left) { *next_row = rows; break; }
    int64_t wider = W > (INT64_MAX >> 2) ? INT64_MAX : W * 4;
    if (p->be_window_fail > 0 && wider >= p->be_window_fail) wider = std::max(W, p->be_window_fail / 2);
    if (wider <= W) { *next_row = start_row + W; break; }
    W = wider; p->be_window = W;
  }
  if (out) *out = &p->result;
  return SSGPU_OK;
}

int32_t ssgpu_plan_specialized(const ssgpu_plan* p) {
  if (!p) return 0;
  int32_t n = 0;
  for (auto& ex : p->exec) n += (ex.rtc_main.h ? 1 : 0) + (ex.rtc_pscatter.h ? 1 : 0) + (ex.rtc_plain.h ? 1 : 0) + (ex.rtc_part.h ? 1 : 0) + (ex.rtc_resident.h ? 1 : 0) + (ex.rtc_hot.h ? 1 : 0);
  return n;
}
const char* ssgpu_plan_specialize_reason(const ssgpu_plan* p) {
  if (!p) return "";
  for (auto& ex : p->exec) {
    if (ex.rtc_why.empty()) continue;
    if (ex.rtc_why.find("being compiled") != std::string::npos && !(ex.rtc_main.pending || ex.rtc_pscatter.pending || ex.rtc_plain.pending || ex.rtc_part.pending ||
                                                                    ex.rtc_resident.pending || ex.rtc_hot.pending)) continue;
    return ex.rtc_why.c_str();
  }
  return "";
}
int ssgpu_plan_specialize(ssgpu_plan* p) {
  if (!p) return SSGPU_ERROR_INVALID_ARGUMENT_VALUE;
  ssgpu_ctx* c = p->ctx;
  if (!c || c->device < 0) { if (c) c->err = "no gfx950 device bound to this context (bind-only context)"; return SSGPU_ERROR_NO_DEVICE; }
  HIP_TRY(c, hipSetDevice(c->device));
  p->specialize = true;
  if (p->cached_only) {
    p->cached_only = false; p->background = false;
    for (auto& ex : p->exec) {
      for (StageExec::RtcSlot* sl : {&ex.rtc_main, &ex.rtc_pscatter, &ex.rtc_plain, &ex.rtc_part, &ex.rtc_resident, &ex.rtc_hot}) if (!sl->h) sl->tried = false;
      ex.rtc_why.clear();
    }
  }
  ssgpu_rtc_cached_only(false);
  for (size_t si = 0; si < p->stages.size(); ++si) {
    const int rc = prepare_stage(p, si);
    if (rc != SSGPU_OK) return rc;
    Stage& st = p->stages[si]; StageExec& ex = p->exec[si];
    if (st.main.empty() || st.kind == STAGE_GROUP_AGG) continue;
    (void)rtc_for(p, ex, ex.rtc_main, st.main, ex.lay, ex.host_prog_main, ex.n_instr_main, ex.lay.lds_bytes, "");
  }
  return SSGPU_OK;
}
int32_t ssgpu_plan_stage_count(const ssgpu_plan* p) { return p ? (int32_t)p->stages.size() : 0; }
int ssgpu_plan_stage_info(const ssgpu_plan* p, int32_t stage, ssgpu_stage_info* out) {
  if (!p || !out || stage < 0 || stage >= (int32_t)p->stages.size()) return SSGPU_ERROR_INVALID_ARGUMENT_VALUE;
  const StageExec& ex = p->exec[stage];
  memset(out, 0, sizeof(*out));
  out->kind = (int32_t)p->stages[stage].kind;
  out->group_shape = ex.last_group_shape; out->part_n = (int32_t)ex.part_n; out->part_seg_growth = (int32_t)ex.part_seg_growth;
  out->group_wgs_per_cu = ex.group_wgs; out->reruns = ex.last_reruns;
  out->sort_passes = ex.last_sort_passes; out->sort_mode = ex.last_sort_mode;
  out->specialized = (ex.rtc_main.h ? 1 : 0) + (ex.rtc_pscatter.h ? 2 : 0) + (ex.rtc_part.h ? 4 : 0) + (ex.rtc_plain.h ? 8 : 0) + (ex.rtc_resident.h ? 16 : 0);
  out->plain_scatter = ex.last_plain_scatter ? 1 : 0;
  out->hot_keys = (int32_t)ex.hot_n;
  out->dense_slots = ex.dense.on ? (int32_t)ex.dense.slots : 0;
  return SSGPU_OK;
}
void ssgpu_specialized_kernels_trim(int32_t keep) { ssgpu_rtc_trim(keep); }
int ssgpu_memory_stats(ssgpu_memory_stats_t* out) {
// ... 1227 lines not shown
```

supersonic_amd/csrc/vm.h:

```cpp
#ifndef SSGPU_VM_H_
#define SSGPU_VM_H_

#ifdef __HIPCC_RTC__
typedef signed char int8_t; typedef unsigned char uint8_t; typedef short int16_t; typedef unsigned short uint16_t;
typedef int int32_t; typedef unsigned int uint32_t; typedef long int64_t; typedef unsigned long uint64_t; typedef unsigned long uintptr_t;
typedef int hipError_t; typedef struct ihipStream_t* hipStream_t;
#else
#include <stdint.h>
#endif

#define VM_NONE 0xFFFFFFFFu
enum { VM_MATH_EXP = 1, VM_MATH_LN, VM_MATH_LOG10, VM_MATH_LOG2, VM_MATH_SIN, VM_MATH_COS, VM_MATH_TAN, VM_MATH_ASIN, VM_MATH_ACOS,
       VM_MATH_ATAN, VM_MATH_SINH, VM_MATH_COSH, VM_MATH_TANH, VM_MATH_ASINH, VM_MATH_ACOSH, VM_MATH_ATANH, VM_MATH_POW, VM_MATH_ATAN2 };
#ifndef VM_THREADS
#define VM_THREADS 256
#endif
#ifndef VM_PF_UNITS
#define VM_PF_UNITS 8
#endif
#ifndef VM_WAVES_PER_EU
#define VM_WAVES_PER_EU 4
#endif
#ifndef VM_STAGE_PRIO
#define VM_STAGE_PRIO 1
// ... 55 lines not shown
  X(AND3) X(OR3)                                                               \
  X(NULL_OR)                                   \
  X(NULL_DIVZERO_32) X(NULL_DIVZERO_64) X(NULL_DIVZERO_F32) X(NULL_DIVZERO_F64)\
  X(FAIL_DIVZERO_32) X(FAIL_DIVZERO_64) X(FAIL_DIVZERO_F32) X(FAIL_DIVZERO_F64)\
  X(FILL_8) X(FILL_32) X(FILL_64) X(ROWID_64)                                  \
  \
  X(MATH1_F64) X(MATH2_F64)                                                    \
  X(SELECT_8) X(SELECT_32) X(SELECT_64)    \
  X(SEL_FROM_PRED)     \
  \
  X(AGG_COUNT)                                                                 \
  X(AGG_SUM_I32) X(AGG_SUM_U32) X(AGG_SUM_I64) X(AGG_SUM_F32) X(AGG_SUM_F64)   \
  X(AGG_MIN_I32) X(AGG_MIN_U32) X(AGG_MIN_I64) X(AGG_MIN_U64)                  \
  X(AGG_MIN_F32) X(AGG_MIN_F64) X(AGG_MIN_B8)                                  \
  X(AGG_MAX_I32) X(AGG_MAX_U32) X(AGG_MAX_I64) X(AGG_MAX_U64)                  \
  X(AGG_MAX_F32) X(AGG_MAX_F64) X(AGG_MAX_B8)                                  \
  X(AGG_FIRST_8) X(AGG_FIRST_32) X(AGG_FIRST_64)                               \
  X(AGG_LAST_8) X(AGG_LAST_32) X(AGG_LAST_64)                                  \
  \
  X(AGG_SUM_I64_ADD) X(AGG_SUM_I64_SUB) X(AGG_SUM_I64_MUL)                     \
  X(AGG_SUM_F64_ADD) X(AGG_SUM_F64_SUB) X(AGG_SUM_F64_MUL)                     \
  \
  X(SEL_COUNT)              \
  X(SEL_RANK) X(PART_RANK) X(PART_REC_8) X(PART_REC_32) X(PART_REC_64) X(PART_REC_128) X(PART_FLUSH) X(JOIN_PROBE) X(JOIN_PROBE_WIDE) X(IDX_VALID) X(GATHER_64) X(GATHER_32) X(GATHER_8) X(GATHER_NULL)              \
  X(STORE_8) X(STORE_32) X(STORE_64)     \
  X(STOREC_8) X(STOREC_32) X(STOREC_64)  \
  X(STORE_ROWID)     \
  \
  \
  \
  \
  \
  X(KEY_ZERO)                                                 \
  X(KEY_APPEND_8) X(KEY_APPEND_32) X(KEY_APPEND_64)                            \
                 \
                 \
  X(GRP_INSERT)                \
  X(GAGG_COUNT)                                                                \
  X(GAGG_SUM_I32) X(GAGG_SUM_U32) X(GAGG_SUM_I64) X(GAGG_SUM_F32) X(GAGG_SUM_F64)\
  X(GAGG_MIN_I32) X(GAGG_MIN_U32) X(GAGG_MIN_I64) X(GAGG_MIN_U64)              \
  X(GAGG_MIN_F32) X(GAGG_MIN_F64) X(GAGG_MIN_B8)                               \
  X(GAGG_MAX_I32) X(GAGG_MAX_U32) X(GAGG_MAX_I64) X(GAGG_MAX_U64)              \
  X(GAGG_MAX_F32) X(GAGG_MAX_F64) X(GAGG_MAX_B8)                               \
  X(GAGG_FIRST) X(GAGG_LAST)                                                   \
  X(OP_COUNT_)

enum VmOp : uint16_t {
#define X(n) VM_##n,
  VM_OPS(X)
#undef X
};

struct VmInstr {
  uint16_t op;
  uint8_t reg_ops;
  uint8_t imm_width;
  uint32_t dst;
  uint32_t a, b, c, d;
  uint64_t imm;
};
static_assert(sizeof(VmInstr) == 32, "VmInstr must be 32 bytes");

struct VmStagedCol {
  const void* src;
  uint32_t lds_off;
  uint32_t width;
};

struct VmOutCol {
  void* dst;
  uint32_t width;
  uint32_t pad;
};

struct VmAccRec {
  uint64_t v0;
  uint64_t v1;
  uint64_t cnt;
  uint64_t pad;
};

struct VmGroupTable {
  unsigned long long* keys;
  unsigned long long* acc;
  unsigned int* cnt;
  unsigned int* overflow;
  uint32_t capacity_mask;
  uint32_t local_capacity;
  uint32_t local_sub;
  uint32_t local_sub_capacity;
  uint32_t local_keys_off;
  uint32_t local_acc_off;
  uint32_t local_cnt_off;
  uint32_t local_stride;
  uint32_t local_pad;
  uint32_t n_gaggs;
  const unsigned long long* acc_init;
  const unsigned int* merge_op;
  unsigned int* stats;
};
#define VM_MERGE_ADD_U64 0u
#define VM_MERGE_MIN_U64 1u
#define VM_MERGE_MAX_U64 2u
#define VM_MERGE_ADD_F64 3u
#define VM_MERGE_ADD_F64_HI 4u
#define VM_SLOT_LOCAL 0x80000000u
#define VM_KEY_EMPTY 0xFFFFFFFFFFFFFFFFull

struct VmJoin {
  const unsigned long long* keys;
  const unsigned int* rows;
  const unsigned int* special;
  uint32_t capacity_mask;
  uint32_t answer_slot;
  const unsigned long long* keys_hi;
};
struct VmJoinCol { const void* data; const unsigned char* is_null; };
#define VM_MAX_JOINS 2
#define VM_MAX_JOIN_COLS 24

struct VmParams {
  const VmInstr* prog;
  int32_t n_instr;
  int32_t n_staged;
  int32_t n_outputs;
  int32_t n_slots;
  int64_t n_rows;
  int64_t row_id_base;
  int32_t tile_rows;
  int32_t n_tiles;
  uint32_t acc_lds_off;
  uint32_t scratch_lds_off;
  uint32_t imm_pool_lds_off;
  uint32_t const_lds_off;
  uint32_t lds_bytes;
  int32_t count_sub_k;
  uint32_t flags;
  uint64_t slot_init0[VM_FAST_SLOTS];
  uint64_t slot_init1[VM_FAST_SLOTS];
  int32_t slot_kind[VM_FAST_SLOTS];
  VmAccRec* wg_partials;
  unsigned int* tile_counts;
  uint32_t part_n;
  uint32_t part_lds_off;
  uint32_t part_seg_cap;
  unsigned int* part_overflow;
  const unsigned int* tile_offsets;
  const unsigned long long* n_rows_dev;
  unsigned int* error_flag;
  unsigned long long* debug;
  unsigned long long* debug_pc;
  uint32_t debug_pc_lds_off;
  uint32_t uses_math;
  VmGroupTable group;
  VmJoin join[VM_MAX_JOINS];
  VmJoinCol join_cols[VM_MAX_JOIN_COLS];
  VmStagedCol staged[VM_MAX_STAGED];
  VmOutCol outputs[VM_MAX_OUTPUTS];
};
static_assert(sizeof(VmParams) <= 4096, "VmParams must fit the 4 KiB kernel-argument block");

#define VM_FLAG_XCD_CHUNKS 1u

#ifndef __HIPCC__
static inline const char* vm_op_name(uint16_t op) {
  static const char* names[] = {
#define X(n) #n,
      VM_OPS(X)
#undef X
  };
  return op < VM_OP_COUNT_ ? names[op] : "?";
}
#endif

#define SSGPU_FLAG_NAN_IN_MINMAX 0x100u

#endif
```

Baseline: 103.9 billion rows/s.

## Fuse scalar-aggregate finish into main kernel via last-block ticket reduction

Removes the separate finish_slots kernel launch. Each workgroup now pre-combines its per-wave partials and writes one record per slot. An atomic ticket picks the last workgroup to fold all partials, write the slot records, state and emitted scalars, and publish or reset the error flag. This saves a kernel launch and the larger partials traffic, but adds a grid-wide atomic and a serial tail reduction in one workgroup. It also adds error-flag plumbing so the ticket is reset after failures, and fixes FIRST/LAST fold semantics for empty images.

Measured after the change: 102.1 billion rows/s. 1.7% lower.

```diff
diff --git a/supersonic_amd/csrc/launch.h b/supersonic_amd/csrc/launch.h
--- a/supersonic_amd/csrc/launch.h
+++ b/supersonic_amd/csrc/launch.h
@@ -203,9 +203,6 @@
 void ssgpu_rtc_stats(long long* modules, long long* code_bytes, long long* compilations, long long* disk_hits);
 #endif
 hipError_t ssgpu_pipeline_set_max_lds(int bytes);
-hipError_t ssgpu_launch_finish_slots(const VmAccRec* partials, int n_slots, int n_parts, const int* slot_kind,
-                                     VmAccRec* out, uint64_t* state , hipStream_t stream,
-                                     const EmitDesc* descs = nullptr, int n_out = 0 );
 hipError_t ssgpu_launch_slots_to_state(const VmAccRec* recs, int n_slots, const int* slot_kind, uint64_t* state,
                                        hipStream_t stream);
 hipError_t ssgpu_launch_fold_state(const uint64_t* images, int n_images, uint64_t* state, int n_slots, const int* slot_kind, hipStream_t stream);
diff --git a/supersonic_amd/csrc/pipeline_kernels.hip b/supersonic_amd/csrc/pipeline_kernels.hip
--- a/supersonic_amd/csrc/pipeline_kernels.hip
+++ b/supersonic_amd/csrc/pipeline_kernels.hip
@@ -520,6 +520,142 @@
 }
 
 #ifndef SSGPU_RTC_PART
+__device__ __forceinline__ VmAccRec rec_identity(int kind) {
+  VmAccRec r; r.v0 = 0; r.v1 = 0; r.cnt = 0; r.pad = 0;
+  if (kind == SLOT_SUM_DD) { r.v0 = d2u(-0.0); r.v1 = d2u(0.0); }
+  return r;
+}
+__device__ __forceinline__ void combine_rec(int kind, VmAccRec& acc, const VmAccRec& r) {
+  if (r.cnt == 0) return;
+  switch (kind) {
+    case SLOT_COUNT:
+    case SLOT_SUM_INT: acc.v0 += r.v0; break;
+    case SLOT_SUM_DD: {
+      DD a; a.hi = u2d(acc.v0); a.lo = u2d(acc.v1);
+      DD b; b.hi = u2d(r.v0); b.lo = u2d(r.v1);
+      a = dd_add(a, b); acc.v0 = d2u(a.hi); acc.v1 = d2u(a.lo);
+    } break;
+    case SLOT_MIN_U64: acc.v0 = acc.cnt ? (r.v0 < acc.v0 ? r.v0 : acc.v0) : r.v0; break;
+    case SLOT_MAX_U64: acc.v0 = acc.cnt ? (r.v0 > acc.v0 ? r.v0 : acc.v0) : r.v0; break;
+    case SLOT_MIN_F64: acc.v0 = acc.cnt ? (u2d(r.v0) < u2d(acc.v0) ? r.v0 : acc.v0) : r.v0; break;
+    case SLOT_MAX_F64: acc.v0 = acc.cnt ? (u2d(acc.v0) < u2d(r.v0) ? r.v0 : acc.v0) : r.v0; break;
+    case SLOT_FIRST: if (!acc.cnt || r.v1 < acc.v1) { acc.v0 = r.v0; acc.v1 = r.v1; } break;
+    case SLOT_LAST: if (!acc.cnt || r.v1 >= acc.v1) { acc.v0 = r.v0; acc.v1 = r.v1; } break;
+  }
+  acc.cnt += r.cnt;
+}
+
+__device__ __forceinline__ void slot_to_state(const VmAccRec r, int kind, int s, int n_slots, u64* __restrict__ state) {
+  u64* sum_i = state; u64* cnt = state + n_slots; u64* hi = state + 2 * n_slots; u64* lo = state + 3 * n_slots;
+  u64* mn = state + 4 * n_slots; u64* mx = state + 5 * n_slots;
+  u64* mnf = state + 6 * n_slots; u64* mxf = state + 7 * n_slots;
+  const bool fl = kind == SLOT_FIRST || kind == SLOT_LAST;
+  sum_i[s] = (kind == SLOT_SUM_INT || kind == SLOT_COUNT || fl) ? r.v0 : 0;
+  cnt[s] = r.cnt;
+  hi[s] = kind == SLOT_SUM_DD ? r.v0 : d2u(0.0);
+  lo[s] = kind == SLOT_SUM_DD ? r.v1 : d2u(0.0);
+  mn[s] = (kind == SLOT_MIN_U64 && r.cnt) ? (r.v0 ^ 0x8000000000000000ull) : (kind == SLOT_FIRST && r.cnt) ? (r.v1 ^ 0x8000000000000000ull) : 0x7FFFFFFFFFFFFFFFull;
+  mx[s] = (kind == SLOT_MAX_U64 && r.cnt) ? (r.v0 ^ 0x8000000000000000ull) : (kind == SLOT_LAST && r.cnt) ? (r.v1 ^ 0x8000000000000000ull) : 0x8000000000000000ull;
+  mnf[s] = (kind == SLOT_MIN_F64 && r.cnt) ? r.v0 : d2u(__builtin_inf());
+  mxf[s] = (kind == SLOT_MAX_F64 && r.cnt) ? r.v0 : d2u(-__builtin_inf());
+}
+
+__device__ __forceinline__ void emit_value(void* dst, size_t idx, int out_kind, u64 v0, u64 v1) {
+  switch (out_kind) {
+    case EMIT_U64: reinterpret_cast<u64*>(dst)[idx] = v0; break;
+    case EMIT_I64KEY: reinterpret_cast<i64*>(dst)[idx] = unkey_i64(v0); break;
+    case EMIT_U32: reinterpret_cast<u32*>(dst)[idx] = (u32)v0; break;
+    case EMIT_I32KEY: reinterpret_cast<i32*>(dst)[idx] = (i32)unkey_i64(v0); break;
+    case EMIT_F64: reinterpret_cast<double*>(dst)[idx] = u2d(v0); break;
+    case EMIT_F32: reinterpret_cast<float*>(dst)[idx] = (float)u2d(v0); break;
+    case EMIT_DD_F64: { double hi = u2d(v0), lo = u2d(v1);
+      reinterpret_cast<double*>(dst)[idx] = (lo == 0.0) ? hi : hi + lo; } break;
+    case EMIT_DDRES_F64: { const double hi = u2d(v0), lo = u2d(v1), sm = hi + lo, bp = sm - hi;
+      reinterpret_cast<double*>(dst)[idx] = (lo == 0.0) ? 0.0 : (hi - (sm - bp)) + (lo - bp); } break;
+    case EMIT_DD_F32: { double hi = u2d(v0), lo = u2d(v1);
+      reinterpret_cast<float*>(dst)[idx] = (float)((lo == 0.0) ? hi : hi + lo); } break;
+    case EMIT_U8: reinterpret_cast<u8*>(dst)[idx] = (u8)(v0 != 0); break;
+    default: break;
+  }
+}
+__device__ __forceinline__ void emit_scalar_one(const EmitDesc d, const VmAccRec r) {
+  if (d.out_kind == EMIT_CNT_U64 || d.out_kind == EMIT_CNT_U32)
+    emit_value(d.data, 0, d.out_kind == EMIT_CNT_U64 ? EMIT_U64 : EMIT_U32, r.cnt, 0);
+  else
+    emit_value(d.data, 0, d.out_kind, r.v0, r.v1);
+  if (d.is_null) d.is_null[0] = r.cnt == 0;
+}
+
+#define VM_FOLD_BATCH 12
+__device__ __forceinline__ void vm_finish_scalar(const VmParams& P, int t) {
+  const int lane = t & 63, wave = t >> 6, ns = P.n_slots;
+  for (int s = t; s < ns; s += VM_COMPUTE_THREADS) {
+    const int kind = P.slot_kinds[s];
+    VmAccRec acc = rec_identity(kind);
+    for (int w = 0; w < VM_WAVES; ++w) combine_rec(kind, acc, *acc_rec(P, (u32)s, w));
+    VmAccRec* out = &P.wg_partials[(size_t)blockIdx.x * ns + s];
+    __hip_atomic_store(&out->v0, acc.v0, __ATOMIC_RELAXED, __HIP_MEMORY_SCOPE_AGENT);
+    __hip_atomic_store(&out->v1, acc.v1, __ATOMIC_RELAXED, __HIP_MEMORY_SCOPE_AGENT);
+    __hip_atomic_store(&out->cnt, acc.cnt, __ATOMIC_RELAXED, __HIP_MEMORY_SCOPE_AGENT);
+  }
+  asm volatile("s_waitcnt vmcnt(0)" ::: "memory");
+  __syncthreads();
+  u32* const last_flag = reinterpret_cast<u32*>(smem + P.scratch_lds_off);
+  if (t == 0) {
+    const u32 ticket = __hip_atomic_fetch_add(P.agg_ticket, 1u, __ATOMIC_RELAXED, __HIP_MEMORY_SCOPE_AGENT);
+    const bool last = ticket == gridDim.x - 1u;
+    if (last) {
+      __builtin_amdgcn_fence(__ATOMIC_ACQUIRE, "agent");
+      asm volatile("s_waitcnt vmcnt(0)" ::: "memory");
+    }
+    *last_flag = last ? 1u : 0u;
+  }
+  __syncthreads();
+  if (*last_flag == 0u) return;
+
+  const u32 grid = gridDim.x;
+  for (int s = wave; s < ns; s += VM_WAVES) {
+    const int kind = P.slot_kinds[s];
+    VmAccRec acc = rec_identity(kind);
+    for (u32 g0 = (u32)lane; g0 < grid + (u32)lane; g0 += 64u * VM_FOLD_BATCH) {
+      u64 v0[VM_FOLD_BATCH], v1[VM_FOLD_BATCH], cnt[VM_FOLD_BATCH];
+#pragma unroll
+      for (int j = 0; j < VM_FOLD_BATCH; ++j) {
+        const u32 g = g0 + 64u * (u32)j;
+        const VmAccRec* r = &P.wg_partials[(size_t)(g < grid ? g : grid - 1u) * ns + s];
+        v0[j] = r->v0; v1[j] = r->v1; cnt[j] = r->cnt;
+      }
+#pragma unroll
+      for (int j = 0; j < VM_FOLD_BATCH; ++j) {
+        VmAccRec r; r.v0 = v0[j]; r.v1 = v1[j]; r.cnt = g0 + 64u * (u32)j < grid ? cnt[j] : 0ull; r.pad = 0;
+        combine_rec(kind, acc, r);
+      }
+    }
+#pragma unroll
+    for (int d = 32; d > 0; d >>= 1) {
+      VmAccRec r; r.pad = 0;
+      r.v0 = __shfl_down((u64)acc.v0, d); r.v1 = __shfl_down((u64)acc.v1, d); r.cnt = __shfl_down((u64)acc.cnt, d);
+      combine_rec(kind, acc, r);
+    }
+    if (lane == 0) {
+      P.slot_recs[s] = acc;
+      if (P.state) slot_to_state(acc, kind, s, ns, (u64*)P.state);
+      *acc_rec(P, (u32)s, 0) = acc;
+    }
+  }
+  __syncthreads();
+  for (int i = t; i < P.n_emit; i += VM_COMPUTE_THREADS) { const EmitDesc d = P.emit_descs[i]; emit_scalar_one(d, *acc_rec(P, (u32)d.slot, 0)); }
+  if (t == 0) {
+    const u32 f = __hip_atomic_exchange(P.error_flag, 0u, __ATOMIC_RELAXED, __HIP_MEMORY_SCOPE_AGENT);
+    u32 pub = f;
+    if (P.flags & VM_FLAG_KEEP_ERRORS) {
+      const u32 old = __hip_atomic_load(P.error_publish, __ATOMIC_RELAXED, __HIP_MEMORY_SCOPE_AGENT);
+      pub = ((f & 0xFFu) ? (f & 0xFFu) : (old & 0xFFu)) | ((old | f) & ~0xFFu);
+    }
+    __hip_atomic_store(P.error_publish, pub, __ATOMIC_RELAXED, __HIP_MEMORY_SCOPE_AGENT);
+    __hip_atomic_store(P.agg_ticket, 0u, __ATOMIC_RELAXED, __HIP_MEMORY_SCOPE_AGENT);
+  }
+}
 template <int K, bool MATH>
 __global__ __launch_bounds__(VM_WG_THREADS, VM_WAVES_PER_EU) void ssgpu_pipeline_kernel(const VmParams P) {
 #ifdef SSGPU_RTC_STATIC_LDS
@@ -727,48 +863,12 @@
   }
 
   __syncthreads();
-  for (int s = t; s < P.n_slots; s += VM_COMPUTE_THREADS)
-    for (int w = 0; w < VM_WAVES; ++w)
-      P.wg_partials[((size_t)blockIdx.x * P.n_slots + s) * VM_WAVES + w] = *acc_rec(P, (u32)s, w);
+  if (!P.agg_ticket) return;
+  vm_finish_scalar(P, t);
 }
 #endif
 
 #ifndef __HIPCC_RTC__
-
-__device__ __forceinline__ void combine_rec(int kind, VmAccRec& acc, const VmAccRec& r) {
-  if (r.cnt == 0) return;
-  switch (kind) {
-    case SLOT_COUNT:
-    case SLOT_SUM_INT: acc.v0 += r.v0; break;
-    case SLOT_SUM_DD: {
-      DD a; a.hi = u2d(acc.v0); a.lo = u2d(acc.v1);
-      DD b; b.hi = u2d(r.v0); b.lo = u2d(r.v1);
-      a = dd_add(a, b); acc.v0 = d2u(a.hi); acc.v1 = d2u(a.lo);
-    } break;
-    case SLOT_MIN_U64: acc.v0 = acc.cnt ? (r.v0 < acc.v0 ? r.v0 : acc.v0) : r.v0; break;
-    case SLOT_MAX_U64: acc.v0 = acc.cnt ? (r.v0 > acc.v0 ? r.v0 : acc.v0) : r.v0; break;
-    case SLOT_MIN_F64: acc.v0 = acc.cnt ? (u2d(r.v0) < u2d(acc.v0) ? r.v0 : acc.v0) : r.v0; break;
-    case SLOT_MAX_F64: acc.v0 = acc.cnt ? (u2d(acc.v0) < u2d(r.v0) ? r.v0 : acc.v0) : r.v0; break;
-    case SLOT_FIRST: if (!acc.cnt || r.v1 < acc.v1) { acc.v0 = r.v0; acc.v1 = r.v1; } break;
-    case SLOT_LAST: if (!acc.cnt || r.v1 >= acc.v1) { acc.v0 = r.v0; acc.v1 = r.v1; } break;
-  }
-  acc.cnt += r.cnt;
-}
-
-__device__ __forceinline__ void slot_to_state(const VmAccRec r, int kind, int s, int n_slots, u64* __restrict__ state) {
-  u64* sum_i = state; u64* cnt = state + n_slots; u64* hi = state + 2 * n_slots; u64* lo = state + 3 * n_slots;
-  u64* mn = state + 4 * n_slots; u64* mx = state + 5 * n_slots;
-  u64* mnf = state + 6 * n_slots; u64* mxf = state + 7 * n_slots;
-  const bool fl = kind == SLOT_FIRST || kind == SLOT_LAST;
-  sum_i[s] = (kind == SLOT_SUM_INT || kind == SLOT_COUNT || fl) ? r.v0 : 0;
-  cnt[s] = r.cnt;
-  hi[s] = kind == SLOT_SUM_DD ? r.v0 : d2u(0.0);
-  lo[s] = kind == SLOT_SUM_DD ? r.v1 : d2u(0.0);
-  mn[s] = (kind == SLOT_MIN_U64 && r.cnt) ? (r.v0 ^ 0x8000000000000000ull) : (kind == SLOT_FIRST && r.cnt) ? (r.v1 ^ 0x8000000000000000ull) : 0x7FFFFFFFFFFFFFFFull;
-  mx[s] = (kind == SLOT_MAX_U64 && r.cnt) ? (r.v0 ^ 0x8000000000000000ull) : (kind == SLOT_LAST && r.cnt) ? (r.v1 ^ 0x8000000000000000ull) : 0x8000000000000000ull;
-  mnf[s] = (kind == SLOT_MIN_F64 && r.cnt) ? r.v0 : d2u(__builtin_inf());
-  mxf[s] = (kind == SLOT_MAX_F64 && r.cnt) ? r.v0 : d2u(-__builtin_inf());
-}
 __device__ __forceinline__ VmAccRec state_to_slot(const u64* __restrict__ state, int kind, int s, int n_slots) {
   VmAccRec r; r.v0 = 0; r.v1 = 0; r.pad = 0;
   r.cnt = state[n_slots + s];
@@ -790,31 +890,6 @@
   return r;
 }
 
-__device__ __forceinline__ void emit_scalar_one(const EmitDesc d, const VmAccRec r);
-__global__ __launch_bounds__(256) void ssgpu_finish_slots_kernel(const VmAccRec* __restrict__ partials, int n_slots,
-                                                                 int n_parts, const int* __restrict__ slot_kind,
-                                                                 VmAccRec* __restrict__ out, u64* __restrict__ state,
-                                                                 const EmitDesc* __restrict__ descs, int n_out) {
-  __shared__ VmAccRec tree[256];
-  const int s = blockIdx.x, t = threadIdx.x;
-  const int kind = slot_kind[s];
-  VmAccRec acc; acc.v0 = 0; acc.v1 = 0; acc.cnt = 0; acc.pad = 0;
-  if (kind == SLOT_SUM_DD) { acc.v0 = d2u(-0.0); acc.v1 = d2u(0.0); }
-  for (int i = t; i < n_parts; i += 256) {
-    const VmAccRec r = partials[((size_t)(i / VM_WAVES) * n_slots + s) * VM_WAVES + (i % VM_WAVES)];
-    combine_rec(kind, acc, r);
-  }
-  tree[t] = acc;
-  __syncthreads();
-  for (int stride = 128; stride > 0; stride >>= 1) {
-    if (t < stride) { VmAccRec a = tree[t]; combine_rec(kind, a, tree[t + stride]); tree[t] = a; }
-    __syncthreads();
-  }
-  if (t == 0) { out[s] = tree[0]; if (state) slot_to_state(tree[0], kind, s, n_slots, state); }
-  if (descs)
-    for (int i = t; i < n_out; i += 256) { const EmitDesc d = descs[i]; if (d.slot == s) emit_scalar_one(d, tree[0]); }
-}
-
 __global__ void ssgpu_slots_to_state_kernel(const VmAccRec* __restrict__ recs, int n_slots,
                                             const int* __restrict__ slot_kind, u64* __restrict__ state) {
   int s = blockIdx.x * blockDim.x + threadIdx.x;
@@ -828,34 +903,6 @@
   recs[s] = state_to_slot(state, slot_kind[s], s, n_slots);
 }
 
-
-__device__ __forceinline__ void emit_value(void* dst, size_t idx, int out_kind, u64 v0, u64 v1) {
-  switch (out_kind) {
-    case EMIT_U64: reinterpret_cast<u64*>(dst)[idx] = v0; break;
-    case EMIT_I64KEY: reinterpret_cast<i64*>(dst)[idx] = unkey_i64(v0); break;
-    case EMIT_U32: reinterpret_cast<u32*>(dst)[idx] = (u32)v0; break;
-    case EMIT_I32KEY: reinterpret_cast<i32*>(dst)[idx] = (i32)unkey_i64(v0); break;
-    case EMIT_F64: reinterpret_cast<double*>(dst)[idx] = u2d(v0); break;
-    case EMIT_F32: reinterpret_cast<float*>(dst)[idx] = (float)u2d(v0); break;
-    case EMIT_DD_F64: { double hi = u2d(v0), lo = u2d(v1);
-      reinterpret_cast<double*>(dst)[idx] = (lo == 0.0) ? hi : hi + lo; } break;
-    case EMIT_DDRES_F64: { const double hi = u2d(v0), lo = u2d(v1), sm = hi + lo, bp = sm - hi;
-      reinterpret_cast<double*>(dst)[idx] = (lo == 0.0) ? 0.0 : (hi - (sm - bp)) + (lo - bp); } break;
-    case EMIT_DD_F32: { double hi = u2d(v0), lo = u2d(v1);
-      reinterpret_cast<float*>(dst)[idx] = (float)((lo == 0.0) ? hi : hi + lo); } break;
-    case EMIT_U8: reinterpret_cast<u8*>(dst)[idx] = (u8)(v0 != 0); break;
-    default: break;
-  }
-}
-
-
-__device__ __forceinline__ void emit_scalar_one(const EmitDesc d, const VmAccRec r) {
-  if (d.out_kind == EMIT_CNT_U64 || d.out_kind == EMIT_CNT_U32)
-    emit_value(d.data, 0, d.out_kind == EMIT_CNT_U64 ? EMIT_U64 : EMIT_U32, r.cnt, 0);
-  else
-    emit_value(d.data, 0, d.out_kind, r.v0, r.v1);
-  if (d.is_null) d.is_null[0] = r.cnt == 0;
-}
 __global__ void ssgpu_emit_scalar_kernel(const VmAccRec* __restrict__ recs, const EmitDesc* __restrict__ descs,
                                          int n_out) {
   int i = blockIdx.x * blockDim.x + threadIdx.x;
@@ -1797,11 +1844,6 @@
   e = hipFuncSetAttribute(reinterpret_cast<const void*>(ssgpu_pipeline_kernel<4, true>), hipFuncAttributeMaxDynamicSharedMemorySize, bytes);
   return e;
 }
-hipError_t ssgpu_launch_finish_slots(const VmAccRec* partials, int n_slots, int n_parts, const int* slot_kind,
-                                     VmAccRec* out, uint64_t* state, hipStream_t stream, const EmitDesc* descs, int n_out) {
-  hipLaunchKernelGGL(ssgpu_finish_slots_kernel, dim3(n_slots), dim3(256), 0, stream, partials, n_slots, n_parts, slot_kind, out, (u64*)state, descs, n_out);
-  return hipGetLastError();
-}
 hipError_t ssgpu_launch_slots_to_state(const VmAccRec* recs, int n_slots, const int* slot_kind, uint64_t* state, hipStream_t stream) {
   int blocks = (n_slots + 63) / 64;
   hipLaunchKernelGGL(ssgpu_slots_to_state_kernel, dim3(blocks), dim3(64), 0, stream, recs, n_slots, slot_kind, (u64*)state);
@@ -1821,8 +1863,8 @@
   for (int r = 1; r < n_images; ++r) {
     u64 v[SSGPU_STATE_ARRAYS];
     for (int k = 0; k < SSGPU_STATE_ARRAYS; ++k) v[k] = images[(size_t)r * total + (size_t)k * n_slots + s];
-    if (kind == SLOT_FIRST) { if ((i64)v[4] < (i64)a[4]) a[0] = v[0]; }
-    else if (kind == SLOT_LAST) { if ((i64)v[5] > (i64)a[5]) a[0] = v[0]; }
+    if (kind == SLOT_FIRST) { if (v[1] && (!a[1] || (i64)v[4] < (i64)a[4])) a[0] = v[0]; }
+    else if (kind == SLOT_LAST) { if (v[1] && (!a[1] || (i64)v[5] > (i64)a[5])) a[0] = v[0]; }
     else a[0] += v[0];
     a[1] += v[1];
     a[2] = d2u(u2d(a[2]) + u2d(v[2]));
diff --git a/supersonic_amd/csrc/runtime.cpp b/supersonic_amd/csrc/runtime.cpp
--- a/supersonic_amd/csrc/runtime.cpp
+++ b/supersonic_amd/csrc/runtime.cpp
@@ -61,7 +61,6 @@
   int64_t async_handoff = 1;
   int64_t lazy_feedback = 0;
   int64_t part_prefetch = 1;
-  int64_t fuse_emit = 1;
   int64_t pscat_pipe = 1;
   int64_t pscat_threads = 0, pscat_rows = 0, pscat_wgs = 0;
   int64_t part_plain = 1;
@@ -207,6 +206,8 @@
   int n_instr_main = 0, n_instr_count = 0;
   int grid = 0;
   DevBuf wg_partials, slot_recs, slot_kind, emit_descs, state;
+  DevBuf agg_ctl;
+  bool agg_ctl_stale = false;
   DevBuf tile_counts, tile_offsets, total;
   DevBuf xstatus; uint64_t x_epoch = 0;
   DevBuf gkeys, gacc, gcnt, goverflow, gpattern, gmergeop;
@@ -260,7 +261,7 @@
   DevBuf route_scratch;
   uint64_t sort_epoch = 0;
   bool emit_ready = false;
-  bool emitted_with_finish = false;
+  bool emitted_by_run = false;
   bool pattern_ready = false;
   DevBuf out_arena;
   std::vector<OutCol> out;
@@ -458,7 +459,6 @@
   else if (k == "pscat_rows") c->pscat_rows = value;
   else if (k == "pscat_wgs") c->pscat_wgs = value;
   else if (k == "pscat_pipe") c->pscat_pipe = value;
-  else if (k == "fuse_emit") c->fuse_emit = value;
   else if (k == "part_prefetch") c->part_prefetch = value;
   else if (k == "lazy_feedback") c->lazy_feedback = value;
   else if (k == "async_handoff") c->async_handoff = value;
@@ -1288,7 +1288,7 @@
   const int grid = grid_for(c, ex.lay, P.n_tiles);
   ex.grid = grid;
   const int ns = st.main.n_slots;
-  HIP_TRY(c, ex.wg_partials.ensure((size_t)grid * ns * VM_WAVES * sizeof(VmAccRec)));
+  HIP_TRY(c, ex.wg_partials.ensure((size_t)grid * ns * sizeof(VmAccRec)));
   HIP_TRY(c, ex.slot_recs.ensure((size_t)ns * sizeof(VmAccRec)));
   HIP_TRY(c, ex.state.ensure((size_t)ns * SSGPU_STATE_ARRAYS * sizeof(uint64_t)));
   if (!ex.slot_kind.p) {
@@ -1298,8 +1298,24 @@
     HIP_TRY(c, ex.slot_kind.ensure(kinds.size() * sizeof(int)));
     HIP_TRY(c, hipMemcpy(ex.slot_kind.p, kinds.data(), kinds.size() * sizeof(int), hipMemcpyHostToDevice));
   }
+  if (!ex.agg_ctl.p || ex.agg_ctl_stale) {
+    HIP_TRY(c, ex.agg_ctl.ensure(16));
+    HIP_TRY(c, hipMemsetAsync(ex.agg_ctl.p, 0, 16, c->stream));
+    ex.agg_ctl_stale = false;
+  }
+  int n_emit = 0;
+  ex.emitted_by_run = false;
+  if (!stop_at_partial) { const int rc = prepare_scalar_emit(p, si, &n_emit); if (rc != SSGPU_OK) return rc; ex.emitted_by_run = true; }
   P.wg_partials = ex.wg_partials.as<VmAccRec>();
-  P.error_flag = ex.error_flag.as<unsigned int>();
+  P.agg_ticket = ex.agg_ctl.as<unsigned int>();
+  P.error_flag = ex.agg_ctl.as<unsigned int>() + 1;
+  P.error_publish = ex.error_flag.as<unsigned int>();
+  if (p->keep_error_flags) P.flags |= VM_FLAG_KEEP_ERRORS;
+  P.slot_kinds = ex.slot_kind.as<int32_t>();
+  P.slot_recs = ex.slot_recs.as<VmAccRec>();
+  P.state = stop_at_partial ? ex.state.as<uint64_t>() : nullptr;
+  P.emit_descs = ex.emitted_by_run ? ex.emit_descs.as<EmitDesc>() : nullptr;
+  P.n_emit = n_emit;
   if (c->debug_timing) {
     HIP_TRY(c, ex.debug.ensure((size_t)grid * 4 * 8));
     P.debug = ex.debug.as<unsigned long long>();
@@ -1309,13 +1325,7 @@
   HIP_TRY(c, launch_main(p, st, ex, P, ex.lay.K, grid));
   if (c->profile) HIP_TRY(c, hipEventRecord(p->ev_dom1, c->stream));
   { int rc = print_pc_profile(c, ex, st.main, P.n_instr); if (rc != SSGPU_OK) return rc; }
-  int n_emit = 0;
-  ex.emitted_with_finish = false;
-  if (!stop_at_partial && c->fuse_emit) { const int rc = prepare_scalar_emit(p, si, &n_emit); if (rc != SSGPU_OK) return rc; ex.emitted_with_finish = true; }
-  HIP_TRY(c, ssgpu_launch_finish_slots(ex.wg_partials.as<VmAccRec>(), ns, grid * VM_WAVES, ex.slot_kind.as<int>(),
-                                       ex.slot_recs.as<VmAccRec>(), stop_at_partial ? ex.state.as<uint64_t>() : nullptr, c->stream,
-                                       ex.emitted_with_finish ? ex.emit_descs.as<EmitDesc>() : nullptr, n_emit));
-  p->counters.n_launches += 2;
+  p->counters.n_launches += 1;
   p->counters.tile_rows = P.tile_rows; p->counters.grid = grid; p->counters.lds_bytes = (int32_t)ex.lay.lds_bytes;
   if (c->debug_timing) {
     std::vector<unsigned long long> dbg((size_t)grid * 4);
@@ -1386,7 +1396,7 @@
   int n_out = 0;
   const int rc = prepare_scalar_emit(p, si, &n_out);
   if (rc != SSGPU_OK) return rc;
-  if (ex.emitted_with_finish) { ex.emitted_with_finish = false; ex.out_rows = 1; return SSGPU_OK; }
+  if (ex.emitted_by_run) { ex.emitted_by_run = false; ex.out_rows = 1; return SSGPU_OK; }
   HIP_TRY(c, ssgpu_launch_emit_scalar(ex.slot_recs.as<VmAccRec>(), ex.emit_descs.as<EmitDesc>(), n_out, c->stream));
   p->counters.n_launches += 1;
   ex.out_rows = 1;
@@ -2655,12 +2665,12 @@
   return SSGPU_OK;
 }
 
-int check_error_flags(ssgpu_plan* p);
-
-int check_error_flags(ssgpu_plan* p) {
+int check_error_flags(ssgpu_plan* p, size_t n_stages = (size_t)-1);
+
+static int read_error_flags(ssgpu_plan* p, size_t n_stages) {
   ssgpu_ctx* c = p->ctx;
-  std::vector<uint32_t> flags(p->exec.size(), 0);
-  for (size_t i = 0; i < p->exec.size(); ++i)
+  std::vector<uint32_t> flags(std::min(n_stages, p->exec.size()), 0);
+  for (size_t i = 0; i < flags.size(); ++i)
     if (p->exec[i].error_flag.p)
       HIP_TRY(c, hipMemcpyAsync(&flags[i], p->exec[i].error_flag.p, 4, hipMemcpyDeviceToHost, c->stream));
   HIP_TRY(c, hipStreamSynchronize(c->stream));
@@ -2677,6 +2687,12 @@
     }
   }
   return SSGPU_OK;
+}
+
+int check_error_flags(ssgpu_plan* p, size_t n_stages) {
+  const int rc = read_error_flags(p, n_stages);
+  if (rc != SSGPU_OK) for (auto& ex : p->exec) ex.agg_ctl_stale = true;
+  return rc;
 }
 
 static int order_after_uploads(ssgpu_ctx* c) {
@@ -2731,7 +2747,13 @@
   return rc;
 }
 
+static int run_plan_stages(ssgpu_plan* p, const ssgpu_column* cols, int32_t n_cols, int64_t rows, int64_t row_id_base, bool partial);
 int run_plan(ssgpu_plan* p, const ssgpu_column* cols, int32_t n_cols, int64_t rows, int64_t row_id_base, bool partial) {
+  const int rc = run_plan_stages(p, cols, n_cols, rows, row_id_base, partial);
+  if (rc != SSGPU_OK) for (auto& ex : p->exec) ex.agg_ctl_stale = true;
+  return rc;
+}
+static int run_plan_stages(ssgpu_plan* p, const ssgpu_column* cols, int32_t n_cols, int64_t rows, int64_t row_id_base, bool partial) {
   ssgpu_ctx* c = p->ctx;
   if (!c || c->device < 0) { if (c) c->err = "no gfx950 device bound to this context (bind-only context)"; return SSGPU_ERROR_NO_DEVICE; }
   ssgpu_rtc_mode(!p->cached_only ? 0 : p->background && rows >= p->background_min_rows ? 2 : 1);
@@ -2776,7 +2798,7 @@
     if (c->profile_total) HIP_TRY(c, hipEventRecord(p->ev_begin, c->stream));
   }
   for (size_t si = 0; si < p->exec.size(); ++si)
-    if (p->exec[si].error_flag.p && !p->keep_error_flags && !(si == 0 && p->stages[si].kind == STAGE_GROUP_AGG)) HIP_TRY(c, hipMemsetAsync(p->exec[si].error_flag.p, 0, sizeof(uint32_t), c->stream));
+    if (p->exec[si].error_flag.p && !p->keep_error_flags && !(si == 0 && p->stages[si].kind == STAGE_GROUP_AGG) && p->stages[si].kind != STAGE_SCALAR_AGG) HIP_TRY(c, hipMemsetAsync(p->exec[si].error_flag.p, 0, sizeof(uint32_t), c->stream));
   int64_t alg_bytes = 0;
   for (size_t si = 0; si < p->stages.size(); ++si) {
     if (p->interrupted.exchange(0)) { c->err = "interrupted"; return SSGPU_INTERRUPTED; }
@@ -2813,7 +2835,7 @@
       } else {
         rc = stage_rows(p, si, &r);
         if (rc != SSGPU_OK) return rc;
-        rc = check_error_flags(p);
+        rc = check_error_flags(p, si + 1);
         if (rc != SSGPU_OK) return rc;
       }
       in.cols.clear();
diff --git a/supersonic_amd/csrc/vm.h b/supersonic_amd/csrc/vm.h
--- a/supersonic_amd/csrc/vm.h
+++ b/supersonic_amd/csrc/vm.h
@@ -231,6 +231,14 @@
   unsigned long long* debug_pc;
   uint32_t debug_pc_lds_off;
   uint32_t uses_math;
+  unsigned int* agg_ticket;
+  unsigned int* error_publish;
+  const int32_t* slot_kinds;
+  VmAccRec* slot_recs;
+  uint64_t* state;
+  const struct EmitDesc* emit_descs;
+  int32_t n_emit;
+  int32_t agg_pad;
   VmGroupTable group;
   VmJoin join[VM_MAX_JOINS];
   VmJoinCol join_cols[VM_MAX_JOIN_COLS];
@@ -240,6 +248,7 @@
 static_assert(sizeof(VmParams) <= 4096, "VmParams must fit the 4 KiB kernel-argument block");
 
 #define VM_FLAG_XCD_CHUNKS 1u
+#define VM_FLAG_KEEP_ERRORS 2u
 
 #ifndef __HIPCC__
 static inline const char* vm_op_name(uint16_t op) {
```
